# lhaippp/DMHomo

Measured on AMD Instinct MI355X. Metric: sampled images/sec (128x128, s_step=32), higher is better.
Workload: dtype f32; 1 GPU; DGM CFG-Unet dim=64 128x128 bs=25/GPU s_step=32 cond_scale=3 (BASELINE configs[1]); global_batch=25, cfg_mode=streams, hip_graph=True, weights=seeded random init

## Files before the change

dmhomo_amd/_lib.py:

```python
import ctypes as C
import os

import torch

_HERE = os.path.dirname(os.path.abspath(__file__))
LIB_PATH = os.environ.get('DMH_LIB_PATH') or os.path.join(_HERE, 'libdmhomo_hip.so')

c_f32p = C.c_void_p
c_i64 = C.c_int64
c_int = C.c_int
c_float = C.c_float


ABI_VERSION = 500


class DmhConv(C.Structure):
    _fields_ = [('struct_size', C.c_uint64)] + \
               [(n, C.c_void_p) for n in ('src0', 'src1', 'wpack', 'bias', 'in_coef', 'res', 'res_coef', 'out',
                                          'stats')] + \
               [(n, C.c_int32) for n in ('B', 'Hin', 'Win', 'C0', 'C1', 'Cout', 'KH', 'KW', 'stride', 'upsample2')] + \
               [('in_bound', C.c_void_p), ('in_bound_n', C.c_int32), ('fin_n', C.c_int32), ('fin_w', C.c_void_p),
                ('fin_b', C.c_void_p), ('fin_out', C.c_void_p), ('pix_stats', C.c_void_p), ('pix_eps', C.c_float),
                ('rows', C.c_void_p)]


class DmhPackJob(C.Structure):
    _fields_ = [('src', C.c_void_p), ('ws', C.c_void_p), ('wpack', C.c_void_p), ('Cout', C.c_int32), ('C0', C.c_int32),
                ('C1', C.c_int32), ('KH', C.c_int32), ('transposed', C.c_int32)]


class DmhStep(C.Structure):
    _fields_ = [('objective', C.c_int32), ('clip', C.c_int32), ('mode', C.c_int32), ('cond_scale', C.c_float),
                ('sqrt_recip_ac', C.c_float), ('sqrt_recipm1_ac', C.c_float), ('sqrt_ac', C.c_float),
                ('sqrt_1m_ac', C.c_float), ('c0', C.c_float), ('c1', C.c_float), ('c2', C.c_float)]


SIGNATURES = {
    'dmh_last_error': (C.c_char_p, []),
    'dmh_version': (c_int, []),
    'dmh_ws_standardize': (c_int, [c_f32p, c_f32p, c_int, c_int, c_float, C.c_void_p]),
    'dmh_conv_pack_floats': (c_i64, [c_int, c_int, c_int, c_int, c_int]),
    'dmh_pack_conv_weight': (c_int, [c_f32p, c_f32p, c_int, c_int, c_int, c_int, c_int, C.c_void_p]),
    'dmh_pack_conv_weights_multi': (c_int, [C.c_void_p, c_int, c_float, C.c_void_p]),
    'dmh_conv_up2_pack_floats': (c_i64, [c_int, c_int]),
    'dmh_pack_conv_weight_up2': (c_int, [c_f32p, c_f32p, c_int, c_int, C.c_void_p]),
    'dmh_conv_tiles': (c_int, [c_int, c_int, c_int, c_int]),
    'dmh_conv2d': (c_int, [C.POINTER(DmhConv), C.c_void_p]),
    'dmh_rows_from_keep': (c_int, [C.c_void_p, c_int, c_int, C.c_void_p, C.c_void_p]),
    'dmh_gn_finalize': (c_int, [c_f32p, c_int, c_f32p, c_f32p, c_f32p, c_i64, c_f32p, c_int, c_int, c_int, c_int,
                                c_float, C.c_void_p, C.c_void_p]),
    'dmh_gn_finalize_bound': (c_int, [c_f32p, c_int, c_f32p, c_f32p, c_f32p, c_i64, c_f32p, c_f32p, c_int, c_int, c_int,
                                      c_int, c_float, C.c_void_p, C.c_void_p]),
    'dmh_gn_silu_residual': (c_int, [c_f32p, c_f32p, c_f32p, c_f32p, c_int, c_int, c_int, C.c_void_p, C.c_void_p]),
    'dmh_gn_silu_residual_stats': (c_int, [c_f32p, c_f32p, c_f32p, c_f32p, c_f32p, c_int, c_int, c_int, c_float, C.c_void_p,
                                           C.c_void_p]),
    'dmh_chan_layernorm': (c_int, [c_f32p, c_f32p, c_f32p, c_f32p, c_i64, c_int, c_float, C.c_void_p, c_i64, C.c_void_p]),
    'dmh_linattn_splits': (c_int, [c_int]),
    'dmh_linattn_partial_floats': (c_i64, [c_int, c_int]),
    'dmh_linattn_context': (c_int, [c_f32p, c_f32p, c_int, c_int, C.c_void_p, C.c_void_p]),
    'dmh_linattn_merge': (c_int, [c_f32p, c_f32p, c_int, c_int, C.c_void_p, C.c_void_p]),
    'dmh_linattn_apply': (c_int, [c_f32p, c_f32p, c_f32p, c_int, c_int, c_float, C.c_void_p, C.c_void_p]),
    'dmh_conv_wgrad_workspace_floats': (c_i64, [c_int, c_int, c_int, c_int, c_int, c_int, c_int]),
    'dmh_conv_wgrad': (c_int, [c_f32p, c_f32p, c_f32p, c_f32p, c_f32p, c_f32p, c_f32p, c_int, c_int, c_int, c_int, c_int,
                               c_int, c_int, c_int, C.c_void_p]),
    'dmh_conv_unshuffle_wgrad_workspace_floats': (c_i64, [c_int, c_int, c_int, c_int, c_int]),
    'dmh_conv_unshuffle_wgrad': (c_int, [c_f32p, c_f32p, c_f32p, c_f32p, c_f32p, c_int, c_int, c_int, c_int, c_int, C.c_void_p]),
    'dmh_s2d_shift': (c_int, [c_f32p, c_f32p, c_int, c_int, c_int, c_int, C.c_void_p]),
    'dmh_d2s': (c_int, [c_f32p, c_f32p, c_int, c_int, c_int, c_int, C.c_void_p]),
    'dmh_sumpool2': (c_int, [c_f32p, c_f32p, c_int, c_int, c_int, c_int, C.c_void_p]),
    'dmh_gn_finalize_train': (c_int, [c_f32p, c_int, c_f32p, c_f32p, c_f32p, c_i64, c_f32p, c_f32p, c_int, c_int, c_int,
                                      c_int, c_float, C.c_void_p]),
    'dmh_gn_bwd_chunks': (c_int, [c_int]),
    'dmh_gn_silu_backward': (c_int, [c_f32p, c_f32p, c_f32p, c_f32p, c_f32p, c_f32p, c_f32p, c_i64, c_f32p, c_f32p, c_f32p,
                                     c_f32p, c_int, c_int, c_int, c_int, C.c_void_p]),
    'dmh_sum_over_batch': (c_int, [c_f32p, c_f32p, c_int, c_i64, C.c_void_p]),
    'dmh_ws_backward': (c_int, [c_f32p, c_f32p, c_f32p, c_int, c_int, c_float, C.c_void_p]),
    'dmh_lnb_blocks': (c_int, []),
    'dmh_chan_layernorm_backward': (c_int, [c_f32p, c_f32p, c_f32p, c_f32p, c_f32p, c_i64, c_int, c_float, C.c_void_p]),
    'dmh_linattn_merge_ms': (c_int, [c_f32p, c_f32p, c_f32p, c_int, c_int, C.c_void_p]),
    'dmh_linattn_bwd_workspace_floats': (c_i64, [c_int, c_int]),
    'dmh_linattn_backward': (c_int, [c_f32p, c_f32p, c_f32p, c_f32p, c_f32p, c_f32p, c_int, c_int, c_float, C.c_void_p]),
    'dmh_bgemm': (c_int, [c_f32p, C.POINTER(c_i64), c_f32p, C.POINTER(c_i64), c_f32p, C.POINTER(c_i64), c_int, c_int, c_int,
                          c_int, c_int, c_float, C.c_void_p]),
    'dmh_softmax_rows': (c_int, [c_f32p, c_f32p, c_i64, c_int, C.c_void_p]),
    'dmh_softmax_rows_backward': (c_int, [c_f32p, c_f32p, c_i64, c_int, C.c_void_p]),
    'dmh_act': (c_int, [c_f32p, c_f32p, c_f32p, c_i64, c_int, C.c_void_p]),
    'dmh_class_embed_backward': (c_int, [c_f32p, c_f32p, c_f32p, c_f32p, c_f32p, c_int, c_int, c_int, C.c_void_p]),
    'dmh_loss_backward_ddp': (c_int, [c_f32p, c_f32p, c_f32p, c_f32p, c_int, c_i64, c_int, c_float, C.c_void_p]),
    'dmh_loss_backward': (c_int, [c_f32p, c_f32p, c_f32p, c_f32p, c_f32p, c_f32p, c_f32p, c_f32p, c_int, c_int, c_int, c_int,
                                  C.c_void_p]),
    'dmh_sumsq_blocks': (c_int, []),
    'dmh_sumsq': (c_int, [c_f32p, c_i64, c_f32p, C.c_void_p]),
    'dmh_gradnorm_finalize': (c_int, [c_f32p, c_int, c_float, c_f32p, C.c_void_p]),
    'dmh_adam': (c_int, [c_f32p, c_f32p, c_f32p, c_f32p, c_f32p, c_i64, c_float, c_float, c_float, c_float, c_int,
                         C.c_void_p]),
    'dmh_ema': (c_int, [c_f32p, c_f32p, c_i64, c_float, C.c_void_p]),
    'dmh_multi_blocks': (c_i64, [C.c_void_p, c_int]),
    'dmh_sumsq_multi': (c_int, [C.c_void_p, C.c_void_p, c_int, c_f32p, C.c_void_p]),
    'dmh_adam_multi': (c_int, [C.c_void_p, C.c_void_p, C.c_void_p, C.c_void_p, C.c_void_p, c_int, c_f32p, c_float, c_float,
                               c_float, c_float, c_int, C.c_void_p]),
    'dmh_resize_bilinear_u8': (c_int, [C.c_void_p, c_f32p, c_int, c_int, c_int, c_int, c_int, c_int, c_i64, c_float,
                                       C.c_void_p]),
    'dmh_mask_open_nearest': (c_int, [c_f32p, c_f32p, c_int, c_int, c_int, c_int, c_int, c_i64, C.c_void_p]),
    'dmh_pixel_stats': (c_int, [c_f32p, c_f32p, c_i64, c_int, c_float, C.c_void_p, c_i64, C.c_void_p]),
    'dmh_linattn_fused_pack_floats': (c_i64, [c_int]),
    'dmh_linattn_fused_pack': (c_int, [c_f32p, c_f32p, c_int, C.c_void_p]),
    'dmh_linattn_fused_splits': (c_int, [c_int, c_int]),
    'dmh_linattn_fused_context': (c_int, [c_f32p, c_f32p, c_f32p, c_f32p, c_f32p, c_int, c_int, c_int, C.c_void_p, C.c_void_p]),
    'dmh_linattn_out_pack_floats': (c_i64, []),
    'dmh_linattn_out_pack': (c_int, [c_f32p, c_f32p, C.c_void_p]),
    'dmh_linattn_fused_apply_out': (c_int, [c_f32p, c_f32p, c_f32p, c_f32p, c_f32p, c_f32p, c_f32p, c_f32p, c_f32p, c_int,
                                            c_int, c_int, c_float, c_float, C.c_void_p, C.c_void_p]),
    'dmh_linattn_merge_n': (c_int, [c_f32p, c_f32p, c_int, c_int, c_int, C.c_void_p, C.c_void_p]),
    'dmh_linattn_fused_apply': (c_int, [c_f32p, c_f32p, c_f32p, c_f32p, c_f32p, c_f32p, c_int, c_int, c_int, c_float,
                                        C.c_void_p, C.c_void_p]),
    'dmh_attention': (c_int, [c_f32p, c_f32p, c_int, c_int, c_float, C.c_void_p, C.c_void_p]),
    'dmh_sinusoidal_embed': (c_int, [C.c_void_p, c_f32p, c_f32p, c_int, c_int, C.c_void_p]),
    'dmh_fourier_embed': (c_int, [C.c_void_p, c_f32p, c_f32p, c_int, c_int, C.c_void_p]),
    'dmh_class_embed': (c_int, [C.c_void_p, C.c_void_p, c_f32p, c_f32p, c_f32p, c_int, c_int, c_int, C.c_void_p]),
    'dmh_linear': (c_int, [c_f32p, c_i64, c_f32p, c_f32p, c_f32p, c_i64, c_int, c_int, c_int, c_int, c_int,
                           C.c_void_p]),
    'dmh_ss_gather': (c_int, [c_f32p, c_f32p, c_f32p, C.c_void_p, C.c_void_p, C.c_void_p, c_int, c_f32p, c_int, c_int, c_int,
                              C.c_void_p]),
    'dmh_assemble_input': (c_int, [c_f32p, c_int, c_f32p, c_int, c_f32p, c_f32p, c_int, c_int, c_int, c_int,
                                   C.c_void_p]),
    'dmh_final_conv_nchw': (c_int, [c_f32p, c_f32p, c_f32p, c_f32p, c_int, c_int, c_int, c_int, C.c_void_p]),
    'dmh_sampler_step': (c_int, [C.POINTER(DmhStep), c_f32p, c_f32p, c_f32p, c_f32p, c_f32p, c_f32p, c_f32p, c_i64,
                                 C.c_void_p, c_i64, C.c_void_p]),
    'dmh_sampler_step_dev': (c_int, [C.c_void_p, c_f32p, c_f32p, c_f32p, c_f32p, c_f32p, c_f32p, c_f32p, c_i64, C.c_void_p,
                                     c_i64, C.c_void_p]),
    'dmh_sampler_seek': (c_int, [C.c_void_p, c_int, C.c_void_p, C.c_void_p, c_int, C.c_void_p, C.c_void_p, c_int,
                                 C.c_void_p]),
    'dmh_sampler_step_ddp_dev': (c_int, [C.c_void_p, C.c_void_p, C.c_void_p, c_f32p, c_f32p, c_f32p, C.c_void_p, C.c_void_p,
                                         c_f32p, c_f32p, c_int, c_int, c_int, c_int, c_int, C.c_void_p]),
    'dmh_rng_indexed': (c_int, [c_f32p, c_int, c_i64, C.c_void_p, C.c_void_p, c_int, C.c_void_p]),
    'dmh_rng_keep_mask': (c_int, [C.c_void_p, c_int, C.c_void_p, C.c_void_p, c_float, C.c_void_p]),
    'dmh_rows_lincomb': (c_int, [c_f32p, c_f32p, c_f32p, c_f32p, c_f32p, c_f32p, c_int, c_i64, c_int, C.c_void_p]),
    'dmh_pixel_grid': (c_int, [c_f32p, c_int, c_int, c_int, c_float, C.c_void_p]),
    'dmh_norm_grid': (c_int, [c_f32p, c_f32p, c_int, c_int, c_int, C.c_void_p]),
    'dmh_homography_flow_points': (c_int, [C.c_void_p, C.c_void_p, C.c_void_p, c_int, c_int, c_int, c_int, c_int, C.c_void_p]),
    'dmh_dlt_points': (c_int, [C.c_void_p, C.c_void_p, C.c_void_p, C.c_void_p, c_int, c_int, C.c_void_p]),
    'dmh_affine': (c_int, [c_f32p, c_f32p, c_float, c_float, c_i64, C.c_void_p]),
    'dmh_affine_tail': (c_int, [c_f32p, c_int, c_int, c_int, c_int, c_float, c_float, C.c_void_p]),
    'dmh_q_sample': (c_int, [c_f32p, c_f32p, c_f32p, c_f32p, c_f32p, c_int, c_i64, C.c_void_p]),
    'dmh_diff_mean': (c_int, [c_f32p, c_f32p, c_f32p, c_int, C.c_void_p, c_f32p, c_int, c_int, c_int, C.c_void_p]),
    'dmh_loss_combine': (c_int, [c_f32p, c_f32p, c_f32p, c_f32p, c_int, C.c_void_p]),
    'dmh_to_uint8': (c_int, [c_f32p, C.c_void_p, c_i64, C.c_void_p]),
    'dmh_homography_flow': (c_int, [C.c_void_p, c_f32p, c_f32p, c_int, c_int, c_int, c_float, C.c_void_p]),
    'dmh_flow_to_image': (c_int, [c_f32p, c_f32p, c_int, c_int, c_float, C.c_void_p]),
    'dmh_flow_warp': (c_int, [c_f32p, c_f32p, c_f32p, C.c_void_p, C.c_void_p, c_int, c_int, c_int, c_int, c_int, c_int,
                              C.c_void_p]),
    'dmh_dlt_homography': (c_int, [c_f32p, C.c_void_p, C.c_void_p, c_int, c_int, c_int, C.c_void_p]),
    'dmh_post_process': (c_int, [c_f32p, c_f32p, c_f32p, c_f32p, c_f32p, c_int, c_int, c_int, C.c_void_p]),
    'dmh_preview_sheet': (c_int, [c_f32p, c_f32p, c_f32p, C.c_void_p, C.c_void_p, c_int, c_int, c_int, c_int, c_int, c_int,
                                  C.c_void_p]),
    'dmh_homography_warp': (c_int, [c_f32p, C.c_void_p, c_f32p, c_int, c_int, c_int, c_int, c_int, C.c_void_p]),
}

DLT_BLOCKS = 64

_lib = None


class DmhError(RuntimeError):
    pass


def lib():
    global _lib
    if _lib is None:
        if not os.path.exists(LIB_PATH):
            raise DmhError(f'{LIB_PATH} not found: build it with `python -c "import __graft_entry__ as g; g.build()"` '
                           f'or `make -C dmhomo_amd/csrc` — dmhomo_amd has no CPU / eager fallback')
        h = C.CDLL(LIB_PATH)
        for name, (res, args) in SIGNATURES.items():
            fn = getattr(h, name)
            fn.restype = res
            fn.argtypes = args
        got = int(h.dmh_version())
        if got != ABI_VERSION:
            raise DmhError(f'{LIB_PATH} reports ABI version {got}, this binding was written against {ABI_VERSION} '
                           f'(include/dmhomo_hip.h): rebuild the library with `make -C dmhomo_amd/csrc`')
        _lib = h
    return _lib


def stream():
    return C.c_void_p(torch.cuda.current_stream().cuda_stream)


def call(name, *args):
    h = lib()
    rc = getattr(h, name)(*args, stream())
    if rc != 0:
        raise DmhError(f'{name} failed ({rc}): {h.dmh_last_error().decode()}')


def ptr(t, dtype=torch.float32):
    if t is None:
        return None
    if not t.is_cuda:
        raise DmhError('dmhomo_amd kernels need tensors on the GPU (got a CPU tensor); there is no CPU path')
    if dtype is not None and t.dtype != dtype:
        raise DmhError(f'expected dtype {dtype}, got {t.dtype}')
    if not t.is_contiguous():
        raise DmhError('expected a contiguous tensor')
    return C.c_void_p(t.data_ptr())
```

dmhomo_amd/csrc/conv.hip:

```cpp
#include <stdlib.h>

#include "common.h"

#include "conv_args.h"

template <int KH, int KW, int S, int UPS, int KC, int TH, int TW>
struct ConvCfg {
  static constexpr int BM = TH * TW;
  static constexpr int MB = BM / 128;
  static constexpr int IN_H = (TH - 1) * S + KH;
  static constexpr int IN_W = (TW - 1) * S + KW;
  static constexpr int IN_PIX = IN_H * IN_W;
  static constexpr int KCP = KC + 4;
  static constexpr int C4 = KC / 4;
  static constexpr int NLOAD = (IN_PIX * C4 + 255) / 256;
  static constexpr int WL = 64 * C4 / 256;
  static constexpr int PAD = (S == 1) ? (KH / 2) : (KH == 4 ? 1 : 0);
  static constexpr int IN_FLOATS = IN_PIX * KCP;
  static constexpr int W_FLOATS = 64 * KCP;
  static constexpr int EPI_BYTES = 4 * 32 * 68 * 4;
  static constexpr int MAIN_BYTES = (IN_FLOATS + 2 * W_FLOATS) * 4;
  static constexpr int LDS_BYTES = MAIN_BYTES > EPI_BYTES ? MAIN_BYTES : EPI_BYTES;
};

template <int MB, int TH, int TW>
__device__ __forceinline__ void conv_epilogue(floatx16 (&acc)[MB][2], const ConvArgs& p, float* lds, int b, int n0,
                                              int oy0, int ox0, int tile_in_sample) {
  constexpr int EP = EpilogueRows::EP;
  const int lane = threadIdx.x & 63, wave = threadIdx.x >> 6, half = lane >> 5, l31 = lane & 31;
  float* wl = lds + wave * (32 * EP);
  EpilogueRows er(p, b, n0);
#pragma unroll
  for (int mb = 0; mb < MB; ++mb) {
    __syncthreads();
#pragma unroll
    for (int nb = 0; nb < 2; ++nb)
#pragma unroll
      for (int r = 0; r < 16; ++r) wl[((r & 3) + 8 * (r >> 2) + 4 * half) * EP + nb * 32 + l31] = acc[mb][nb][r];
    __syncthreads();
    er.template store_rows<TW>(p, wl, wave * (MB * 32) + mb * 32, oy0, ox0);
  }
  er.write_stats(p, lds, tile_in_sample);
}

template <int KH, int KW, int S, int UPS, int KC, int TH, int TW, int WPE>
__global__ __launch_bounds__(256, WPE) void conv_igemm_kernel(ConvArgs p) {
  using Cfg = ConvCfg<KH, KW, S, UPS, KC, TH, TW>;
  constexpr int MB = Cfg::MB, IN_W = Cfg::IN_W, IN_PIX = Cfg::IN_PIX, KCP = Cfg::KCP, C4 = Cfg::C4;
  constexpr int NLOAD = Cfg::NLOAD, WL = Cfg::WL, NTAPS = KH * KW;

  extern __shared__ __attribute__((aligned(16))) float lds[];
  float* in_tile = lds;
  float* w_tile = lds + Cfg::IN_FLOATS;

  const int tid = threadIdx.x;
  const int lane = tid & 63;
  const int wave = tid >> 6;
  const int half = lane >> 5;
  const int l31 = lane & 31;

  int t = blockIdx.x;
  const int tx = t % p.tilesX;
  t /= p.tilesX;
  const int ty = t % p.tilesY;
  if (t / p.tilesY >= dmh_rows_n(p.rows, p.B)) return;
  const int b = dmh_rows_phys(p.rows, t / p.tilesY);
  const int nt = blockIdx.y;
  const int n0 = nt * 64;
  const int tile_in_sample = ty * p.tilesX + tx;

  const int oy0 = ty * TH, ox0 = tx * TW;
  const int iy0 = oy0 * S - Cfg::PAD, ix0 = ox0 * S - Cfg::PAD;
  const int Hlim = UPS ? p.Hin * 2 : p.Hin;
  const int Wlim = UPS ? p.Win * 2 : p.Win;

  int arow[MB];
#pragma unroll
  for (int mb = 0; mb < MB; ++mb) {
    const int r = wave * (MB * 32) + mb * 32 + l31;
    const int py = r / TW, px = r % TW;
    arow[mb] = ((py * S) * IN_W + px * S) * KCP + half * 4;
  }
  const int brow = l31 * KCP + half * 4;

  floatx16 acc[MB][2];
#pragma unroll
  for (int mb = 0; mb < MB; ++mb)
#pragma unroll
    for (int nb = 0; nb < 2; ++nb)
#pragma unroll
      for (int r = 0; r < 16; ++r) acc[mb][nb][r] = 0.f;

  const int nchunks = p.nch0 + p.nch1;
  const float* wbase = p.wpack + (size_t)nt * nchunks * NTAPS * 64 * KC;

  float4 wreg[WL];
#pragma unroll
  for (int i = 0; i < WL; ++i) wreg[i] = ld4(wbase + (size_t)(tid + i * 256) * 4);

  const int c4 = tid % C4;
  int wbuf = 0;

  float4 v[NLOAD];
  float4 ca, cb;
  int poff[NLOAD];
  unsigned inside = 0;
#pragma unroll
  for (int i = 0; i < NLOAD; ++i) {
    const int pix = (tid + i * 256) / C4;
    const int pixc = pix < IN_PIX ? pix : IN_PIX - 1;
    const int yy = iy0 + pixc / IN_W, xx = ix0 + pixc % IN_W;
    const bool ok = pix < IN_PIX && yy >= 0 && yy < Hlim && xx >= 0 && xx < Wlim;
    const int yc = min(max(yy, 0), Hlim - 1), xc = min(max(xx, 0), Wlim - 1);
    const int sy = UPS ? (yc >> 1) : yc, sx = UPS ? (xc >> 1) : xc;
    poff[i] = (b * p.Hin + sy) * p.Win + sx;
    inside |= (ok ? 1u : 0u) << i;
  }
  auto issue_chunk_loads = [&](int ch) {
    const bool s1 = ch >= p.nch0;
    const float* src = s1 ? p.src1 : p.src0;
    const int Csrc = s1 ? p.C1 : p.C0;
    const int c = (s1 ? ch - p.nch0 : ch) * KC + c4 * 4;
    const int cc = c < Csrc ? c : 0;
#pragma unroll
    for (int i = 0; i < NLOAD; ++i) v[i] = ld4(src + (size_t)poff[i] * Csrc + cc);
    ca = make_float4(1.f, 1.f, 1.f, 1.f);
    cb = make_float4(0.f, 0.f, 0.f, 0.f);
    if (p.in_coef != nullptr && !s1) {
      ca = ld4(p.in_coef + (size_t)(b * 2 + 0) * p.C0 + cc);
      cb = ld4(p.in_coef + (size_t)(b * 2 + 1) * p.C0 + cc);
    }
  };
  issue_chunk_loads(0);
  const int wr_in0 = (tid / C4) * KCP + c4 * 4;
  const int wr_w0 = (tid / C4) * KCP + (tid % C4) * 4;

  for (int ch = 0; ch < nchunks; ++ch) {
    const bool s1c = ch >= p.nch0;
    const bool pro = (p.in_coef != nullptr) && !s1c;
    const bool cvalid = (s1c ? ch - p.nch0 : ch) * KC + c4 * 4 < (s1c ? p.C1 : p.C0);
    const unsigned msk = cvalid ? inside : 0u;
    __syncthreads();
#pragma unroll
    for (int i = 0; i < NLOAD; ++i) {
      if ((i + 1) * 256 <= IN_PIX * C4 || (tid + i * 256) / C4 < IN_PIX) {
        float4 x = v[i];
        if (!((msk >> i) & 1u)) {
          x = make_float4(0.f, 0.f, 0.f, 0.f);
        } else if (pro) {
          x.x = silu_fast(fmaf(ca.x, x.x, cb.x));
          x.y = silu_fast(fmaf(ca.y, x.y, cb.y));
          x.z = silu_fast(fmaf(ca.z, x.z, cb.z));
          x.w = silu_fast(fmaf(ca.w, x.w, cb.w));
        }
        st4(in_tile + wr_in0 + i * (256 / C4) * KCP, x);
      }
    }

    for (int tap = 0; tap < NTAPS; ++tap) {
      float* wt = w_tile + wbuf * Cfg::W_FLOATS;
#pragma unroll
      for (int i = 0; i < WL; ++i) st4(wt + wr_w0 + i * (256 / C4) * KCP, wreg[i]);
      __syncthreads();
      {
        int nch = ch, ntap = tap + 1;
        if (ntap == NTAPS) {
          ntap = 0;
          nch = ch + 1;
        }
        if (nch < nchunks) {
          const float* wsrc = wbase + ((size_t)nch * NTAPS + ntap) * 64 * KC;
#pragma unroll
          for (int i = 0; i < WL; ++i) wreg[i] = ld4(wsrc + (size_t)(tid + i * 256) * 4);
        }
        if (tap == NTAPS - 1) issue_chunk_loads(ch + 1 < nchunks ? ch + 1 : ch);
      }
      __builtin_amdgcn_sched_barrier(0);
      const int kh = tap / KW, kw = tap % KW;
      const float* at = in_tile + (kh * IN_W + kw) * KCP;
      const float* bt = wt + brow;
#pragma unroll
      for (int k8 = 0; k8 < KC / 8; ++k8) {
        float4 a[MB], bq[2];
#pragma unroll
        for (int mb = 0; mb < MB; ++mb) a[mb] = ld4(at + arow[mb] + k8 * 8);
#pragma unroll
        for (int nb = 0; nb < 2; ++nb) bq[nb] = ld4(bt + nb * 32 * KCP + k8 * 8);
#pragma unroll
        for (int mb = 0; mb < MB; ++mb)
#pragma unroll
          for (int nb = 0; nb < 2; ++nb) {
            acc[mb][nb] = __builtin_amdgcn_mfma_f32_32x32x2f32(a[mb].x, bq[nb].x, acc[mb][nb], 0, 0, 0);
            acc[mb][nb] = __builtin_amdgcn_mfma_f32_32x32x2f32(a[mb].y, bq[nb].y, acc[mb][nb], 0, 0, 0);
            acc[mb][nb] = __builtin_amdgcn_mfma_f32_32x32x2f32(a[mb].z, bq[nb].z, acc[mb][nb], 0, 0, 0);
            acc[mb][nb] = __builtin_amdgcn_mfma_f32_32x32x2f32(a[mb].w, bq[nb].w, acc[mb][nb], 0, 0, 0);
          }
      }
      __builtin_amdgcn_sched_barrier(0);
      wbuf ^= 1;
    }
  }

  conv_epilogue<MB, TH, TW>(acc, p, lds, b, n0, oy0, ox0, tile_in_sample);
}

__global__ void pack_conv_weight_kernel(const float* __restrict__ w, float* __restrict__ wp, int Cout, int C0,
                                        int C1, int KH, int KW, int KC, int nch0, int nch1, int64_t total) {
  const int64_t idx = (int64_t)blockIdx.x * blockDim.x + threadIdx.x;
  if (idx >= total) return;
  int64_t r = idx;
  const int k = r % KC;
  r /= KC;
  const int j = r % 64;
  r /= 64;
  const int tap = r % (KH * KW);
  r /= (KH * KW);
  const int ch = r % (nch0 + nch1);
  const int nt = r / (nch0 + nch1);
  const int o = nt * 64 + j;
  int c;
  bool ok;
  if (ch < nch0) {
    c = ch * KC + k;
    ok = c < C0;
  } else {
    c = (ch - nch0) * KC + k;
    ok = c < C1;
    c += C0;
  }
  float val = 0.f;
  if (ok && o < Cout) val = w[((size_t)o * (C0 + C1) + c) * (KH * KW) + tap];
  wp[idx] = val;
}

__global__ __launch_bounds__(256) void ws_standardize_kernel(const float* __restrict__ w, float* __restrict__ out,
                                                             int K, float eps) {
  __shared__ float red[8];
  const int o = blockIdx.x;
  const float* wr = w + (size_t)o * K;
  float s = 0.f;
  for (int i = threadIdx.x; i < K; i += 256) s += wr[i];
  for (int off = 32; off; off >>= 1) s += __shfl_xor(s, off);
  if ((threadIdx.x & 63) == 0) red[threadIdx.x >> 6] = s;
  __syncthreads();
  const float mean = (red[0] + red[1] + red[2] + red[3]) / (float)K;
  float q = 0.f;
  for (int i = threadIdx.x; i < K; i += 256) {
    const float d = wr[i] - mean;
    q = fmaf(d, d, q);
  }
  for (int off = 32; off; off >>= 1) q += __shfl_xor(q, off);
  if ((threadIdx.x & 63) == 0) red[4 + (threadIdx.x >> 6)] = q;
  __syncthreads();
  const float var = (red[4] + red[5] + red[6] + red[7]) / (float)K;
  const float rstd = 1.0f / sqrtf(var + eps);
  for (int i = threadIdx.x; i < K; i += 256) out[(size_t)o * K + i] = (wr[i] - mean) * rstd;
}

template <int KH, int KW, int S, int UPS, int KC, int TH, int TW, int WPE = 2>
static int launch_conv(const DmhConv* d, int Hout, int Wout, hipStream_t st) {
  using Cfg = ConvCfg<KH, KW, S, UPS, KC, TH, TW>;
  ConvArgs a = fill_conv_args(d, Hout, Wout, KC, TH, TW);
  dim3 grid(a.tilesX * a.tilesY * a.B, cdiv(a.Cout, 64));
  hipLaunchKernelGGL((conv_igemm_kernel<KH, KW, S, UPS, KC, TH, TW, WPE>), grid, dim3(256), Cfg::LDS_BYTES, st, a);
  DMH_CHECK_LAUNCH("dmh_conv2d");
  return DMH_OK;
}

#define DMH_CONV3_DEFAULT 9
static int conv3_variant() {
  static int v = -1;
  if (v < 0) {
    const char* e = getenv("DMH_CONV3_VARIANT");
    v = e ? atoi(e) : DMH_CONV3_DEFAULT;
    if (v != 0 && v != 6) v = DMH_CONV3_DEFAULT;
  }
  return v;
}

static bool use_f16x3(int KH, int stride) {
  return conv3_variant() == 9 && stride == 1 && (KH == 3 || KH == 1 || KH == 7);
}
static bool use_f16x3_s2d(int KH, int stride, int C0, int C1) {
  return conv3_variant() == 9 && KH == 4 && stride == 2 && C1 == 0 && C0 % 32 == 0;
}

static int conv_out_dim(int in, int KH, int stride, int ups) {
  if (ups) return in * 2;
  if (stride == 1) return in;
  return KH == 4 ? (in + 2 - 4) / 2 + 1 : in / 2;
}

static int conv_th(int KH, int stride) {
  if (stride == 2) return 8;
  if (use_f16x3(KH, stride)) return 8;
  if (KH == 3 && conv3_variant() == 6) return 8;
  return 16;
}

extern "C" int dmh_conv_tiles(int Hout, int Wout, int KH, int stride) {
  if (!dmh_dims_ok({Hout, Wout})) return -1;
  return cdiv(Hout, conv_th(KH, stride)) * cdiv(Wout, 16);
}

extern "C" int64_t dmh_conv_pack_floats(int Cout, int C0, int C1, int KH, int KW) {
  if (!dmh_dims_ok({Cout, C0}) || !dmh_dims_ok({C1}, 0) || !dmh_dims_ok({KH, KW}, 1, 16)) return -1;
  if (KH == 3 && conv3_variant() == 6) return dmh_wino_pack_floats(Cout, C0, C1);
  if (use_f16x3(KH, (KH == 4 || KH == 2) ? 2 : 1) || use_f16x3_s2d(KH, 2, C0, C1))
    return dmh_f16x3_pack_floats(Cout, C0, C1, KH, KW);
  const int stride = (KH == 4 || KH == 2) ? 2 : 1;
  const int KC = conv_kc(KH, stride);
  return (int64_t)cdiv(Cout, 64) * (cdiv(C0, KC) + cdiv(C1, KC)) * KH * KW * 64 * KC;
}

extern "C" int dmh_pack_conv_weight(const float* w, float* wpack, int Cout, int C0, int C1, int KH, int KW,
                                    void* stream) {
  DMH_REQUIRE(w && wpack && Cout > 0 && C0 > 0 && C1 >= 0, "dmh_pack_conv_weight: bad arguments");
  DMH_REQUIRE(KH == KW && (KH == 1 || KH == 2 || KH == 3 || KH == 4 || KH == 7),
              "dmh_pack_conv_weight: unsupported kernel %dx%d", KH, KW);
  if (KH == 3 && conv3_variant() == 6) return dmh_wino_pack(w, wpack, Cout, C0, C1, (hipStream_t)stream);
  if (use_f16x3(KH, (KH == 4 || KH == 2) ? 2 : 1) || use_f16x3_s2d(KH, 2, C0, C1))
    return dmh_f16x3_pack(w, wpack, Cout, C0, C1, KH, KW, (hipStream_t)stream);
  const int stride = (KH == 4 || KH == 2) ? 2 : 1;
  const int KC = conv_kc(KH, stride);
  const int nch0 = cdiv(C0, KC), nch1 = cdiv(C1, KC);
  const int64_t total = dmh_conv_pack_floats(Cout, C0, C1, KH, KW);
  hipLaunchKernelGGL(pack_conv_weight_kernel, dim3((unsigned)cdiv64(total, 256)), dim3(256), 0, (hipStream_t)stream,
                     w, wpack, Cout, C0, C1, KH, KW, KC, nch0, nch1, total);
  DMH_CHECK_LAUNCH("dmh_pack_conv_weight");
  return DMH_OK;
}

extern "C" int64_t dmh_conv_up2_pack_floats(int Cout, int C0) {
  if (!dmh_dims_ok({Cout, C0})) return -1;
  if (!use_f16x3(3, 1) || Cout % 64 != 0 || C0 % 4 != 0) return -1;
  return dmh_f16x3_up2_pack_floats(Cout, C0);
}
extern "C" int dmh_pack_conv_weight_up2(const float* w, float* wpack, int Cout, int C0, void* stream) {
  DMH_REQUIRE(w && wpack && dmh_conv_up2_pack_floats(Cout, C0) > 0, "dmh_pack_conv_weight_up2: bad arguments");
  return dmh_f16x3_up2_pack(w, wpack, Cout, C0, (hipStream_t)stream);
}

extern "C" int dmh_pack_conv_weights_multi(const DmhPackJob* jobs, int njobs, float ws_eps, void* stream) {
  DMH_REQUIRE(jobs && njobs > 0, "dmh_pack_conv_weights_multi: bad arguments");
  DMH_REQUIRE(conv3_variant() == 9, "dmh_pack_conv_weights_multi: only the fp16-piece images (DMH_CONV3_VARIANT=9)");
  for (int i = 0; i < njobs; ++i) {
    const DmhPackJob& j = jobs[i];
    DMH_REQUIRE(j.src && j.wpack && j.Cout > 0 && j.C0 > 0 && j.C1 >= 0 && (j.KH == 1 || j.KH == 3) &&
                    (j.transposed == 0 || (j.transposed == 1 && j.C1 == 0)),
                "dmh_pack_conv_weights_multi: job %d: stride-1 1x1 / 3x3 weights only (Cout %d, C0 %d, C1 %d, KH %d, transposed %d)",
                i, j.Cout, j.C0, j.C1, j.KH, j.transposed);
  }
  return dmh_f16x3_pack_multi(jobs, njobs, ws_eps, (hipStream_t)stream);
}

extern "C" int dmh_ws_standardize(const float* w, float* w_out, int Cout, int K, float eps, void* stream) {
  DMH_REQUIRE(w && w_out && Cout > 0 && K > 0, "dmh_ws_standardize: bad arguments");
  hipLaunchKernelGGL(ws_standardize_kernel, dim3(Cout), dim3(256), 0, (hipStream_t)stream, w, w_out, K, eps);
  DMH_CHECK_LAUNCH("dmh_ws_standardize");
  return DMH_OK;
}

extern "C" int dmh_conv2d(const DmhConv* d, void* stream) {
  DMH_REQUIRE(d && d->struct_size == sizeof(DmhConv),
              "dmh_conv2d: DmhConv.struct_size is %llu, this library's DmhConv has %llu bytes (header / library mismatch)",
              d ? (unsigned long long)d->struct_size : 0ull, (unsigned long long)sizeof(DmhConv));
  DMH_REQUIRE(d->src0 && d->wpack, "dmh_conv2d: null pointer");
  DMH_REQUIRE(d->B > 0 && d->Hin > 0 && d->Win > 0 && d->C0 > 0 && d->Cout > 0, "dmh_conv2d: bad shape");
  DMH_REQUIRE(d->C0 % 4 == 0 && (!d->src1 || d->C1 % 4 == 0),
              "dmh_conv2d: input channels must be a multiple of 4 (got %d, %d)", d->C0, d->C1);
  DMH_REQUIRE(!(d->in_coef && d->src1), "dmh_conv2d: the GroupNorm prologue applies to a single source");
  DMH_REQUIRE(!(d->res_coef && !d->res), "dmh_conv2d: res_coef without res");
  DMH_REQUIRE(d->Cout % 4 == 0, "dmh_conv2d: Cout must be a multiple of 4 (got %d)", d->Cout);
  DMH_REQUIRE(!d->in_bound || (d->in_coef && d->in_bound_n > 0 && d->in_bound_n <= 64),
              "dmh_conv2d: in_bound needs in_coef and 1..64 bounds per sample (got %d)", d->in_bound_n);
  hipStream_t st = (hipStream_t)stream;
  const int Hout = conv_out_dim(d->Hin, d->KH, d->stride, d->upsample2);
  const int Wout = conv_out_dim(d->Win, d->KW, d->stride, d->upsample2);
  const int key = d->KH * 100 + d->stride * 10 + d->upsample2;
  DMH_REQUIRE(d->KH == d->KW, "dmh_conv2d: non-square kernel");
  if (d->fin_w) {
    DMH_REQUIRE(d->fin_out && d->fin_n > 0 && d->fin_n <= 8, "dmh_conv2d: fin_w needs fin_out and 1 <= fin_n <= 8 (got %d)",
                d->fin_n);
    DMH_REQUIRE(d->KH == 1 && d->stride == 1 && d->Cout <= 64 && use_f16x3(1, 1),
                "dmh_conv2d: the fused final projection rides on the 1x1 fp16-piece kernel with Cout <= 64 (got %dx%d, Cout %d)",
                d->KH, d->KW, d->Cout);
  } else {
    DMH_REQUIRE(d->out, "dmh_conv2d: null pointer");
  }
  DMH_REQUIRE(!d->pix_stats || (d->KH == 1 && d->stride == 1 && d->Cout == 64 && use_f16x3(1, 1)),
              "dmh_conv2d: pix_stats rides on the 1x1 fp16-piece kernel with Cout == 64 (got %dx%d, Cout %d)", d->KH, d->KW,
              d->Cout);
  switch (key) {
    case 110:
      if (use_f16x3(1, 1)) return dmh_f16x3_launch(d, Hout, Wout, st);
      return launch_conv<1, 1, 1, 0, 32, 16, 16>(d, Hout, Wout, st);
    case 310:
      switch (conv3_variant()) {
        case 6: return dmh_wino_launch(d, Hout, Wout, st);
        case 9: return dmh_f16x3_launch(d, Hout, Wout, st);
        default: return launch_conv<3, 3, 1, 0, 32, 16, 16, 2>(d, Hout, Wout, st);
      }
    case 311:
      switch (conv3_variant()) {
        case 6: return dmh_wino_launch(d, Hout, Wout, st);
        case 9: return dmh_f16x3_launch(d, Hout, Wout, st);
        default: return launch_conv<3, 3, 1, 1, 32, 16, 16, 2>(d, Hout, Wout, st);
      }
    case 312:
      DMH_REQUIRE(use_f16x3(3, 1) && !d->src1 && d->Cout % 64 == 0 && !d->stats,
                  "dmh_conv2d: the sub-pixel upsampling conv needs the fp16-piece kernels, one source, Cout %% 64 == 0, no stats");
      return dmh_f16x3_launch_up2(d, Hout, Wout, st);
    case 710:
      if (use_f16x3(7, 1)) return dmh_f16x3_launch(d, Hout, Wout, st);
      return launch_conv<7, 7, 1, 0, 16, 16, 16>(d, Hout, Wout, st);
    case 420:
      if (use_f16x3_s2d(4, 2, d->C0, d->src1 ? d->C1 : 0)) {
        DMH_REQUIRE(!d->in_coef, "dmh_conv2d: the 4x4 / stride-2 conv takes no GroupNorm prologue");
        return dmh_f16x3_launch(d, Hout, Wout, st);
      }
      return launch_conv<4, 4, 2, 0, 16, 8, 16>(d, Hout, Wout, st);
    case 220:
      DMH_REQUIRE(d->Hin % 2 == 0 && d->Win % 2 == 0, "dmh_conv2d: 2x2/s2 needs even input size");
      return launch_conv<2, 2, 2, 0, 16, 8, 16>(d, Hout, Wout, st);
    default:
      dmh_set_error("dmh_conv2d: unsupported variant k=%d stride=%d upsample=%d", d->KH, d->stride, d->upsample2);
      return DMH_EINVAL;
  }
}
```

dmhomo_amd/csrc/conv_args.h:

```cpp
#pragma once
#include "common.h"

typedef float floatx16 __attribute__((ext_vector_type(16)));

struct ConvArgs {
  const float* src0;
  const float* src1;
  const float* wpack;
  const float* bias;
  const float* in_coef;
  const float* res;
  const float* res_coef;
  float* out;
  float* stats;
  const float* oscale;
  const float* in_bound;
  int in_bound_n;
  int fin_n;
  const float* fin_w;
  const float* fin_b;
  float* fin_out;
  float* pix_stats;
  float pix_eps;
  int B, Hin, Win, C0, C1, Cout, Hout, Wout;
  int nch0, nch1, tilesX, tilesY;
  int ablate;
  int xcd;
  const int32_t* rows;
};


static inline ConvArgs fill_conv_args(const DmhConv* d, int Hout, int Wout, int KC, int TH, int TW) {
  ConvArgs a;
  a.src0 = d->src0;
  a.src1 = d->src1;
  a.wpack = d->wpack;
  a.bias = d->bias;
  a.in_coef = d->in_coef;
  a.res = d->res;
  a.res_coef = d->res_coef;
  a.out = d->out;
  a.stats = d->stats;
  a.oscale = nullptr;
  a.in_bound = d->in_coef ? d->in_bound : nullptr;
  a.in_bound_n = d->in_bound_n;
  a.fin_n = d->fin_w ? d->fin_n : 0;
  a.fin_w = d->fin_w;
  a.fin_b = d->fin_b;
  a.fin_out = d->fin_out;
  a.pix_stats = d->pix_stats;
  a.pix_eps = d->pix_eps;
  a.B = d->B;
  a.Hin = d->Hin;
  a.Win = d->Win;
  a.C0 = d->C0;
  a.C1 = d->src1 ? d->C1 : 0;
  a.Cout = d->Cout;
  a.Hout = Hout;
  a.Wout = Wout;
  a.nch0 = cdiv(a.C0, KC);
  a.nch1 = cdiv(a.C1, KC);
  a.tilesX = cdiv(Wout, TW);
  a.tilesY = cdiv(Hout, TH);
  a.ablate = 0;
  a.xcd = 1;
  a.rows = d->rows;
  return a;
}


int64_t dmh_wino_pack_floats(int Cout, int C0, int C1);
int dmh_wino_pack(const float* w, float* wpack, int Cout, int C0, int C1, hipStream_t st);
int dmh_wino_launch(const DmhConv* d, int Hout, int Wout, hipStream_t st);


int64_t dmh_f16x3_pack_floats(int Cout, int C0, int C1, int KH, int KW);
int dmh_f16x3_pack(const float* w, float* wpack, int Cout, int C0, int C1, int KH, int KW, hipStream_t st);
int dmh_f16x3_launch(const DmhConv* d, int Hout, int Wout, hipStream_t st);
int dmh_f16x3_pack_multi(const DmhPackJob* jobs, int njobs, float eps, hipStream_t st);
int64_t dmh_f16x3_up2_pack_floats(int Cout, int C0);
int dmh_f16x3_up2_pack(const float* w, float* wpack, int Cout, int C0, hipStream_t st);
int dmh_f16x3_launch_up2(const DmhConv* d, int Hout, int Wout, hipStream_t st);


struct EpilogueRows {
  static constexpr int EP = 68;
  int b, n0, chn, c4, rsub;
  bool cok;
  float4 bias, ra, rb, s1, s2, osc;

  __device__ __forceinline__ EpilogueRows(const ConvArgs& p, int b_, int n0_) : b(b_), n0(n0_) {
    const int lane = threadIdx.x & 63;
    c4 = lane & 15;
    rsub = lane >> 4;
    chn = n0 + c4 * 4;
    cok = chn < p.Cout;
    bias = make_float4(0.f, 0.f, 0.f, 0.f);
    ra = bias;
    rb = bias;
    s1 = bias;
    s2 = bias;
    osc = make_float4(1.f, 1.f, 1.f, 1.f);
    if (cok && p.oscale) osc = ld4(p.oscale + chn);
    if (cok && p.bias) bias = ld4(p.bias + chn);
    if (cok && p.res_coef) {
      ra = ld4(p.res_coef + (size_t)(b * 2 + 0) * p.Cout + chn);
      rb = ld4(p.res_coef + (size_t)(b * 2 + 1) * p.Cout + chn);
    }
  }

  template <int TW, bool FIN = false>
  __device__ __forceinline__ void store_rows(const ConvArgs& p, const float* wl, int row_base, int oy0, int ox0,
                                             int mul = 1, int dy = 0, int dx = 0) {
    const int c4_ = c4;
    store_rows_fn<TW, 8, FIN>(p, [wl, c4_](int rr) { return ld4(wl + rr * EP + c4_ * 4); }, row_base, oy0, ox0, mul, dy, dx);
  }

  size_t oo[8];
  bool okr[8];
  float4 rv[8];
  bool pre = false;
  template <int TW, int NR = 8>
  __device__ __forceinline__ void prefetch_rows(const ConvArgs& p, int row_base, int oy0, int ox0, int mul = 1, int dy = 0,
                                                int dx = 0) {
#pragma unroll
    for (int i = 0; i < NR; ++i) {
      const int row = row_base + i * 4 + rsub;
      const int oy = (oy0 + row / TW) * mul + dy, ox = (ox0 + row % TW) * mul + dx;
      okr[i] = cok && oy < p.Hout && ox < p.Wout;
      const int oyc = min(oy, p.Hout - 1), oxc = min(ox, p.Wout - 1);
      oo[i] = ((size_t)(b * p.Hout + oyc) * p.Wout + oxc) * p.Cout + (cok ? chn : 0);
    }
    if (p.res) {
#pragma unroll
      for (int i = 0; i < NR; ++i) rv[i] = ld4(p.res + oo[i]);
    }
    pre = true;
  }

  template <int TW, int NR = 8, bool FIN = false, typename Fetch>
  __device__ __forceinline__ void store_rows_fn(const ConvArgs& p, Fetch fetch, int row_base, int oy0, int ox0,
                                                int mul = 1, int dy = 0, int dx = 0) {
    if (!pre) prefetch_rows<TW, NR>(p, row_base, oy0, ox0, mul, dy, dx);
    pre = false;
    float4 val[8];
#pragma unroll
    for (int i = 0; i < NR; ++i) val[i] = fetch(i * 4 + rsub);
#pragma unroll
    for (int i = 0; i < NR; ++i) {
      val[i].x = fmaf(val[i].x, osc.x, bias.x);
      val[i].y = fmaf(val[i].y, osc.y, bias.y);
      val[i].z = fmaf(val[i].z, osc.z, bias.z);
      val[i].w = fmaf(val[i].w, osc.w, bias.w);
    }
    if (p.res) {
      if (p.res_coef) {
#pragma unroll
        for (int i = 0; i < NR; ++i) {
          val[i].x += silu_fast(fmaf(ra.x, rv[i].x, rb.x));
          val[i].y += silu_fast(fmaf(ra.y, rv[i].y, rb.y));
          val[i].z += silu_fast(fmaf(ra.z, rv[i].z, rb.z));
          val[i].w += silu_fast(fmaf(ra.w, rv[i].w, rb.w));
        }
      } else {
#pragma unroll
        for (int i = 0; i < NR; ++i) {
          val[i].x += rv[i].x;
          val[i].y += rv[i].y;
          val[i].z += rv[i].z;
          val[i].w += rv[i].w;
        }
      }
    }
    if constexpr (FIN) {
      if (p.fin_n > 0) {
        const int hw = p.Hout * p.Wout;
#pragma unroll
        for (int o = 0; o < 8; ++o) {
          if (o < p.fin_n) {
            const float4 wq = cok ? ld4(p.fin_w + (size_t)o * p.Cout + chn) : make_float4(0.f, 0.f, 0.f, 0.f);
            const float bo = p.fin_b ? p.fin_b[o] : 0.f;
#pragma unroll
            for (int i = 0; i < NR; ++i) {
              float acc = fmaf(val[i].x, wq.x, 0.f);
              acc = fmaf(val[i].y, wq.y, acc);
              acc = fmaf(val[i].z, wq.z, acc);
              acc = fmaf(val[i].w, wq.w, acc);
              const float t = row16_sum(acc);
              const int row = row_base + i * 4 + rsub;
              const int oy = (oy0 + row / TW) * mul + dy, ox = (ox0 + row % TW) * mul + dx;
              if (c4 == o && oy < p.Hout && ox < p.Wout) p.fin_out[((size_t)b * p.fin_n + o) * hw + oy * p.Wout + ox] = t + bo;
            }
          }
        }
      }
      if (p.pix_stats) {
#pragma unroll
        for (int i = 0; i < NR; ++i) {
          float s = (val[i].x + val[i].y) + (val[i].z + val[i].w);
          s = lanes_sum<16>(s);
          const float mean = s / 64.0f;
          const float dx_ = val[i].x - mean, dy_ = val[i].y - mean, dz_ = val[i].z - mean, dw_ = val[i].w - mean;
          float qsum = (dx_ * dx_ + dy_ * dy_) + (dz_ * dz_ + dw_ * dw_);
          qsum = lanes_sum<16>(qsum);
          if (c4 == 0 && okr[i]) {
            float* ps = p.pix_stats + (oo[i] / (size_t)p.Cout) * 2;
            ps[0] = mean;
            ps[1] = 1.0f / sqrtf(qsum / 64.0f + p.pix_eps);
          }
        }
      }
    }
#pragma unroll
    for (int i = 0; i < NR; ++i) {
      if (okr[i] && (!FIN || p.out)) st4(p.out + oo[i], val[i]);
      const float k = okr[i] ? 1.f : 0.f;
      const float vx = val[i].x * k, vy = val[i].y * k, vz = val[i].z * k, vw = val[i].w * k;
      s1.x += vx;
      s1.y += vy;
      s1.z += vz;
      s1.w += vw;
      s2.x = fmaf(vx, vx, s2.x);
      s2.y = fmaf(vy, vy, s2.y);
      s2.z = fmaf(vz, vz, s2.z);
      s2.w = fmaf(vw, vw, s2.w);
    }
  }

  template <int WM, int WN, int TH>
  __device__ __forceinline__ void write_stats_grid(const ConvArgs& p, float* lds, int ty, int tx, int by = -1) {
    if (by < 0) by = blockIdx.y;
    if (!p.stats) return;
    const int lane = threadIdx.x & 63, wave = threadIdx.x >> 6, tid = threadIdx.x;
    s1.x = rows_sum(s1.x);
    s1.y = rows_sum(s1.y);
    s1.z = rows_sum(s1.z);
    s1.w = rows_sum(s1.w);
    s2.x = rows_sum(s2.x);
    s2.y = rows_sum(s2.y);
    s2.z = rows_sum(s2.z);
    s2.w = rows_sum(s2.w);
    __syncthreads();
    float* red = lds;
    if (lane < 16) {
      float* q = red + (wave * 64 + c4 * 4) * 2;
      q[0] = s1.x;
      q[1] = s2.x;
      q[2] = s1.y;
      q[3] = s2.y;
      q[4] = s1.z;
      q[5] = s2.z;
      q[6] = s1.w;
      q[7] = s2.w;
    }
    __syncthreads();
    if (tid < 128) {
      const int q = tid >> 6, c = tid & 63;
      const int g = WN == 1 ? q : 0, wnq = WN == 1 ? 0 : q;
      const int chan = (by * WN + wnq) * 64 + c;
      const int srow = ty * (TH / 8) + g;
      if (chan < p.Cout && srow * 8 < p.Hout) {
        const int w0 = (g * 2 + 0) * WN + wnq, w1 = (g * 2 + 1) * WN + wnq;
        const float a0 = red[(w0 * 64 + c) * 2 + 0] + red[(w1 * 64 + c) * 2 + 0];
        const float a1 = red[(w0 * 64 + c) * 2 + 1] + red[(w1 * 64 + c) * 2 + 1];
        const int stiles = ((p.Hout + 7) / 8) * p.tilesX;
        float* st = p.stats + ((size_t)(b * stiles + srow * p.tilesX + tx) * p.Cout + chan) * 2;
        st[0] = a0;
        st[1] = a1;
      }
    }
  }

  __device__ __forceinline__ void write_stats(const ConvArgs& p, float* lds, int tile_in_sample) {
    if (!p.stats) return;
    const int lane = threadIdx.x & 63, wave = (threadIdx.x >> 6) & 3, tid = threadIdx.x & 255;
    lds += (threadIdx.x >> 8) * 512;
    s1.x = rows_sum(s1.x);
    s1.y = rows_sum(s1.y);
    s1.z = rows_sum(s1.z);
    s1.w = rows_sum(s1.w);
    s2.x = rows_sum(s2.x);
    s2.y = rows_sum(s2.y);
    s2.z = rows_sum(s2.z);
    s2.w = rows_sum(s2.w);
    __syncthreads();
    float* red = lds;
    if (lane < 16) {
      float* q = red + (wave * 64 + c4 * 4) * 2;
      q[0] = s1.x;
      q[1] = s2.x;
      q[2] = s1.y;
      q[3] = s2.y;
      q[4] = s1.z;
      q[5] = s2.z;
      q[6] = s1.w;
      q[7] = s2.w;
    }
    __syncthreads();
    if (tid < 64 && n0 + tid < p.Cout) {
      float a0 = 0.f, a1 = 0.f;
#pragma unroll
      for (int w = 0; w < 4; ++w) {
        a0 += red[(w * 64 + tid) * 2 + 0];
        a1 += red[(w * 64 + tid) * 2 + 1];
      }
      float* st = p.stats + ((size_t)(b * p.tilesX * p.tilesY + tile_in_sample) * p.Cout + n0 + tid) * 2;
      st[0] = a0;
      st[1] = a1;
    }
  }
};
```

dmhomo_amd/csrc/conv_f16x3.hip:

```cpp
#include <stdlib.h>

#include "common.h"

#include "conv_args.h"

typedef _Float16 half8 __attribute__((ext_vector_type(8)));
typedef _Float16 half4 __attribute__((ext_vector_type(4)));
typedef float float4v __attribute__((ext_vector_type(4)));

namespace {

constexpr int KC = 32;
constexpr int PITCH = 160;
constexpr int STEP_U4 = 4 * 64;

template <int KH, int KW, int S, int UPS, int TH, int TW, int WM, int WN>
struct F16Cfg {
  static_assert(WM * WN == 4, "four waves per workgroup");
  static constexpr bool SUB = UPS == 3;
  static_assert(SUB || TH * TW == WM * 64, "64 pixels per wave");
  static_assert(!SUB || (KH == 2 && KW == 2 && S == 1 && TH == 4 && TW == 16 && WM == 4 && WN == 1), "sub-pixel geometry");
  static constexpr int IN_H = SUB ? TH + 2 : (TH - 1) * S + KH;
  static constexpr int IN_W = SUB ? TW + 2 : (TW - 1) * S + KW;
  static constexpr int IN_PIX = IN_H * IN_W;
  static constexpr int QS = UPS == 4 ? 2 : 3, NQ = 1 << QS;
  static constexpr int NLOAD = (IN_PIX * NQ + 255) / 256;
  static constexpr int PAD = UPS == 2 ? 0 : ((S == 1) ? (KH / 2) : (KH == 4 ? 1 : 0));
  static constexpr int ROWP = IN_W * PITCH;
  static constexpr int IN_BYTES = IN_H * ROWP;
  static constexpr int EPI_BYTES = 4 * 32 * EpilogueRows::EP * 4;
  static constexpr int TILE_BYTES = IN_BYTES > EPI_BYTES ? IN_BYTES : EPI_BYTES;
  static constexpr int LDS_BYTES = TILE_BYTES + 16;
};

__device__ __forceinline__ unsigned absbits(float x) { return __float_as_uint(x) & 0x7fffffffu; }

__device__ __forceinline__ int64_t f16x3_frag_floats_dev(int Cout, int C0, int C1, int T) {
  return (int64_t)((Cout + 63) / 64) * ((C0 + KC - 1) / KC + (C1 + KC - 1) / KC) * T * 2 * STEP_U4 * 4;
}

}

template <int KH, int KW, int S, int UPS, int TH, int TW, int WM, int WN>
__global__ __launch_bounds__(256, 2) void conv_f16x3_kernel(ConvArgs p) {
  using Cfg = F16Cfg<KH, KW, S, UPS, TH, TW, WM, WN>;
  constexpr bool PK = UPS == 4;
  constexpr int IN_W = Cfg::IN_W, IN_PIX = Cfg::IN_PIX, NLOAD = Cfg::NLOAD, NTAPS = PK ? (KH * KW + 1) / 2 : KH * KW,
                ROWP = Cfg::ROWP;

  extern __shared__ __attribute__((aligned(16))) float lds[];
  unsigned char* in_tile = reinterpret_cast<unsigned char*>(lds);
  unsigned* mxslot = reinterpret_cast<unsigned*>(in_tile + Cfg::TILE_BYTES);

  const int tid = threadIdx.x;
  const int lane = tid & 63;
  const int wave = tid >> 6;
  const int wave_u = __builtin_amdgcn_readfirstlane(wave);
  const int kg = lane >> 4;
  const int l15 = lane & 15;
  const int wm = wave / WN, wn = wave % WN;

  int t = blockIdx.x, by = blockIdx.y, nb = gridDim.x;
  if (p.rows) {
    nb = p.tilesX * p.tilesY * p.rows[0];
    const int lin = t + by * (int)gridDim.x;
    if (lin >= nb * (int)gridDim.y) return;
    t = lin % nb;
    by = lin / nb;
  }
  if (p.xcd) {
    const int total = nb * gridDim.y, lin = t + by * nb;
    const int q = total >> 3, r = total & 7, xcd = lin & 7, local = lin >> 3;
    const int nl = xcd * q + min(xcd, r) + local;
    if (p.xcd == 2) {
      by = nl % (int)gridDim.y;
      t = nl / (int)gridDim.y;
    } else {
      t = nl % nb;
      by = nl / nb;
    }
  }
  const int tx = t % p.tilesX;
  t /= p.tilesX;
  const int ty = t % p.tilesY;
  const int b = dmh_rows_phys(p.rows, t / p.tilesY);
  const int nt = UPS == 3 ? wm * (int)gridDim.y + by : by * WN + wn;
  const int n0 = UPS == 3 ? by * 64 : nt * 64;

  const int oy0 = ty * TH, ox0 = tx * TW;
  const int iy0 = oy0 * S - Cfg::PAD, ix0 = ox0 * S - Cfg::PAD;
  const int Hlim = UPS == 1 ? p.Hin * 2 : (UPS == 2 ? p.Hin / 2 + 1 : p.Hin);
  const int Wlim = UPS == 1 ? p.Win * 2 : (UPS == 2 ? p.Win / 2 + 1 : p.Win);

  if (tid < 2) mxslot[tid] = 0u;
#ifdef DMH_STAMPS
  unsigned long long tk[8] = {0, 0, 0, 0, 0, 0, 0, 0};
  unsigned long long t_prev, t_now;
#define STAMP(i)                                                                 \
  __builtin_amdgcn_sched_barrier(0);                                             \
  asm volatile("s_memtime %0\n\ts_waitcnt lgkmcnt(0)" : "=s"(t_now)::"memory"); \
  __builtin_amdgcn_sched_barrier(0);                                             \
  tk[i] += t_now - t_prev;                                                       \
  t_prev = t_now;
  asm volatile("s_memtime %0\n\ts_waitcnt lgkmcnt(0)" : "=s"(t_prev)::"memory");
  const unsigned long long t_begin = t_prev;
  const unsigned long long rt_begin = __builtin_amdgcn_s_memrealtime();
#else
#define STAMP(i)
#endif

  static_assert(TW == 16, "a 16-row MFMA block is one tile row");
  int arow[4];
#pragma unroll
  for (int mb = 0; mb < 4; ++mb)
    arow[mb] = UPS == 3 ? (mb + (wm >> 1)) * ROWP + (l15 + (wm & 1)) * PITCH + kg * 16
                        : ((wm * 4 + mb) * S) * ROWP + (l15 * S) * PITCH + (PK ? (kg & 1) : kg) * 16;

  float4v acc[4][4];
#pragma unroll
  for (int mb = 0; mb < 4; ++mb)
#pragma unroll
    for (int nb = 0; nb < 4; ++nb) acc[mb][nb] = float4v{0.f, 0.f, 0.f, 0.f};

  const int nchunks = p.nch0 + p.nch1;
  const int nsteps = nchunks * NTAPS * 2;
  const uint4* wbase = reinterpret_cast<const uint4*>(p.wpack) + (size_t)__builtin_amdgcn_readfirstlane(nt) * nsteps * STEP_U4;

  constexpr bool ROWREUSE = KH == 3 && KW == 3 && S == 1 && UPS != 3 && UPS != 2;
  constexpr int NSTEP = NTAPS * 2;
  constexpr int NB = (NSTEP % 3 == 0 && WN != 1) ? 3 : 2;
  uint4 bq[NB][4];
  auto tap_of = [](int pos) constexpr { return ROWREUSE ? (pos % 3) * 3 + pos / 3 : pos; };
  auto load_b = [&](int buf, int ch_, int st_) {
    if (st_ >= NSTEP) {
      st_ -= NSTEP;
      ch_ += 1;
    }
    if (ch_ >= nchunks) ch_ = nchunks - 1;
    const uint4* src = wbase + ((size_t)(ch_ * NTAPS + tap_of(st_ >> 1)) * 2 + (st_ & 1)) * STEP_U4;
#pragma unroll
    for (int i = 0; i < 4; ++i) bq[buf][i] = src[i * 64 + lane];
  };
#pragma unroll
  for (int i = 0; i < NB - 1; ++i) load_b(i, 0, i);

  constexpr int QS = Cfg::QS, NQ = Cfg::NQ;
  const int c4 = tid & (NQ - 1);
  float4 v[NLOAD];
  constexpr bool PACKPW = KH == 3 && KW == 3 && S == 1 && UPS == 0 && WN == 1;
  int poff[NLOAD], wroff[PACKPW ? 1 : NLOAD];
  const int y0c = min(max(iy0, 0), Hlim - 1), x0c = min(max(ix0, 0), Wlim - 1);
  const int pbase = PACKPW ? (b * p.Hin + y0c) * p.Win + x0c : 0;
  unsigned inside = 0;
#pragma unroll
  for (int i = 0; i < NLOAD; ++i) {
    const int pix = (tid + i * 256) >> QS;
    const int pixc = pix < IN_PIX ? pix : IN_PIX - 1;
    const int wro = (pixc / IN_W) * ROWP + (pixc % IN_W) * PITCH + c4 * 8;
    if (!PACKPW) wroff[i] = wro;
    const int yy = iy0 + pixc / IN_W, xx = ix0 + pixc % IN_W;
    const bool ok = pix < IN_PIX && yy >= 0 && yy < Hlim && xx >= 0 && xx < Wlim;
    const int yc = min(max(yy, 0), Hlim - 1), xc = min(max(xx, 0), Wlim - 1);
    const int sy = UPS == 1 ? (yc >> 1) : yc, sx = UPS == 1 ? (xc >> 1) : xc;
    poff[i] = UPS == 2 ? ((yc << 16) | xc) : (b * p.Hin + sy) * p.Win + sx;
    if (PACKPW) poff[i] = (int)((unsigned)wro | ((unsigned)((yc - y0c) * p.Win + (xc - x0c)) << 16));
    inside |= (ok ? 1u : 0u) << i;
  }
  unsigned inside_ch = inside;
  const float* ld_src = p.src0;
  int ld_C = p.C0, ld_c = 0, ld_py = 0, ld_px = 0;
  auto issue_prep = [&](int ch) {
    const bool s1 = ch >= p.nch0;
    ld_src = s1 ? p.src1 : p.src0;
    ld_C = s1 ? p.C1 : p.C0;
    if (UPS == 2) {
      const int nchc = p.C0 / KC, par = ch / nchc;
      ld_py = par >> 1;
      ld_px = par & 1;
      ld_c = (ch - par * nchc) * KC + c4 * 4;
      inside_ch = 0u;
    } else {
      const int c = (s1 ? ch - p.nch0 : ch) * KC + c4 * 4;
      ld_c = c < ld_C ? c : 0;
    }
  };
  auto issue_one = [&](int i) {
    const float* a;
    if (UPS == 2) {
      const int ry = 2 * (poff[i] >> 16) - 1 + ld_py, rx = 2 * (poff[i] & 0xffff) - 1 + ld_px;
      const bool ok = ((inside >> i) & 1u) && ry >= 0 && ry < p.Hin && rx >= 0 && rx < p.Win;
      const int yc = min(max(ry, 0), p.Hin - 1), xc = min(max(rx, 0), p.Win - 1);
      a = ld_src + ((size_t)(b * p.Hin + yc) * p.Win + xc) * ld_C + ld_c;
      inside_ch |= (ok ? 1u : 0u) << i;
    } else {
      if (PACKPW) a = ld_src + (size_t)pbase * ld_C + (int)(((unsigned)poff[i] >> 16) * (unsigned)ld_C + (unsigned)ld_c);
      else a = ld_src + (size_t)poff[i] * ld_C + ld_c;
    }
#ifdef DMH_STAMPS
    a = (p.ablate & 32) ? ld_src + ld_c : a;
#endif
    v[i] = ld4(a);
  };
  issue_prep(0);
#pragma unroll
  for (int i = 0; i < NLOAD; ++i) issue_one(i);
  __syncthreads();
#ifdef DMH_STAMPS
  if (p.ablate & 128) {
    const float* gs = p.src0 + (size_t)b * p.Hin * p.Win * p.C0;
    double q1 = 0.0, q2 = 0.0;
#pragma unroll
    for (int j = 0; j < 4; ++j) {
      const float2 t2 = *reinterpret_cast<const float2*>(gs + (size_t)(((tid & 31) + 32 * j) * 8 + (tid >> 5)) * 2);
      q1 += (double)t2.x;
      q2 += (double)t2.y;
    }
    for (int off = 16; off; off >>= 1) {
      q1 += __shfl_xor(q1, off);
      q2 += __shfl_xor(q2, off);
    }
    const double nn = (double)p.Hin * p.Win * (p.C0 / 8);
    const double mean = q1 / nn;
    double var = q2 / nn - mean * mean;
    var = var < 0.0 ? 0.0 : var;
    const float rstd = (float)(1.0 / sqrt(var + 1e-5)), meanf = (float)mean;
    float* tab = reinterpret_cast<float*>(in_tile);
    float* gtab = tab + 2 * 768;
    if ((tid & 31) == 0) {
      gtab[(tid >> 5) * 2 + 0] = meanf;
      gtab[(tid >> 5) * 2 + 1] = rstd;
    }
    __syncthreads();
    const float* cf = p.in_coef ? p.in_coef + (size_t)b * 2 * p.C0 : p.bias;
    for (int c = tid; c < p.C0 && c < 768; c += 256) {
      const int g8 = c / max(p.C0 / 8, 1);
      const float ga = cf ? cf[c % 64] : 1.f, be = cf ? cf[(c + 32) % 64] : 0.f;
      const float aa = gtab[g8 * 2 + 1] * ga;
      tab[c * 2 + 0] = aa;
      tab[c * 2 + 1] = be - gtab[g8 * 2 + 0] * aa;
    }
    __syncthreads();
    const float probe = tab[(tid & 63) * 2] + tab[(tid & 63) * 2 + 1];
    asm volatile("" ::"v"(probe));
    __syncthreads();
  }
#endif

  int e_run = 16;
  bool stat = p.in_bound != nullptr;
  int e_fix = 16;
  if (stat) {
    float m = 0.f;
    for (int i = 0; i < p.in_bound_n; ++i) {
      const float v = p.in_bound[b * p.in_bound_n + i];
      m = (v < INFINITY) ? fmaxf(m, v) : INFINITY;
    }
    const unsigned mb = __builtin_amdgcn_readfirstlane(__float_as_uint(m));
    stat = mb < 0x7f000000u;
    e_fix = min(max((int)(mb >> 23) + 1, 16), 254);
  }
  for (int ch = 0; ch < nchunks; ++ch) {
    const bool s1c = ch >= p.nch0;
    const bool pro = (p.in_coef != nullptr) && !s1c;
    float4 ca = make_float4(1.f, 1.f, 1.f, 1.f), cb = make_float4(0.f, 0.f, 0.f, 0.f);
    if (pro) {
      const int cq = ch * KC + c4 * 4;
      const int ccq = cq < p.C0 ? cq : 0;
      ca = ld4(p.in_coef + (size_t)(b * 2 + 0) * p.C0 + ccq);
      cb = ld4(p.in_coef + (size_t)(b * 2 + 1) * p.C0 + ccq);
    }
    const bool cvalid = UPS == 2 || (s1c ? ch - p.nch0 : ch) * KC + c4 * 4 < (s1c ? p.C1 : p.C0);
    const unsigned msk = cvalid ? inside_ch : 0u;
    if (pro) {
#pragma unroll
      for (int i = 0; i < NLOAD; ++i) {
        if ((i + 1) * 256 > IN_PIX * NQ && ((wave_u * 64 + i * 256) >> QS) >= IN_PIX) continue;
        v[i].x = silu_fast(fmaf(ca.x, v[i].x, cb.x));
        v[i].y = silu_fast(fmaf(ca.y, v[i].y, cb.y));
        v[i].z = silu_fast(fmaf(ca.z, v[i].z, cb.z));
        v[i].w = silu_fast(fmaf(ca.w, v[i].w, cb.w));
      }
    }
    if (!stat) {
      float mxf = 0.f;
#pragma unroll
      for (int i = 0; i < NLOAD; ++i) {
        if (pro && (i + 1) * 256 > IN_PIX * NQ && ((wave_u * 64 + i * 256) >> QS) >= IN_PIX) continue;
        mxf = fmaxf(fmaxf(mxf, fmaxf(fabsf(v[i].x), fabsf(v[i].y))), fmaxf(fabsf(v[i].z), fabsf(v[i].w)));
      }
      unsigned mx = __float_as_uint(mxf);
      mx = wave_max_u32(mx);
      if (lane == 0) atomicMax(&mxslot[ch & 1], mx);
    }
    STAMP(0)
    __syncthreads();
    STAMP(1)
    const int e_old = e_run;
    int e_ch = e_fix;
    if (!stat) {
      const unsigned bmx = mxslot[ch & 1];
      if (tid == 0) mxslot[(ch + 1) & 1] = 0u;
      e_ch = min(max((int)(__builtin_amdgcn_readfirstlane(bmx) >> 23), 16), 254);
    }
    e_run = max(e_run, e_ch);
    const float sc = __uint_as_float((unsigned)(268 - e_run) << 23);
    if (e_run != e_old && ch > 0) {
      const int fe = 127 + e_old - e_run;
      const float f = fe > 0 ? __uint_as_float((unsigned)fe << 23) : 0.f;
#pragma unroll
      for (int mb = 0; mb < 4; ++mb)
#pragma unroll
        for (int nb = 0; nb < 4; ++nb) acc[mb][nb] *= f;
    }
    const bool more = ch + 1 < nchunks;
    if (more) issue_prep(ch + 1);
#ifdef DMH_STAMPS
    if (p.ablate & 1) {
#pragma unroll
      for (int i = 0; i < NLOAD; ++i)
        if (more) issue_one(i);
    } else
#endif
#pragma unroll
    for (int i = 0; i < NLOAD; ++i) {
      if ((i + 1) * 256 <= IN_PIX * NQ || ((tid + i * 256) >> QS) < IN_PIX) {
        const float si = ((msk >> i) & 1u) ? sc : 0.f;
        uint2 h1, h2;
        dmh_split2(v[i].x, v[i].y, si, h1.x, h2.x);
        dmh_split2(v[i].z, v[i].w, si, h1.y, h2.y);
        int slot = PACKPW ? poff[i] : wroff[i];
        if (PACKPW) asm volatile("v_and_b32 %0, 0xffff, %0" : "+v"(slot));
        unsigned char* dst = in_tile + slot;
        *reinterpret_cast<uint2*>(dst) = h1;
        *reinterpret_cast<uint2*>(dst + 64) = h2;
      }
      if (more) issue_one(i);
    }
    STAMP(2)
    __syncthreads();
    STAMP(3)
    __builtin_amdgcn_sched_barrier(0);

    half8 a[4][2];
    half8 ar[ROWREUSE ? 5 : 1][2];
    auto read_a = [&](int tap) {
      const unsigned char* at = in_tile + (tap / KW) * ROWP + (tap % KW) * PITCH;
      if constexpr (PK) {
        const int t0 = 2 * tap, t1 = 2 * tap + 1 < KH * KW ? 2 * tap + 1 : 2 * tap;
        const int o0 = (t0 / KW) * ROWP + (t0 % KW) * PITCH, o1 = (t1 / KW) * ROWP + (t1 % KW) * PITCH;
        at = in_tile + ((kg >> 1) ? o1 : o0);
      }
#pragma unroll
      for (int mb = 0; mb < 4; ++mb)
#pragma unroll
        for (int pl = 0; pl < 2; ++pl) a[mb][pl] = *reinterpret_cast<const half8*>(at + arow[mb] + pl * 64);
    };
    auto read_rows = [&](int kx, int r0, int r1) {
      const unsigned char* at = in_tile + kx * PITCH;
#pragma unroll
      for (int r = r0; r < r1; ++r)
#pragma unroll
        for (int pl = 0; pl < 2; ++pl)
          ar[ROWREUSE ? r % 5 : 0][pl] = *reinterpret_cast<const half8*>(at + arow[0] + r * ROWP + pl * 64);
    };
#ifdef DMH_STAMPS
    if (!(p.ablate & 2))
#endif
    {
#pragma unroll
      for (int st = 0; st < NSTEP; ++st) {
#ifdef DMH_STAMPS
        if (!(p.ablate & 8))
#endif
        load_b((st + NB - 1) % NB, ch, st + NB - 1);
        __builtin_amdgcn_sched_barrier(0);
        const int pos = st >> 1;
#ifdef DMH_STAMPS
        if (!(p.ablate & 16) || st == 0)
#endif
        {
          if (ROWREUSE) {
            if ((st & 1) == 0) read_rows(pos / 3, pos % 3 == 0 ? 0 : 3 + pos % 3, 4 + pos % 3);
          } else if ((st & 1) == 0) {
            read_a(pos);
          }
        }
        auto afrag = [&](int mb, int pl) -> half8 {
          if constexpr (ROWREUSE) return ar[(mb + pos % 3) % 5][pl];
          else return a[mb][pl];
        };
#define DMH_A(mb, pl) afrag(mb, pl)
#pragma unroll
        for (int mb = 0; mb < 4; ++mb)
#pragma unroll
          for (int nb = 0; nb < 2; ++nb) {
            float4v& c = acc[mb][(st & 1) * 2 + nb];
            const half8 g1 = __builtin_bit_cast(half8, bq[st % NB][nb * 2]), g2 = __builtin_bit_cast(half8, bq[st % NB][nb * 2 + 1]);
            const half8 h1 = DMH_A(mb, 0), h2 = DMH_A(mb, 1);
            asm("v_mfma_f32_16x16x32_f16 %0, %1, %4, %0\n\t"
                "v_mfma_f32_16x16x32_f16 %0, %2, %3, %0\n\t"
                "v_mfma_f32_16x16x32_f16 %0, %1, %3, %0"
                : "+v"(c) : "v"(g1), "v"(g2), "v"(h1), "v"(h2));
          }
#undef DMH_A
      }
    }
#pragma unroll
    for (int mb = 0; mb < 4; mb += 2)
      asm volatile("s_nop 15" : "+v"(acc[mb][0]), "+v"(acc[mb][1]), "+v"(acc[mb][2]), "+v"(acc[mb][3]), "+v"(acc[mb + 1][0]),
                   "+v"(acc[mb + 1][1]), "+v"(acc[mb + 1][2]), "+v"(acc[mb + 1][3]));
    __builtin_amdgcn_sched_barrier(0);
    STAMP(4)
  }

#ifdef DMH_STAMPS
  if (!(p.ablate & 4))
#endif
  {
    constexpr int EP = EpilogueRows::EP;
    const float inv_s = __uint_as_float((unsigned)(e_run - 14) << 23);
    float* wl = lds + wave * (32 * EP);
    EpilogueRows er(p, b, n0);
    if (UPS == 3 && p.oscale) er.osc = ld4(p.oscale + nt * 64 + er.c4 * 4);
    er.osc.x *= inv_s;
    er.osc.y *= inv_s;
    er.osc.z *= inv_s;
    er.osc.w *= inv_s;
    __syncthreads();
#pragma unroll
    for (int hb = 0; hb < 2; ++hb) {
#pragma unroll
      for (int m2 = 0; m2 < 2; ++m2)
#pragma unroll
        for (int nb = 0; nb < 4; ++nb)
          *reinterpret_cast<float4v*>(wl + (m2 * 16 + l15) * EP + nb * 16 + kg * 4) = acc[hb * 2 + m2][nb];
      __builtin_amdgcn_fence(__ATOMIC_RELEASE, "wavefront");
      __builtin_amdgcn_wave_barrier();
      __builtin_amdgcn_fence(__ATOMIC_ACQUIRE, "wavefront");
      if (UPS == 3) er.template store_rows<TW>(p, wl, hb * 32, oy0, ox0, 2, wm >> 1, wm & 1);
      else er.template store_rows<TW, (KH == 1 && KW == 1 && WN == 1 && UPS == 0)>(p, wl, wm * 64 + hb * 32, oy0, ox0);
    }
#ifdef DMH_STAMPS
    STAMP(5)
    if (p.stats && lane == 0 && by == 0) {
      const int stiles = ((p.Hout + 7) / 8) * p.tilesX;
      unsigned long long* d = reinterpret_cast<unsigned long long*>(
                                  p.stats + ((size_t)(b * stiles + (ty * (TH / 8)) * p.tilesX + tx) * p.Cout) * 2) + wave * 8;
      for (int i = 0; i < 6; ++i) d[i] = tk[i];
      d[6] = t_now - t_begin;
      d[7] = __builtin_amdgcn_s_memrealtime() - rt_begin;
    }
#else
    er.template write_stats_grid<WM, WN, TH>(p, lds, ty, tx, by);
#endif
  }
}
#undef STAMP

__global__ __launch_bounds__(64) void f16x3_wscale_kernel(const float* __restrict__ w, float* __restrict__ oscale,
                                                           int Cout, int K) {
  const int o = blockIdx.x;
  float m = 0.f;
  if (o < Cout)
    for (int i = threadIdx.x; i < K; i += 64) m = fmaxf(m, fabsf(w[(size_t)o * K + i]));
  for (int off = 32; off; off >>= 1) m = fmaxf(m, __shfl_xor(m, off));
  if (threadIdx.x == 0) {
    float s = 1.f;
    if (m > 0.f && m < 3.0e38f) {
      int e;
      frexpf(m, &e);
      s = ldexpf(1.f, min(max(e - 15, -100), 100));
    }
    oscale[o] = s;
  }
}

__global__ void pack_f16x3_weight_kernel(const float* __restrict__ w, const float* __restrict__ oscale,
                                         _Float16* __restrict__ wp, int Cout, int C0, int C1, int NTAPS, int nch0,
                                         int nch1, int64_t total, int s2d, int pk) {
  const int64_t idx = (int64_t)blockIdx.x * blockDim.x + threadIdx.x;
  if (idx >= total) return;
  int64_t r = idx;
  const int j = r % 8;
  r /= 8;
  const int lane = r % 64;
  r /= 64;
  const int plane = r % 2;
  r /= 2;
  const int nb = r % 2;
  r /= 2;
  const int nh = r % 2;
  r /= 2;
  const int tap = r % NTAPS;
  r /= NTAPS;
  const int ch = r % (nch0 + nch1);
  const int nt = r / (nch0 + nch1);
  const int o = nt * 64 + nh * 32 + nb * 16 + (lane & 15);
  const int k = (lane >> 4) * 8 + j;
  int c;
  bool ok;
  if (ch < nch0) {
    c = ch * KC + k;
    ok = c < C0;
  } else {
    c = (ch - nch0) * KC + k;
    ok = c < C1;
    c += C0;
  }
  float ws = 0.f;
  if (s2d) {
    const int nchc = C0 / KC, par = ch / nchc;
    const int cr = (ch - par * nchc) * KC + k;
    const int ky = 2 * (tap >> 1) + (par >> 1), kx = 2 * (tap & 1) + (par & 1);
    if (o < Cout) ws = w[((size_t)o * C0 + cr) * 16 + ky * 4 + kx] / oscale[o];
  } else if (pk) {
    const int tt = 2 * tap + (k >> 4), cc = k & 15;
    if (o < Cout && cc < C0 && tt < 49) ws = w[((size_t)o * C0 + cc) * 49 + tt] / oscale[o];
  } else if (ok && o < Cout) {
    ws = w[((size_t)o * (C0 + C1) + c) * NTAPS + tap] / oscale[o];
  }
  const _Float16 g1 = (_Float16)ws;
  const _Float16 g2 = (_Float16)(ws - (float)g1);
  wp[idx] = plane == 0 ? g1 : g2;
}

static int64_t f16x3_frag_floats(int Cout, int C0, int C1, int KH, int KW);
#define PM_MAX 32
struct PmTable {
  const float* src[PM_MAX];
  float* ws[PM_MAX];
  float* wpack[PM_MAX];
  int Cout[PM_MAX], C0[PM_MAX], C1[PM_MAX], T[PM_MAX], tr[PM_MAX];
  int blk0[PM_MAX + 1];
  int count;
};
__device__ __forceinline__ int pm_find(const PmTable& t, int blk) {
  int lo = 0, hi = t.count;
  while (hi - lo > 1) {
    const int mid = (lo + hi) >> 1;
    if (t.blk0[mid] <= blk) lo = mid; else hi = mid;
  }
  return lo;
}
__device__ __forceinline__ float pm_elem(const float* w, int o, int c, int tap, int Cout, int Cin, int T, int tr) {
  return tr ? w[((size_t)c * Cout + o) * T + (T - 1 - tap)] : w[((size_t)o * Cin + c) * T + tap];
}
__global__ __launch_bounds__(256) void pm_ws_kernel(PmTable t, float eps) {
  __shared__ float red[8];
  const int ti = pm_find(t, blockIdx.x), o = blockIdx.x - t.blk0[ti];
  const int K = (t.tr[ti] ? t.Cout[ti] : t.C0[ti] + t.C1[ti]) * t.T[ti];
  const float* wr = t.src[ti] + (size_t)o * K;
  float* out = t.ws[ti] + (size_t)o * K;
  float s = 0.f;
  for (int i = threadIdx.x; i < K; i += 256) s += wr[i];
  for (int off = 32; off; off >>= 1) s += __shfl_xor(s, off);
  if ((threadIdx.x & 63) == 0) red[threadIdx.x >> 6] = s;
  __syncthreads();
  const float mean = (red[0] + red[1] + red[2] + red[3]) / (float)K;
  float q = 0.f;
  for (int i = threadIdx.x; i < K; i += 256) {
    const float d = wr[i] - mean;
    q = fmaf(d, d, q);
  }
  for (int off = 32; off; off >>= 1) q += __shfl_xor(q, off);
  if ((threadIdx.x & 63) == 0) red[4 + (threadIdx.x >> 6)] = q;
  __syncthreads();
  const float var = (red[4] + red[5] + red[6] + red[7]) / (float)K;
  const float rstd = 1.0f / sqrtf(var + eps);
  for (int i = threadIdx.x; i < K; i += 256) out[i] = (wr[i] - mean) * rstd;
}
__global__ __launch_bounds__(64) void pm_wscale_kernel(PmTable t) {
  const int ti = pm_find(t, blockIdx.x), o = blockIdx.x - t.blk0[ti];
  const int Cout = t.Cout[ti], Cin = t.C0[ti] + t.C1[ti], T = t.T[ti], tr = t.tr[ti], K = Cin * T;
  const float* w = t.ws[ti] ? t.ws[ti] : t.src[ti];
  float* oscale = t.wpack[ti] + f16x3_frag_floats_dev(Cout, t.C0[ti], t.C1[ti], T);
  float m = 0.f;
  if (o < Cout)
    for (int i = threadIdx.x; i < K; i += 64) m = fmaxf(m, fabsf(pm_elem(w, o, i / T, i % T, Cout, Cin, T, tr)));
  for (int off = 32; off; off >>= 1) m = fmaxf(m, __shfl_xor(m, off));
  if (threadIdx.x == 0) {
    float sc = 1.f;
    if (m > 0.f && m < 3.0e38f) {
      int e;
      frexpf(m, &e);
      sc = ldexpf(1.f, min(max(e - 15, -100), 100));
    }
    oscale[o] = sc;
  }
}
__global__ __launch_bounds__(256) void pm_pack_kernel(PmTable t) {
  const int ti = pm_find(t, blockIdx.x);
  const int Cout = t.Cout[ti], C0 = t.C0[ti], C1 = t.C1[ti], T = t.T[ti], tr = t.tr[ti];
  const int nch0 = (C0 + KC - 1) / KC, nch1 = (C1 + KC - 1) / KC;
  const int64_t frag = f16x3_frag_floats_dev(Cout, C0, C1, T);
  const int64_t total = frag * 2;
  const float* w = t.ws[ti] ? t.ws[ti] : t.src[ti];
  const float* oscale = t.wpack[ti] + frag;
  _Float16* wp = reinterpret_cast<_Float16*>(t.wpack[ti]);
  const int64_t base = (int64_t)(blockIdx.x - t.blk0[ti]) * 2048;
  for (int64_t idx = base + threadIdx.x; idx < min(base + 2048, total); idx += 256) {
    int64_t r = idx;
    const int j = r % 8;
    r /= 8;
    const int lane = r % 64;
    r /= 64;
    const int plane = r % 2;
    r /= 2;
    const int nb = r % 2;
    r /= 2;
    const int nh = r % 2;
    r /= 2;
    const int tap = r % T;
    r /= T;
    const int ch = r % (nch0 + nch1);
    const int nt = r / (nch0 + nch1);
    const int o = nt * 64 + nh * 32 + nb * 16 + (lane & 15);
    const int k = (lane >> 4) * 8 + j;
    int c;
    bool ok;
    if (ch < nch0) {
      c = ch * KC + k;
      ok = c < C0;
    } else {
      c = (ch - nch0) * KC + k;
      ok = c < C1;
      c += C0;
    }
    float ws = 0.f;
    if (ok && o < Cout) ws = pm_elem(w, o, c, tap, Cout, C0 + C1, T, tr) / oscale[o];
    const _Float16 g1 = (_Float16)ws;
    const _Float16 g2 = (_Float16)(ws - (float)g1);
    wp[idx] = plane == 0 ? g1 : g2;
  }
}

int dmh_f16x3_pack_multi(const DmhPackJob* jobs, int njobs, float eps, hipStream_t st) {
  for (int phase = 0; phase < 3; ++phase) {
    for (int i0 = 0; i0 < njobs;) {
      PmTable t;
      int k = 0, blocks = 0;
      for (; k < PM_MAX && i0 < njobs; ++i0) {
        const DmhPackJob& j = jobs[i0];
        if (phase == 0 && !j.ws) continue;
        const int T = j.KH * j.KH;
        t.src[k] = j.src;
        t.ws[k] = j.ws;
        t.wpack[k] = j.wpack;
        t.Cout[k] = j.Cout;
        t.C0[k] = j.C0;
        t.C1[k] = j.C1;
        t.T[k] = T;
        t.tr[k] = j.transposed;
        t.blk0[k] = blocks;
        if (phase == 0) blocks += j.transposed ? j.C0 + j.C1 : j.Cout;
        else if (phase == 1) blocks += cdiv(j.Cout, 64) * 64;
        else blocks += (int)cdiv64(f16x3_frag_floats(j.Cout, j.C0, j.C1, j.KH, j.KH) * 2, 2048);
        ++k;
      }
      if (k == 0) continue;
      t.blk0[k] = blocks;
      t.count = k;
      if (phase == 0) hipLaunchKernelGGL(pm_ws_kernel, dim3(blocks), dim3(256), 0, st, t, eps);
      else if (phase == 1) hipLaunchKernelGGL(pm_wscale_kernel, dim3(blocks), dim3(64), 0, st, t);
      else hipLaunchKernelGGL(pm_pack_kernel, dim3(blocks), dim3(256), 0, st, t);
      DMH_CHECK_LAUNCH("dmh_pack_conv_weights_multi");
    }
  }
  return DMH_OK;
}

static bool f16x3_pk(int C0, int C1, int KH) { return KH == 7 && C1 == 0 && C0 <= 16; }

static int64_t f16x3_frag_floats(int Cout, int C0, int C1, int KH, int KW) {
  if (KH == 4) return (int64_t)cdiv(Cout, 64) * (4 * C0 / KC) * 4 * 2 * STEP_U4 * 4;
  if (f16x3_pk(C0, C1, KH)) return (int64_t)cdiv(Cout, 64) * 25 * 2 * STEP_U4 * 4;
  return (int64_t)cdiv(Cout, 64) * (cdiv(C0, KC) + cdiv(C1, KC)) * KH * KW * 2 * STEP_U4 * 4;
}

int64_t dmh_f16x3_pack_floats(int Cout, int C0, int C1, int KH, int KW) {
  return f16x3_frag_floats(Cout, C0, C1, KH, KW) + (int64_t)cdiv(Cout, 64) * 64;
}

int dmh_f16x3_pack(const float* w, float* wpack, int Cout, int C0, int C1, int KH, int KW, hipStream_t st) {
  const bool s2d = KH == 4;
  const int nch0 = s2d ? 4 * C0 / KC : cdiv(C0, KC), nch1 = s2d ? 0 : cdiv(C1, KC);
  const int64_t frag = f16x3_frag_floats(Cout, C0, C1, KH, KW);
  float* oscale = wpack + frag;
  hipLaunchKernelGGL(f16x3_wscale_kernel, dim3(cdiv(Cout, 64) * 64), dim3(64), 0, st, w, oscale, Cout,
                     (C0 + C1) * KH * KW);
  const int64_t total = frag * 2;
  const bool pk = f16x3_pk(C0, C1, KH);
  hipLaunchKernelGGL(pack_f16x3_weight_kernel, dim3((unsigned)cdiv64(total, 256)), dim3(256), 0, st, w, oscale,
                     reinterpret_cast<_Float16*>(wpack), Cout, C0, C1, s2d ? 4 : (pk ? 25 : KH * KW), nch0, nch1, total,
                     s2d ? 1 : 0, pk ? 1 : 0);
  DMH_CHECK_LAUNCH("dmh_pack_conv_weight(f16x3)");
  return DMH_OK;
}

template <int KH, int KW, int S, int UPS, int TH, int TW, int WM, int WN>
static int launch_f16x3(const DmhConv* d, int Hout, int Wout, hipStream_t st) {
  using Cfg = F16Cfg<KH, KW, S, UPS, TH, TW, WM, WN>;
  ConvArgs a = fill_conv_args(d, Hout, Wout, KC, TH, TW);
  if (UPS == 2) a.nch0 = 4 * a.C0 / KC;
  a.oscale = d->wpack + f16x3_frag_floats(d->Cout, a.C0, a.C1, UPS == 2 ? 4 : KH, UPS == 2 ? 4 : KW);
#ifdef DMH_STAMPS
  if (const char* e = getenv("DMH_WINO_ABLATE")) a.ablate = atoi(e);
#endif
  auto kern = conv_f16x3_kernel<KH, KW, S, UPS, TH, TW, WM, WN>;
  DMH_RAISE_LDS_ONCE(kern, Cfg::LDS_BYTES, "dmh_conv2d(f16x3)");
  static const int xcd_deep = [] {
    const char* e = getenv("DMH_CONV_XCD_DEEP");
    return e ? atoi(e) : 32;
  }();
  if (xcd_deep > 0 && Hout <= xcd_deep && cdiv(a.Cout, 64 * WN) > 1) a.xcd = 2;
  dim3 grid(a.tilesX * a.tilesY * a.B, cdiv(a.Cout, 64 * WN));
  hipLaunchKernelGGL(kern, grid, dim3(256), Cfg::LDS_BYTES, st, a);
  DMH_CHECK_LAUNCH("dmh_conv2d(f16x3)");
  return DMH_OK;
}

__global__ void subpixel_weight_kernel(const float* __restrict__ w, float* __restrict__ wv, int Cout, int Cin) {
  const int64_t idx = (int64_t)blockIdx.x * blockDim.x + threadIdx.x;
  const int64_t total = (int64_t)4 * Cout * Cin * 4;
  if (idx >= total) return;
  const int tb = idx & 1, ta = (idx >> 1) & 1;
  int64_t r = idx >> 2;
  const int c = r % Cin;
  r /= Cin;
  const int o = r % Cout, par = r / Cout;
  const int dy = par >> 1, dx = par & 1;
  const int ky0 = dy == 0 ? (ta == 0 ? 0 : 1) : (ta == 0 ? 0 : 2), ky1 = dy == 0 ? (ta == 0 ? 0 : 2) : (ta == 0 ? 1 : 2);
  const int kx0 = dx == 0 ? (tb == 0 ? 0 : 1) : (tb == 0 ? 0 : 2), kx1 = dx == 0 ? (tb == 0 ? 0 : 2) : (tb == 0 ? 1 : 2);
  const float* wk = w + ((size_t)o * Cin + c) * 9;
  float s = 0.f;
  for (int ky = ky0; ky <= ky1; ++ky)
    for (int kx = kx0; kx <= kx1; ++kx) s += wk[ky * 3 + kx];
  wv[idx] = s;
}

int64_t dmh_f16x3_up2_pack_floats(int Cout, int C0) {
  return dmh_f16x3_pack_floats(4 * Cout, C0, 0, 2, 2) + (int64_t)16 * Cout * C0;
}

int dmh_f16x3_up2_pack(const float* w, float* wpack, int Cout, int C0, hipStream_t st) {
  float* wv = wpack + dmh_f16x3_pack_floats(4 * Cout, C0, 0, 2, 2);
  const int64_t total = (int64_t)16 * Cout * C0;
  hipLaunchKernelGGL(subpixel_weight_kernel, dim3((unsigned)cdiv64(total, 256)), dim3(256), 0, st, w, wv, Cout, C0);
  return dmh_f16x3_pack(wv, wpack, 4 * Cout, C0, 0, 2, 2, st);
}

int dmh_f16x3_launch_up2(const DmhConv* d, int Hout, int Wout, hipStream_t st) {
  using Cfg = F16Cfg<2, 2, 1, 3, 4, 16, 4, 1>;
  ConvArgs a = fill_conv_args(d, Hout, Wout, KC, 4, 16);
  a.tilesX = cdiv(d->Win, 16);
  a.tilesY = cdiv(d->Hin, 4);
  a.oscale = d->wpack + f16x3_frag_floats(4 * d->Cout, a.C0, 0, 2, 2);
  auto kern = conv_f16x3_kernel<2, 2, 1, 3, 4, 16, 4, 1>;
  DMH_RAISE_LDS_ONCE(kern, Cfg::LDS_BYTES, "dmh_conv2d(f16x3 sub-pixel)");
  dim3 grid(a.tilesX * a.tilesY * a.B, cdiv(a.Cout, 64));
  hipLaunchKernelGGL(kern, grid, dim3(256), Cfg::LDS_BYTES, st, a);
  DMH_CHECK_LAUNCH("dmh_conv2d(f16x3 sub-pixel)");
  return DMH_OK;
}

int dmh_f16x3_launch(const DmhConv* d, int Hout, int Wout, hipStream_t st) {
  const bool wide = d->Cout % 128 == 0;
  if (d->KH == 4) {
    return wide ? launch_f16x3<2, 2, 1, 2, 8, 16, 2, 2>(d, Hout, Wout, st)
                : launch_f16x3<2, 2, 1, 2, 16, 16, 4, 1>(d, Hout, Wout, st);
  }
  if (d->KH == 7) {
    if (f16x3_pk(d->C0, d->src1 ? d->C1 : 0, 7)) return launch_f16x3<7, 7, 1, 4, 16, 16, 4, 1>(d, Hout, Wout, st);
    return launch_f16x3<7, 7, 1, 0, 16, 16, 4, 1>(d, Hout, Wout, st);
  }
  if (d->KH == 1) {
    return wide ? launch_f16x3<1, 1, 1, 0, 8, 16, 2, 2>(d, Hout, Wout, st)
                : launch_f16x3<1, 1, 1, 0, 16, 16, 4, 1>(d, Hout, Wout, st);
  }
  if (d->upsample2) {
    return wide ? launch_f16x3<3, 3, 1, 1, 8, 16, 2, 2>(d, Hout, Wout, st)
                : launch_f16x3<3, 3, 1, 1, 16, 16, 4, 1>(d, Hout, Wout, st);
  }
  if (wide) return launch_f16x3<3, 3, 1, 0, 8, 16, 2, 2>(d, Hout, Wout, st);
  DMH_REQUIRE(17 * (int64_t)d->Win + 17 < 65536, "dmh_conv2d: 3x3 with Cout %% 128 != 0 supports Win <= 3853 (got %d)", d->Win);
  return launch_f16x3<3, 3, 1, 0, 16, 16, 4, 1>(d, Hout, Wout, st);
}
```

dmhomo_amd/csrc/norm.hip:

```cpp
#include "common.h"

__global__ __launch_bounds__(256) void gn_finalize_kernel(const float* __restrict__ stats, int tiles,
                                                          const float* __restrict__ gamma,
                                                          const float* __restrict__ beta, const float* __restrict__ ss,
                                                          int64_t ss_stride, float* __restrict__ coef, int C, int groups,
                                                          int hw, float eps, float* __restrict__ mr,
                                                          float* __restrict__ bound, const int32_t* __restrict__ rows) {
  __shared__ double red[2][4];
  __shared__ float bred[4];
  const int jb = blockIdx.x / groups, g = blockIdx.x % groups;
  if (jb >= dmh_rows_n(rows, gridDim.x / groups)) return;
  const int b = dmh_rows_phys(rows, jb);
  const int bg = b * groups + g;
  const int cg = C / groups;
  const int lane = threadIdx.x;
  double s1 = 0.0, s2 = 0.0;
  const int total = tiles * cg;
  for (int i = lane; i < total; i += 256) {
    const int tile = i / cg, cc = i % cg;
    const float2 st = *reinterpret_cast<const float2*>(stats + ((size_t)(b * tiles + tile) * C + g * cg + cc) * 2);
    s1 += (double)st.x;
    s2 += (double)st.y;
  }
  for (int off = 32; off; off >>= 1) {
    s1 += __shfl_xor(s1, off);
    s2 += __shfl_xor(s2, off);
  }
  if ((lane & 63) == 0) {
    red[0][lane >> 6] = s1;
    red[1][lane >> 6] = s2;
  }
  __syncthreads();
  s1 = (red[0][0] + red[0][1]) + (red[0][2] + red[0][3]);
  s2 = (red[1][0] + red[1][1]) + (red[1][2] + red[1][3]);
  const double n = (double)hw * (double)cg;
  const double mean = s1 / n;
  double var = s2 / n - mean * mean;
  if (var < 0.0) var = 0.0;
  const float rstd = (float)(1.0 / sqrt(var + (double)eps));
  const float meanf = (float)mean;
  if (mr && lane == 0) {
    mr[(size_t)bg * 2 + 0] = meanf;
    mr[(size_t)bg * 2 + 1] = rstd;
  }
  const float spread = (s2 > 4096.0 * n * (var + (double)eps)) ? INFINITY : (float)sqrt(s2 > 0.0 ? s2 : 0.0);
  float bmax = 0.f;
  for (int cc = lane; cc < cg; cc += 256) {
    const int c = g * cg + cc;
    float a = rstd * gamma[c];
    float bb = beta[c] - meanf * a;
    if (ss) {
      const float sc = ss[b * ss_stride + c] + 1.0f;
      const float sh = ss[b * ss_stride + C + c];
      a = a * sc;
      bb = fmaf(bb, sc, sh);
    }
    coef[(size_t)(b * 2 + 0) * C + c] = a;
    coef[(size_t)(b * 2 + 1) * C + c] = bb;
    bmax = fmaxf(bmax, spread < INFINITY ? fmaf(fabsf(a), spread, fabsf(fmaf(meanf, a, bb))) : INFINITY);
  }
  if (bound) {
    for (int off = 32; off; off >>= 1) bmax = fmaxf(bmax, __shfl_xor(bmax, off));
    if ((lane & 63) == 0) bred[lane >> 6] = bmax;
    __syncthreads();
    if (lane == 0) bound[bg] = fmaxf(fmaxf(bred[0], bred[1]), fmaxf(bred[2], bred[3]));
  }
}

template <int LPP>
__global__ __launch_bounds__(256) void gn_silu_residual_kernel(const float* __restrict__ y,
                                                               const float* __restrict__ coef,
                                                               const float* __restrict__ res, float* __restrict__ out,
                                                               int64_t per_sample4, int C, int64_t total4_all,
                                                               float* __restrict__ pstats, float eps,
                                                               const int32_t* __restrict__ rows) {
  const int C4 = C >> 2;
  const int lane = threadIdx.x & 63;
  const int64_t total4 = rows ? per_sample4 * rows[0] : total4_all;
  for (int64_t i0 = (int64_t)blockIdx.x * 256 + threadIdx.x; i0 - lane < total4; i0 += (int64_t)gridDim.x * 256) {
    const bool ok = i0 < total4;
    if (LPP == 0 && !ok) break;
    const int64_t il = ok ? i0 : total4 - 1;
    const int jb = (int)(il / per_sample4);
    const int b = dmh_rows_phys(rows, jb);
    const int64_t i = il + (int64_t)(b - jb) * per_sample4;
    const int c = (int)(i % C4) * 4;
    const float4 a = ld4(coef + (size_t)(b * 2 + 0) * C + c);
    const float4 bb = ld4(coef + (size_t)(b * 2 + 1) * C + c);
    const float4 v = ld4(y + i * 4);
    float4 r = make_float4(0.f, 0.f, 0.f, 0.f);
    if (res) r = ld4(res + i * 4);
    float4 o;
    o.x = silu_fast(fmaf(a.x, v.x, bb.x)) + r.x;
    o.y = silu_fast(fmaf(a.y, v.y, bb.y)) + r.y;
    o.z = silu_fast(fmaf(a.z, v.z, bb.z)) + r.z;
    o.w = silu_fast(fmaf(a.w, v.w, bb.w)) + r.w;
    if (ok) st4(out + i * 4, o);
    if (LPP > 0) {
      float s = 0.f;
      s += (o.x + o.y) + (o.z + o.w);
      s = lanes_sum<(LPP > 0 ? LPP : 1)>(s);
      const float mean = s / (float)C;
      float qsum = 0.f;
      const float dx = o.x - mean, dy = o.y - mean, dz = o.z - mean, dw = o.w - mean;
      qsum += (dx * dx + dy * dy) + (dz * dz + dw * dw);
      qsum = lanes_sum<(LPP > 0 ? LPP : 1)>(qsum);
      if (ok && (threadIdx.x % (LPP > 0 ? LPP : 1)) == 0) {
        const int64_t pix = i / C4;
        pstats[pix * 2 + 0] = mean;
        pstats[pix * 2 + 1] = 1.0f / sqrtf(qsum / (float)C + eps);
      }
    }
  }
}

template <int LPP, int NV>
__global__ __launch_bounds__(256) void chan_layernorm_kernel(const float* __restrict__ x, const float* __restrict__ g,
                                                             const float* __restrict__ res, float* __restrict__ out,
                                                             int64_t npix_all, int C, float eps,
                                                             const int32_t* __restrict__ rows, int64_t pix_per_row) {
  const int C4 = C >> 2;
  const int sub = threadIdx.x % LPP;
  const int64_t pix_per_block = 256 / LPP;
  const int64_t npix = rows ? pix_per_row * rows[0] : npix_all;
  for (int64_t pl = (int64_t)blockIdx.x * pix_per_block + threadIdx.x / LPP; pl < npix;
       pl += (int64_t)gridDim.x * pix_per_block) {
    const int64_t pix = rows ? (int64_t)rows[1 + pl / pix_per_row] * pix_per_row + pl % pix_per_row : pl;
    float4 v[NV];
    float s = 0.f;
#pragma unroll
    for (int j = 0; j < NV; ++j) {
      const int q = sub + j * LPP;
      v[j] = make_float4(0.f, 0.f, 0.f, 0.f);
      if (q < C4) v[j] = ld4(x + pix * C + q * 4);
      s += (v[j].x + v[j].y) + (v[j].z + v[j].w);
    }
    s = lanes_sum<LPP>(s);
    const float mean = s / (float)C;
    float qsum = 0.f;
#pragma unroll
    for (int j = 0; j < NV; ++j) {
      const int q = sub + j * LPP;
      if (q < C4) {
        const float dx = v[j].x - mean, dy = v[j].y - mean, dz = v[j].z - mean, dw = v[j].w - mean;
        qsum += (dx * dx + dy * dy) + (dz * dz + dw * dw);
      }
    }
    qsum = lanes_sum<LPP>(qsum);
    const float rstd = 1.0f / sqrtf(qsum / (float)C + eps);
#pragma unroll
    for (int j = 0; j < NV; ++j) {
      const int q = sub + j * LPP;
      if (q < C4) {
        const float4 gg = ld4(g + q * 4);
        float4 o;
        o.x = (v[j].x - mean) * rstd * gg.x;
        o.y = (v[j].y - mean) * rstd * gg.y;
        o.z = (v[j].z - mean) * rstd * gg.z;
        o.w = (v[j].w - mean) * rstd * gg.w;
        if (res) {
          const float4 r = ld4(res + pix * C + q * 4);
          o.x += r.x;
          o.y += r.y;
          o.z += r.z;
          o.w += r.w;
        }
        st4(out + pix * C + q * 4, o);
      }
    }
  }
}

extern "C" int dmh_gn_finalize(const float* stats, int tiles, const float* gamma, const float* beta, const float* ss,
                               int64_t ss_stride, float* coef, int B, int C, int groups, int hw, float eps,
                               const int32_t* rows, void* stream) {
  DMH_REQUIRE(stats && gamma && beta && coef, "dmh_gn_finalize: null pointer");
  DMH_REQUIRE(B > 0 && C > 0 && groups > 0 && C % groups == 0 && tiles > 0 && hw > 0, "dmh_gn_finalize: bad shape");
  hipLaunchKernelGGL(gn_finalize_kernel, dim3(B * groups), dim3(256), 0, (hipStream_t)stream, stats, tiles, gamma, beta,
                     ss, ss_stride, coef, C, groups, hw, eps, (float*)nullptr, (float*)nullptr, rows);
  DMH_CHECK_LAUNCH("dmh_gn_finalize");
  return DMH_OK;
}

extern "C" int dmh_gn_finalize_bound(const float* stats, int tiles, const float* gamma, const float* beta, const float* ss,
                                     int64_t ss_stride, float* coef, float* bound, int B, int C, int groups, int hw,
                                     float eps, const int32_t* rows, void* stream) {
  DMH_REQUIRE(stats && gamma && beta && coef && bound, "dmh_gn_finalize_bound: null pointer");
  DMH_REQUIRE(B > 0 && C > 0 && groups > 0 && C % groups == 0 && tiles > 0 && hw > 0, "dmh_gn_finalize_bound: bad shape");
  hipLaunchKernelGGL(gn_finalize_kernel, dim3(B * groups), dim3(256), 0, (hipStream_t)stream, stats, tiles, gamma, beta,
                     ss, ss_stride, coef, C, groups, hw, eps, (float*)nullptr, bound, rows);
  DMH_CHECK_LAUNCH("dmh_gn_finalize_bound");
  return DMH_OK;
}

extern "C" int dmh_gn_finalize_train(const float* stats, int tiles, const float* gamma, const float* beta,
                                     const float* ss, int64_t ss_stride, float* coef, float* mr, int B, int C,
                                     int groups, int hw, float eps, void* stream) {
  DMH_REQUIRE(stats && gamma && beta && coef && mr, "dmh_gn_finalize_train: null pointer");
  DMH_REQUIRE(B > 0 && C > 0 && groups > 0 && C % groups == 0 && tiles > 0 && hw > 0, "dmh_gn_finalize_train: bad shape");
  hipLaunchKernelGGL(gn_finalize_kernel, dim3(B * groups), dim3(256), 0, (hipStream_t)stream, stats, tiles, gamma, beta,
                     ss, ss_stride, coef, C, groups, hw, eps, mr, (float*)nullptr, (const int32_t*)nullptr);
  DMH_CHECK_LAUNCH("dmh_gn_finalize_train");
  return DMH_OK;
}

extern "C" int dmh_gn_silu_residual(const float* y, const float* coef, const float* res, float* out, int B, int HW,
                                    int C, const int32_t* rows, void* stream) {
  DMH_REQUIRE(y && coef && out, "dmh_gn_silu_residual: null pointer");
  DMH_REQUIRE(B > 0 && HW > 0 && C > 0 && C % 4 == 0, "dmh_gn_silu_residual: bad shape (C %% 4 != 0?)");
  const int64_t per_sample4 = (int64_t)HW * C / 4;
  const int64_t total4 = per_sample4 * B;
  const unsigned grid = (unsigned)(cdiv64(total4, 256) < 8192 ? cdiv64(total4, 256) : 8192);
  hipLaunchKernelGGL(gn_silu_residual_kernel<0>, dim3(grid), dim3(256), 0, (hipStream_t)stream, y, coef, res, out,
                     per_sample4, C, total4, (float*)nullptr, 0.f, rows);
  DMH_CHECK_LAUNCH("dmh_gn_silu_residual");
  return DMH_OK;
}

extern "C" int dmh_gn_silu_residual_stats(const float* y, const float* coef, const float* res, float* out, float* pstats,
                                          int B, int HW, int C, float eps, const int32_t* rows, void* stream) {
  DMH_REQUIRE(y && coef && out && pstats, "dmh_gn_silu_residual_stats: null pointer");
  DMH_REQUIRE(B > 0 && HW > 0 && (C == 64 || C == 128 || C == 256),
              "dmh_gn_silu_residual_stats: C must be 64, 128 or 256 (got %d)", C);
  const int64_t per_sample4 = (int64_t)HW * C / 4;
  const int64_t total4 = per_sample4 * B;
  const unsigned grid = (unsigned)(cdiv64(total4, 256) < 8192 ? cdiv64(total4, 256) : 8192);
  hipStream_t st = (hipStream_t)stream;
  if (C == 64)
    hipLaunchKernelGGL(gn_silu_residual_kernel<16>, dim3(grid), dim3(256), 0, st, y, coef, res, out, per_sample4, C, total4,
                       pstats, eps, rows);
  else if (C == 128)
    hipLaunchKernelGGL(gn_silu_residual_kernel<32>, dim3(grid), dim3(256), 0, st, y, coef, res, out, per_sample4, C, total4,
                       pstats, eps, rows);
  else
    hipLaunchKernelGGL(gn_silu_residual_kernel<64>, dim3(grid), dim3(256), 0, st, y, coef, res, out, per_sample4, C, total4,
                       pstats, eps, rows);
  DMH_CHECK_LAUNCH("dmh_gn_silu_residual_stats");
  return DMH_OK;
}

template <int LPP, int NV>
static int launch_ln(const float* x, const float* g, const float* res, float* out, int64_t npix, int C, float eps,
                     const int32_t* rows, int64_t ppr, hipStream_t st) {
  const int64_t ppb = 256 / LPP;
  const int64_t need = cdiv64(npix, ppb);
  const unsigned grid = (unsigned)(need < 16384 ? need : 16384);
  hipLaunchKernelGGL((chan_layernorm_kernel<LPP, NV>), dim3(grid), dim3(256), 0, st, x, g, res, out, npix, C, eps, rows, ppr);
  DMH_CHECK_LAUNCH("dmh_chan_layernorm");
  return DMH_OK;
}

template <int LPP, int NV>
__global__ __launch_bounds__(256) void pixel_stats_kernel(const float* __restrict__ x, float* __restrict__ stats,
                                                          int64_t npix_all, int C, float eps,
                                                          const int32_t* __restrict__ rows, int64_t pix_per_row) {
  const int C4 = C >> 2;
  const int sub = threadIdx.x % LPP;
  const int64_t pix_per_block = 256 / LPP;
  const int64_t npix = rows ? pix_per_row * rows[0] : npix_all;
  for (int64_t pl = (int64_t)blockIdx.x * pix_per_block + threadIdx.x / LPP; pl < npix;
       pl += (int64_t)gridDim.x * pix_per_block) {
    const int64_t pix = rows ? (int64_t)rows[1 + pl / pix_per_row] * pix_per_row + pl % pix_per_row : pl;
    float4 v[NV];
    float s = 0.f;
#pragma unroll
    for (int j = 0; j < NV; ++j) {
      const int q = sub + j * LPP;
      v[j] = make_float4(0.f, 0.f, 0.f, 0.f);
      if (q < C4) v[j] = ld4(x + pix * C + q * 4);
      s += (v[j].x + v[j].y) + (v[j].z + v[j].w);
    }
    s = lanes_sum<LPP>(s);
    const float mean = s / (float)C;
    float qsum = 0.f;
#pragma unroll
    for (int j = 0; j < NV; ++j) {
      const int q = sub + j * LPP;
      if (q < C4) {
        const float dx = v[j].x - mean, dy = v[j].y - mean, dz = v[j].z - mean, dw = v[j].w - mean;
        qsum += (dx * dx + dy * dy) + (dz * dz + dw * dw);
      }
    }
    qsum = lanes_sum<LPP>(qsum);
    if (sub == 0) {
      stats[pix * 2 + 0] = mean;
      stats[pix * 2 + 1] = 1.0f / sqrtf(qsum / (float)C + eps);
    }
  }
}

template <int LPP, int NV>
static int launch_ps(const float* x, float* stats, int64_t npix, int C, float eps, const int32_t* rows, int64_t ppr,
                     hipStream_t st) {
  const int64_t ppb = 256 / LPP;
  const int64_t need = cdiv64(npix, ppb);
  const unsigned grid = (unsigned)(need < 16384 ? need : 16384);
  hipLaunchKernelGGL((pixel_stats_kernel<LPP, NV>), dim3(grid), dim3(256), 0, st, x, stats, npix, C, eps, rows, ppr);
  DMH_CHECK_LAUNCH("dmh_pixel_stats");
  return DMH_OK;
}

extern "C" int dmh_pixel_stats(const float* x, float* stats, int64_t npix, int C, float eps, const int32_t* rows,
                               int64_t pix_per_row, void* stream) {
  DMH_REQUIRE(x && stats, "dmh_pixel_stats: null pointer");
  DMH_REQUIRE(!rows || (pix_per_row > 0 && npix % pix_per_row == 0), "dmh_pixel_stats: rows needs pix_per_row dividing npix");
  DMH_REQUIRE(npix > 0 && C > 0 && C % 4 == 0 && C <= 2048, "dmh_pixel_stats: unsupported C=%d", C);
  hipStream_t st = (hipStream_t)stream;
  const int C4 = C / 4;
  if (C4 <= 8) return launch_ps<8, 1>(x, stats, npix, C, eps, rows, pix_per_row, st);
  if (C4 <= 16) return launch_ps<16, 1>(x, stats, npix, C, eps, rows, pix_per_row, st);
  if (C4 <= 32) return launch_ps<32, 1>(x, stats, npix, C, eps, rows, pix_per_row, st);
  if (C4 <= 64) return launch_ps<64, 1>(x, stats, npix, C, eps, rows, pix_per_row, st);
  if (C4 <= 128) return launch_ps<64, 2>(x, stats, npix, C, eps, rows, pix_per_row, st);
  if (C4 <= 256) return launch_ps<64, 4>(x, stats, npix, C, eps, rows, pix_per_row, st);
  return launch_ps<64, 8>(x, stats, npix, C, eps, rows, pix_per_row, st);
}

extern "C" int dmh_chan_layernorm(const float* x, const float* g, const float* res, float* out, int64_t npix, int C,
                                  float eps, const int32_t* rows, int64_t pix_per_row, void* stream) {
  DMH_REQUIRE(x && g && out, "dmh_chan_layernorm: null pointer");
  DMH_REQUIRE(!rows || (pix_per_row > 0 && npix % pix_per_row == 0), "dmh_chan_layernorm: rows needs pix_per_row dividing npix");
  DMH_REQUIRE(npix > 0 && C > 0 && C % 4 == 0 && C <= 2048, "dmh_chan_layernorm: unsupported C=%d", C);
  hipStream_t st = (hipStream_t)stream;
  const int C4 = C / 4;
  if (C4 <= 2) return launch_ln<2, 1>(x, g, res, out, npix, C, eps, rows, pix_per_row, st);
  if (C4 <= 4) return launch_ln<4, 1>(x, g, res, out, npix, C, eps, rows, pix_per_row, st);
  if (C4 <= 8) return launch_ln<8, 1>(x, g, res, out, npix, C, eps, rows, pix_per_row, st);
  if (C4 <= 16) return launch_ln<16, 1>(x, g, res, out, npix, C, eps, rows, pix_per_row, st);
  if (C4 <= 32) return launch_ln<32, 1>(x, g, res, out, npix, C, eps, rows, pix_per_row, st);
  if (C4 <= 64) return launch_ln<64, 1>(x, g, res, out, npix, C, eps, rows, pix_per_row, st);
  if (C4 <= 128) return launch_ln<64, 2>(x, g, res, out, npix, C, eps, rows, pix_per_row, st);
  if (C4 <= 256) return launch_ln<64, 4>(x, g, res, out, npix, C, eps, rows, pix_per_row, st);
  return launch_ln<64, 8>(x, g, res, out, npix, C, eps, rows, pix_per_row, st);
}
```

dmhomo_amd/engine.py:

```python
import torch

from . import ops
from .layout import ATTN_SCALE, HIDDEN, sinusoidal_freq, unet_layout

FUSED_FINAL = True


class _Res:
    __slots__ = ('conv1', 'g1', 'b1', 'conv2', 'g2', 'b2', 'res', 'ss_off', 'cout')


class _Attn:
    __slots__ = ('linear', 'ln_g', 'qkv', 'pla', 'plo', 'out', 'out_g')


class UnetEngine:
    def __init__(self, module, groups=8):
        self.module = module
        self.groups = groups
        self._sig = None
        self._rows = None

    def _signature(self):
        return (getattr(self.module, '_dmh_epoch', 0),) + tuple((p.data_ptr(), p._version) for p in self.module.parameters())

    def ensure_prepared(self):
        sig = self._signature()
        if sig != self._sig:
            self.prepare()
            self._sig = sig

    def prepare(self):
        sd = {k: v.detach() for k, v in self.module.named_parameters()}
        dev = next(iter(sd.values())).device
        if dev.type != 'cuda':
            raise RuntimeError('dmhomo_amd: the UNet must live on the GPU (call .cuda()); there is no CPU path')
        f32 = lambda k: sd[k].to(torch.float32).contiguous()

        def conv(w, b, c0, c1=0, ws=False, stride=1, ups=0):
            w = f32(w)
            if ws:
                w = ops.ws_standardize(w)
            return ops.PackedConv(w, None if b is None else f32(b), c0, c1, stride, ups)

        L = unet_layout(sd)
        self.dim, self.has_classes = L.dim, L.has_classes
        emb_dim = sd['time_mlp.3.weight'].shape[0] * (2 if self.has_classes else 1)
        self.emb_dim = emb_dim

        self.fourier_w = f32('time_mlp.0.weights') if L.fourier else None
        if self.fourier_w is None:
            self.freq = sinusoidal_freq(self.dim, dev)
        self.t_w1, self.t_b1 = f32('time_mlp.1.weight').t().contiguous(), f32('time_mlp.1.bias')
        self.t_w2, self.t_b2 = f32('time_mlp.3.weight').t().contiguous(), f32('time_mlp.3.bias')
        if self.has_classes:
            self.c_table, self.c_null = f32('classes_emb.weight'), f32('null_classes_emb')
            self.c_w1, self.c_b1 = f32('classes_mlp.0.weight').t().contiguous(), f32('classes_mlp.0.bias')
            self.c_w2, self.c_b2 = f32('classes_mlp.2.weight').t().contiguous(), f32('classes_mlp.2.bias')

        w0 = f32('init_conv.weight')
        self.cin, self.cin_pad = L.cin, L.cin_pad
        if self.cin_pad != self.cin:
            wp = torch.zeros((w0.shape[0], self.cin_pad, 7, 7), device=dev, dtype=torch.float32)
            wp[:, :self.cin] = w0
            w0 = wp
        self.init_conv = ops.PackedConv(w0, f32('init_conv.bias'), self.cin_pad)

        def res(n):
            r, k = _Res(), n.keys
            r.cout, r.ss_off = n.cout, n.ss_off
            r.conv1 = conv(k['w1'], k['b1'], n.c0, n.c1, ws=True)
            r.g1, r.b1 = f32(k['g1']), f32(k['be1'])
            r.conv2 = conv(k['w2'], k['b2'], n.cout, ws=True)
            r.g2, r.b2 = f32(k['g2']), f32(k['be2'])
            r.res = conv(k['rw'], k['rb'], n.c0, n.c1) if 'rw' in k else None
            return r

        def attn(n):
            a, k, c = _Attn(), n.keys, n.c0
            a.linear = n.kind == 'linattn'
            a.ln_g = f32(k['g']).reshape(-1).contiguous()
            a.pla = None
            if a.linear and c % 32 == 0:
                a.qkv = None
                a.pla = ops.PackedLinAttn(f32(k['qkv']))
            else:
                a.qkv = conv(k['qkv'], None, c)
            a.out = conv(k['ow'], k['ob'], HIDDEN)
            a.out_g = f32(k['og']).reshape(-1).contiguous() if a.linear else None
            a.plo = None
            if a.pla is not None and c == 64:
                a.plo = ops.PackedLinAttnOut(f32(k['ow']), f32(k['ob']), a.out_g)
            return a

        self.blocks = []
        for n in L.nodes:
            k = n.keys
            if n.kind == 'res':
                b = res(n)
            elif n.kind in ('linattn', 'attn'):
                b = attn(n)
            elif n.kind == 'unshuffle':
                w22 = f32(k['w']).reshape(n.cout, n.c0, 2, 2).contiguous()
                b = ops.PackedConv(w22, f32(k['b']), n.c0, 0, stride=2)
            else:
                b = conv(k['w'], k['b'], n.c0, stride=2 if n.kind == 'down4' else 1, ups=1 if n.kind == 'up3' else 0)
            self.blocks.append((n, b))
        nxt = [b for _, b in self.blocks[1:]] + [None]
        self._pixel_stats = [isinstance(a, _Attn) and a.pla is not None for a in nxt]
        self.final_w = f32('final_conv.weight').reshape(L.out_dim, -1).contiguous()
        self.final_b = f32('final_conv.bias')
        res_nodes = [n for n in L.nodes if n.kind == 'res']
        self.mlp_wt = torch.cat([f32(n.keys['mlp_w']).t() for n in res_nodes], dim=1).contiguous()
        self.mlp_b = torch.cat([f32(n.keys['mlp_b']) for n in res_nodes]).contiguous()

    def _res(self, r, x0, x1, ss_all, pixel_stats=False, pre=None, final=None, keep_out=True, fin_out=None):
        B, H, W, _ = x0.shape
        hw = H * W
        rows = self._rows
        y1, st1 = pre if pre is not None else ops.conv2d(r.conv1, x0, x1, want_stats=True, rows=rows)
        ss = ss_all[:, r.ss_off:r.ss_off + 2 * r.cout]
        coef1, bound1 = ops.gn_finalize(st1, r.g1, r.b1, hw, self.groups, ss, want_bound=True, rows=rows)
        y2, st2 = ops.conv2d(r.conv2, y1, in_coef=coef1, want_stats=True, in_bound=bound1, rows=rows)
        coef2 = ops.gn_finalize(st2, r.g2, r.b2, hw, self.groups, rows=rows)
        if final is not None:
            return ops.conv2d(r.res, x0, x1, res=y2, res_coef=coef2, final=final, keep_out=keep_out, fin_out=fin_out, rows=rows)
        if r.res is not None:
            if pixel_stats and r.cout == 64 and r.res.k == 1 and ops.f16x3_default():
                return ops.conv2d(r.res, x0, x1, res=y2, res_coef=coef2, pixel_stats=True, rows=rows)
            x = ops.conv2d(r.res, x0, x1, res=y2, res_coef=coef2, rows=rows)
            return (x, None) if pixel_stats else x
        assert x1 is None
        if pixel_stats:
            if r.cout in ops.PIXEL_STATS_FUSABLE:
                return ops.gn_silu_residual(y2, coef2, x0, pixel_stats=True, rows=rows)
            return ops.gn_silu_residual(y2, coef2, x0, rows=rows), None
        return ops.gn_silu_residual(y2, coef2, x0, rows=rows)

    def _attn(self, a, x, stats=None):
        rows = self._rows
        if a.plo is not None:
            return ops.linear_attention_fused(x, a.ln_g, a.pla, ATTN_SCALE, out=a.plo, stats=stats, rows=rows)
        if a.pla is not None:
            o = ops.linear_attention_fused(x, a.ln_g, a.pla, ATTN_SCALE, stats=stats, rows=rows)
            y = ops.conv2d(a.out, o, rows=rows)
            return ops.chan_layernorm(y, a.out_g, res=x, rows=rows)
        xn = ops.chan_layernorm(x, a.ln_g, rows=rows)
        qkv = ops.conv2d(a.qkv, xn, rows=rows)
        if a.linear:
            o = ops.linear_attention_core(qkv, ATTN_SCALE, rows=rows)
            y = ops.conv2d(a.out, o, rows=rows)
            return ops.chan_layernorm(y, a.out_g, res=x, rows=rows)
        o = ops.attention_core(qkv, ATTN_SCALE, rows=rows)
        return ops.conv2d(a.out, o, res=x, rows=rows)

    def embed(self, time, class_rows, reps):
        B = time.shape[0]
        td = self.t_w2.shape[1]
        cond = torch.empty((reps * B, self.emb_dim), device=time.device, dtype=torch.float32)
        se = ops.fourier_embed(time, self.fourier_w) if self.fourier_w is not None else ops.sinusoidal_embed(time, self.freq)
        hmid = ops.linear(se, self.t_w1, self.t_b1, act_out='gelu')
        for r in range(reps):
            ops.linear(hmid, self.t_w2, self.t_b2, out=cond[r * B:(r + 1) * B, :td])
        if self.has_classes:
            for r, (classes, keep) in enumerate(class_rows):
                ce = ops.class_embed(classes, keep, self.c_table, self.c_null)
                cm = ops.linear(ce, self.c_w1, self.c_b1, act_out='gelu')
                ops.linear(cm, self.c_w2, self.c_b2, out=cond[r * B:(r + 1) * B, td:])
        return cond

    def ss_tables(self, times):
        self.ensure_prepared()
        assert self.has_classes and self.emb_dim == 2 * self.t_w2.shape[1] and self.emb_dim % 4 == 0
        dev, td = self.mlp_wt.device, self.t_w2.shape[1]
        t = torch.as_tensor(list(times), dtype=torch.int64).to(dev)
        ncls = self.c_table.shape[0]
        cls = torch.arange(ncls + 1, dtype=torch.int64, device=dev).clamp(max=ncls - 1)
        keep = torch.ones((ncls + 1,), dtype=torch.uint8, device=dev)
        keep[ncls] = 0
        cond_t = self.embed(t, [(torch.zeros_like(t), None)], 1)
        cond_t[:, td:].zero_()
        cond_c = self.embed(torch.zeros((ncls + 1,), dtype=torch.int64, device=dev), [(cls, keep)], 1)
        cond_c[:, :td].zero_()
        T = ops.linear(cond_t, self.mlp_wt, None, act_in='silu')
        Ct = ops.linear(cond_c, self.mlp_wt, None, act_in='silu')
        return T, Ct

    def stem(self, xin):
        self.ensure_prepared()
        return ops.conv2d(self.init_conv, xin)

    def first_conv(self, x0):
        self.ensure_prepared()
        return ops.conv2d(self.blocks[0][1].conv1, x0, None, want_stats=True)

    def trunk(self, x0, cond, taps=None, first=None, out=None, ss_all=None, rows=None):
        self.ensure_prepared()
        self._rows = rows
        try:
            return self._trunk(x0, cond, taps, first, out, ss_all)
        finally:
            self._rows = None

    def _trunk(self, x0, cond, taps, first, out, ss_all):
        rows = self._rows

        def tap(name, v):
            if taps is not None:
                taps[name] = v
            return v
        if ss_all is None:
            ss_all = ops.linear(cond, self.mlp_wt, self.mlp_b, act_in='silu')
        x = tap('init_conv', x0)
        hs, pst, last = [x], None, len(self.blocks) - 1
        for i, (n, b) in enumerate(self.blocks):
            x1 = hs.pop() if n.c1 else None
            if n.kind == 'res':
                if i == last and FUSED_FINAL and b.res is not None and b.res.k == 1 and b.cout <= 64 \
                        and self.final_w.shape[0] <= 8 and ops.f16x3_default():
                    x, y = self._res(b, x, x1, ss_all, final=(self.final_w, self.final_b), keep_out=taps is not None,
                                     fin_out=out)
                    tap(n.name, x)
                    return y
                if self._pixel_stats[i]:
                    x, pst = self._res(b, x, x1, ss_all, pixel_stats=True)
                else:
                    x = self._res(b, x, x1, ss_all, pre=first if i == 0 else None)
            elif n.kind in ('linattn', 'attn'):
                x, pst = self._attn(b, x, pst), None
            else:
                x = ops.conv2d(b, x, rows=rows)
            tap(n.name, x)
            if n.push:
                hs.append(x)
        y = ops.final_conv_nchw(x, self.final_w, self.final_b)
        if out is not None:
            out.copy_(y)
            return out
        return y
```

dmhomo_amd/ops.py:

```python
import ctypes as C

import os

import torch

from . import _lib
from ._lib import call, ptr, lib

F32 = torch.float32


def _empty(shape, like, dtype=F32):
    return torch.empty(shape, device=like.device, dtype=dtype)


def ws_standardize(w, eps=1e-5):
    w = w.detach().contiguous()
    out = torch.empty_like(w)
    cout = w.shape[0]
    call('dmh_ws_standardize', ptr(w), ptr(out), cout, w.numel() // cout, float(eps))
    return out


class PackBatch:

    def __init__(self):
        self.jobs, self.pre, self.specials, self._keep, self._arr = [], [], [], [], None

    def add(self, src, ws, wpack, cout, c0, c1, kh, transposed):
        self.jobs.append(_lib.DmhPackJob(ptr(src), ptr(ws), ptr(wpack), cout, c0, c1, kh, int(transposed)))
        self._keep.append((src, ws, wpack))
        self._arr = None

    def run(self, eps=1e-5):
        for f in self.pre:
            f()
        if self.jobs:
            if self._arr is None:
                self._arr = (_lib.DmhPackJob * len(self.jobs))(*self.jobs)
            call('dmh_pack_conv_weights_multi', C.cast(self._arr, C.c_void_p), len(self.jobs), float(eps))
        for f in self.specials:
            f()


def f16x3_default():
    return os.environ.get('DMH_CONV3_VARIANT', '9') == '9'


def _batchable(kh, stride, upsample2):
    return kh in (1, 3) and stride == 1 and not upsample2 and os.environ.get('DMH_CONV3_VARIANT', '9') == '9'


class PackedConv:
    __slots__ = ('wpack', 'bias', 'cout', 'c0', 'c1', 'k', 'stride', 'upsample2', '_w', '_up2')

    def __init__(self, w_oihw, bias, c0, c1=0, stride=1, upsample2=0, subpixel=True, batch=None, ws_from=None):
        w = w_oihw.detach()
        assert w.is_contiguous()
        cout, cin, kh, kw = w.shape
        assert cin == c0 + c1 and kh == kw, (w.shape, c0, c1)
        self._w = w
        n_up2 = lib().dmh_conv_up2_pack_floats(cout, c0) if (upsample2 and kh == 3 and c1 == 0 and subpixel) else -1
        self._up2 = n_up2 > 0
        if self._up2:
            self.wpack = _empty((n_up2,), w)
            upsample2 = 2
        else:
            self.wpack = _empty((lib().dmh_conv_pack_floats(cout, c0, c1, kh, kw),), w)
        self.bias = None if bias is None else bias.detach().contiguous()
        self.cout, self.c0, self.c1, self.k, self.stride, self.upsample2 = cout, c0, c1, kh, stride, upsample2
        if batch is not None and _batchable(kh, stride, upsample2):
            if ws_from is not None:
                batch.add(ws_from.detach(), w, self.wpack, cout, c0, c1, kh, 0)
            else:
                batch.add(w, None, self.wpack, cout, c0, c1, kh, 0)
        else:
            assert ws_from is None
            if batch is not None:
                batch.specials.append(self.repack)
            self.repack()

    def repack(self):
        if self._up2:
            call('dmh_pack_conv_weight_up2', ptr(self._w), ptr(self.wpack), self.cout, self.c0)
        else:
            call('dmh_pack_conv_weight', ptr(self._w), ptr(self.wpack), self.cout, self.c0, self.c1, self.k, self.k)


def conv_out_hw(pc, h, w):
    if pc.upsample2:
        return h * 2, w * 2
    if pc.stride == 2:
        return h // 2, w // 2
    return h, w


CONV_LOG = None


def rows_from_keep(keep, extra=0):
    B = keep.shape[0]
    rows = torch.empty((1 + B + extra,), device=keep.device, dtype=torch.int32)
    call('dmh_rows_from_keep', ptr(keep, torch.uint8), B, int(extra), ptr(rows, torch.int32))
    return rows


def _rows(rows):
    return ptr(rows, torch.int32)


def conv2d(pc, src0, src1=None, in_coef=None, res=None, res_coef=None, want_stats=False, in_bound=None, final=None,
           keep_out=True, pixel_stats=False, eps=1e-5, fin_out=None, rows=None):
    B, H, W, c0 = src0.shape
    assert c0 == pc.c0 and (pc.c1 == 0) == (src1 is None), (src0.shape, pc.c0, pc.c1)
    if src1 is not None:
        assert src1.shape == (B, H, W, pc.c1), (src1.shape, pc.c1)
    ho, wo = conv_out_hw(pc, H, W)
    assert keep_out or final is not None
    out = _empty((B, ho, wo, pc.cout), src0) if keep_out else None
    fin_w = fin_b = None
    if final is not None:
        fin_w, fin_b = final
        assert fin_w.shape[1] == pc.cout and fin_w.is_contiguous() and not want_stats, (fin_w.shape, pc.cout)
        if fin_out is None:
            fin_out = _empty((B, fin_w.shape[0], ho, wo), src0)
        assert fin_out.shape == (B, fin_w.shape[0], ho, wo) and fin_out.is_contiguous() and fin_out.dtype == F32
    else:
        assert fin_out is None
    pst = None
    if pixel_stats:
        assert final is None and not want_stats and pc.cout == 64 and pc.k == 1, (pc.cout, pc.k)
        pst = _empty((B, ho * wo, 2), src0)
    stats = None
    if want_stats:
        tiles = lib().dmh_conv_tiles(ho, wo, pc.k, pc.stride)
        stats = _empty((B, tiles, pc.cout, 2), src0)
    if res is not None:
        assert res.shape == (B, ho, wo, pc.cout), (res.shape, (B, ho, wo, pc.cout))
    d = _lib.DmhConv(C.sizeof(_lib.DmhConv), ptr(src0), ptr(src1), ptr(pc.wpack), ptr(pc.bias), ptr(in_coef), ptr(res), ptr(res_coef),
                     ptr(out), ptr(stats), B, H, W, pc.c0, pc.c1, pc.cout, pc.k, pc.k, pc.stride, pc.upsample2,
                     ptr(in_bound), 0 if in_bound is None else in_bound.shape[1],
                     0 if fin_w is None else fin_w.shape[0], ptr(fin_w), ptr(fin_b), ptr(fin_out), ptr(pst), float(eps), _rows(rows))
    if CONV_LOG is not None:
        e0, e1 = torch.cuda.Event(enable_timing=True), torch.cuda.Event(enable_timing=True)
        e0.record()
        call('dmh_conv2d', C.byref(d))
        e1.record()
        CONV_LOG.append((e0, e1, pc.k, pc.stride, B, ho, wo, pc.c0 + pc.c1, pc.cout, pc.upsample2, in_coef is not None))
    else:
        call('dmh_conv2d', C.byref(d))
    if final is not None:
        return out, fin_out
    if pixel_stats:
        return out, pst
    return (out, stats) if want_stats else out


def gn_finalize(stats, gamma, beta, hw, groups, ss=None, eps=1e-5, want_bound=False, rows=None):
    B, tiles, Cc, _ = stats.shape
    coef = _empty((B, 2, Cc), stats)
    ss_ptr, ss_stride = None, 0
    if ss is not None:
        assert ss.stride(1) == 1 and ss.shape[0] == B and ss.shape[1] == 2 * Cc
        ss_ptr, ss_stride = C.c_void_p(ss.data_ptr()), ss.stride(0)
    if want_bound:
        bound = _empty((B, groups), stats)
        call('dmh_gn_finalize_bound', ptr(stats), tiles, ptr(gamma), ptr(beta), ss_ptr, ss_stride, ptr(coef), ptr(bound),
             B, Cc, groups, hw, float(eps), _rows(rows))
        return coef, bound
    call('dmh_gn_finalize', ptr(stats), tiles, ptr(gamma), ptr(beta), ss_ptr, ss_stride, ptr(coef), B, Cc, groups,
         hw, float(eps), _rows(rows))
    return coef


PIXEL_STATS_FUSABLE = (64, 128, 256)


def gn_silu_residual(y, coef, res, pixel_stats=False, eps=1e-5, rows=None):
    B, H, W, Cc = y.shape
    out = torch.empty_like(y)
    if pixel_stats:
        stats = _empty((B, H * W, 2), y)
        call('dmh_gn_silu_residual_stats', ptr(y), ptr(coef), ptr(res), ptr(out), ptr(stats), B, H * W, Cc, float(eps),
             _rows(rows))
        return out, stats
    call('dmh_gn_silu_residual', ptr(y), ptr(coef), ptr(res), ptr(out), B, H * W, Cc, _rows(rows))
    return out


def chan_layernorm(x, g, res=None, eps=1e-5, rows=None):
    Cc = x.shape[-1]
    out = torch.empty_like(x)
    npix = x.numel() // Cc
    call('dmh_chan_layernorm', ptr(x), ptr(g), ptr(res), ptr(out), npix, Cc, float(eps), _rows(rows), npix // x.shape[0])
    return out


def linear_attention_core(qkv, scale, rows=None):
    B, H, W, c = qkv.shape
    assert c == 384
    n = H * W
    partial = _empty((lib().dmh_linattn_partial_floats(B, n),), qkv)
    ctx = _empty((B, 4, 32, 32), qkv)
    out = _empty((B, H, W, 128), qkv)
    call('dmh_linattn_context', ptr(qkv), ptr(partial), B, n, _rows(rows))
    call('dmh_linattn_merge', ptr(partial), ptr(ctx), B, n, _rows(rows))
    call('dmh_linattn_apply', ptr(qkv), ptr(ctx), ptr(out), B, n, float(scale), _rows(rows))
    return out


class PackedLinAttn:

    def __init__(self, w_qkv):
        c = w_qkv.shape[1]
        assert w_qkv.shape[0] == 384 and c % 32 == 0, w_qkv.shape
        w = w_qkv.detach().reshape(384, c).contiguous().float()
        self.c = c
        self.wpack = _empty((lib().dmh_linattn_fused_pack_floats(c),), w)
        call('dmh_linattn_fused_pack', ptr(w), ptr(self.wpack), c)


class PackedLinAttnOut:

    def __init__(self, w_out, bias, ln_g):
        assert tuple(w_out.shape[:2]) == (64, 128), w_out.shape
        w = w_out.detach().reshape(64, 128).contiguous().float()
        self.wpack = _empty((lib().dmh_linattn_out_pack_floats(),), w)
        call('dmh_linattn_out_pack', ptr(w), ptr(self.wpack))
        self.bias = bias.detach().contiguous().float()
        self.ln_g = ln_g.detach().reshape(-1).contiguous().float()


def linear_attention_fused(x, ln_g, pla, scale, eps=1e-5, out=None, stats=None, rows=None):
    B, H, W, c = x.shape
    assert c == pla.c
    n = H * W
    if stats is None:
        stats = _empty((B, n, 2), x)
        call('dmh_pixel_stats', ptr(x), ptr(stats), B * n, c, float(eps), _rows(rows), n)
    assert stats.shape == (B, n, 2)
    ns = lib().dmh_linattn_fused_splits(B, n)
    partial = _empty((B, ns, 4, 1088), x)
    ctx = _empty((B, 4, 32, 32), x)
    call('dmh_linattn_fused_context', ptr(x), ptr(stats), ptr(ln_g), ptr(pla.wpack), ptr(partial), B, n, c, _rows(rows))
    call('dmh_linattn_merge_n', ptr(partial), ptr(ctx), B, n, ns, _rows(rows))
    if out is not None:
        y = _empty((B, H, W, 64), x)
        call('dmh_linattn_fused_apply_out', ptr(x), ptr(stats), ptr(ln_g), ptr(pla.wpack), ptr(ctx), ptr(out.wpack),
             ptr(out.bias), ptr(out.ln_g), ptr(y), B, n, c, float(scale), float(eps), _rows(rows))
        return y
    o = _empty((B, H, W, 128), x)
    call('dmh_linattn_fused_apply', ptr(x), ptr(stats), ptr(ln_g), ptr(pla.wpack), ptr(ctx), ptr(o), B, n, c,
         float(scale), _rows(rows))
    return o


def attention_core(qkv, scale, rows=None):
    B, H, W, c = qkv.shape
    assert c == 384
    out = _empty((B, H, W, 128), qkv)
    call('dmh_attention', ptr(qkv), ptr(out), B, H * W, float(scale), _rows(rows))
    return out


ACT = {None: 0, 'silu': 1, 'gelu': 2}


def sinusoidal_embed(t, freq):
    R, dim = t.shape[0], freq.shape[0] * 2
    out = _empty((R, dim), freq)
    call('dmh_sinusoidal_embed', ptr(t, torch.int64), ptr(freq), ptr(out), R, dim)
    return out


def fourier_embed(t, weights):
    R, half = t.shape[0], weights.shape[0]
    out = _empty((R, 2 * half + 1), weights)
    call('dmh_fourier_embed', ptr(t, torch.int64), ptr(weights), ptr(out), R, half)
    return out


def class_embed(classes, keep, table, null_emb):
    R, dim = classes.shape[0], table.shape[1]
    out = _empty((R, dim), table)
    call('dmh_class_embed', ptr(classes, torch.int64), ptr(keep, torch.uint8), ptr(table), ptr(null_emb), ptr(out), R,
         dim, table.shape[0])
    return out


def linear(x, wt, bias, act_in=None, act_out=None, out=None):
    R, in_dim = x.shape
    out_dim = wt.shape[1]
    assert wt.shape[0] == in_dim and x.stride(1) == 1
    if out is None:
        out = _empty((R, out_dim), wt)
    assert out.shape == (R, out_dim) and out.stride(1) == 1
    call('dmh_linear', C.c_void_p(x.data_ptr()), x.stride(0), ptr(wt), ptr(bias), C.c_void_p(out.data_ptr()),
         out.stride(0), R, in_dim, out_dim, ACT[act_in], ACT[act_out])
    return out


def ss_gather(T, Ct, bias, cursor, classes, keep, out=None):
    B, N = classes.shape[0], T.shape[1]
    if out is None:
        out = _empty((B, N), T)
    assert out.shape == (B, N) and out.is_contiguous() and Ct.shape[1] == N and bias.shape == (N,)
    call('dmh_ss_gather', ptr(T), ptr(Ct), ptr(bias), ptr(cursor, torch.int32), ptr(classes, torch.int64),
         ptr(keep, torch.uint8), Ct.shape[0] - 1, ptr(out), B, N, T.shape[0])
    return out


def assemble_input(a, b=None, m=None, reps=1, cpad=None, out=None):
    B, ca, H, W = a.shape
    cb = 0 if b is None else b.shape[1]
    if cpad is None:
        cpad = (ca + cb + 3) // 4 * 4
    if out is None:
        out = _empty((reps * B, H, W, cpad), a)
    elif tuple(out.shape) != (reps * B, H, W, cpad):
        raise ValueError(f'assemble_input: out has shape {tuple(out.shape)}, expected {(reps * B, H, W, cpad)}')
    call('dmh_assemble_input', ptr(a), ca, ptr(b), cb, ptr(m), ptr(out), B, reps, H * W, cpad)
    return out


def final_conv_nchw(x, w, bias):
    R, H, W, Cc = x.shape
    cout = w.shape[0]
    out = _empty((R, cout, H, W), x)
    call('dmh_final_conv_nchw', ptr(x), ptr(w), ptr(bias), ptr(out), R, H * W, Cc, cout)
    return out


OBJECTIVE = {'pred_noise': 0, 'pred_x0': 1, 'pred_v': 2}
MODE_DDIM, MODE_LAST, MODE_DDPM = 0, 1, 2


def sampler_step(step, model_cond, model_null, x, noise, want_x_start=True, want_pred_noise=False, keep=None):
    img = torch.empty_like(x)
    xs = torch.empty_like(x) if want_x_start else None
    pn = torch.empty_like(x) if want_pred_noise else None
    call('dmh_sampler_step', C.byref(step), ptr(model_cond), ptr(model_null), ptr(x), ptr(noise), ptr(img), ptr(xs),
         ptr(pn), x.numel(), ptr(keep, torch.uint8), x.numel() // x.shape[0])
    return img, xs, pn


def step_table(steps, times, device):
    n = len(steps)
    if n < 1 or len(times) != n:
        raise ValueError(f'step_table: {n} steps, {len(times)} times')
    for i, st in enumerate(steps):
        if st.objective not in (0, 1, 2) or st.mode not in (MODE_DDIM, MODE_LAST, MODE_DDPM):
            raise ValueError(f'step_table: entry {i} has objective {st.objective} / mode {st.mode}')
        if (st.mode == MODE_LAST) != (i == n - 1) and st.mode != MODE_DDPM:
            raise ValueError(f'step_table: entry {i} of {n} has mode {st.mode}: MODE_LAST belongs to the last entry only')
    sz = C.sizeof(_lib.DmhStep)
    arr = (_lib.DmhStep * n)(*steps)
    raw = torch.frombuffer(bytearray(C.string_at(C.addressof(arr), n * sz)), dtype=torch.uint8).clone()
    table = raw.to(device)
    tt = torch.tensor(list(times), dtype=torch.int64).to(device)
    cursor = torch.zeros((1,), dtype=torch.int32, device=device)
    cur = torch.zeros((sz,), dtype=torch.uint8, device=device)
    return table, tt, cursor, cur


def sampler_seek(cursor, k, table, times, cur, tcond):
    call('dmh_sampler_seek', ptr(cursor, torch.int32), int(k), ptr(table, torch.uint8), ptr(times, torch.int64),
         times.shape[0], ptr(cur, torch.uint8), ptr(tcond, torch.int64), tcond.shape[0])


def sampler_step_dev(cur, model_cond, model_null, x, noise, out=None, keep=None):
    img = torch.empty_like(x) if out is None else out
    call('dmh_sampler_step_dev', ptr(cur, torch.uint8), ptr(model_cond), ptr(model_null), ptr(x), ptr(noise), ptr(img),
         None, None, x.numel(), ptr(keep, torch.uint8), x.numel() // x.shape[0])
    return img


def sampler_step_ddp_dev(cur, cursor, draws, model_out, img, noise=None, sample_ids=None, state=None, x_start=None, xin=None,
                         self_cond=False):
    B, Cc, H, W = img.shape
    for t in (model_out, noise, x_start):
        if t is not None and tuple(t.shape) != (B, Cc, H, W):
            raise ValueError(f'sampler_step_ddp_dev: {tuple(t.shape)} against img {(B, Cc, H, W)}')
    cin = Cc * (2 if self_cond else 1)
    if xin is not None:
        if xin.dim() != 4 or tuple(xin.shape[:3]) != (B, H, W):
            raise ValueError(f'sampler_step_ddp_dev: xin {tuple(xin.shape)} against img {(B, Cc, H, W)}')
        cpad = xin.shape[3]
    else:
        cpad = (cin + 3) // 4 * 4
    if sample_ids is not None and sample_ids.shape[0] < B:
        raise ValueError(f'sampler_step_ddp_dev: {sample_ids.shape[0]} sample ids for {B} rows')
    call('dmh_sampler_step_ddp_dev', ptr(cur, torch.uint8), ptr(cursor, torch.int32), ptr(draws, torch.int32), ptr(model_out),
         ptr(img), ptr(noise), ptr(sample_ids, torch.int64), ptr(state, torch.int64), ptr(x_start), ptr(xin), B, Cc, H * W, cpad,
         int(bool(self_cond)))
    return img


def rng_indexed(shape, sample_ids, state, kind=0):
    B = int(shape[0])
    assert sample_ids.shape == (B,) and state.shape == (4,) and state.dtype == torch.int64
    out = torch.empty(tuple(shape), device=sample_ids.device, dtype=F32)
    call('dmh_rng_indexed', ptr(out), B, out.numel() // B, ptr(sample_ids, torch.int64), ptr(state, torch.int64), int(kind))
    return out


def rng_keep_mask(sample_ids, state, prob):
    B = sample_ids.shape[0]
    out = torch.empty((B,), device=sample_ids.device, dtype=torch.uint8)
    call('dmh_rng_keep_mask', ptr(out, torch.uint8), B, ptr(sample_ids, torch.int64), ptr(state, torch.int64), float(prob))
    return out


def affine(x, scale, shift, out=None):
    x = x.contiguous()
    y = torch.empty_like(x) if out is None else out
    call('dmh_affine', ptr(x), ptr(y), float(scale), float(shift), x.numel())
    return y


def lerp(a, b, lam):
    B = a.shape[0]
    ca = torch.full((B,), 1.0 - lam, device=a.device, dtype=torch.float32)
    cb = torch.full((B,), lam, device=a.device, dtype=torch.float32)
    return q_sample(a.contiguous(), b.contiguous(), ca, cb)


def affine_tail_(x, c0, scale, shift):
    B, Cc, H, W = x.shape
    call('dmh_affine_tail', ptr(x), B, Cc, H * W, c0, float(scale), float(shift))
    return x


def q_sample(x_start, noise, ca, cb):
    out = torch.empty_like(x_start)
    B = x_start.shape[0]
    call('dmh_q_sample', ptr(x_start), ptr(noise), ptr(ca), ptr(cb), ptr(out), B, x_start.numel() // B)
    return out


def rows_lincomb(x, ca, y=None, cb=None, div=None, clamp=False):
    x = x.contiguous()
    B = x.shape[0]
    out = torch.empty_like(x)
    call('dmh_rows_lincomb', ptr(x), ptr(None if y is None else y.contiguous()), ptr(ca.contiguous()),
         ptr(None if cb is None else cb.contiguous()), ptr(None if div is None else div.contiguous()), ptr(out), B,
         x.numel() // B, int(bool(clamp)))
    return out


def diff_mean(a, b, mask=None, squared=False):
    B, Cc, H, W = a.shape
    ws = torch.empty((B, 64), device=a.device, dtype=torch.float64)
    out = torch.empty((B,), device=a.device, dtype=F32)
    call('dmh_diff_mean', ptr(a), ptr(b), ptr(mask), int(bool(squared)), ptr(ws, torch.float64), ptr(out), B, Cc,
         H * W)
    return out


def loss_combine(l, photo, w):
    out = torch.empty((1,), device=l.device, dtype=F32)
    call('dmh_loss_combine', ptr(l), ptr(photo), ptr(w), ptr(out), l.shape[0])
    return out[0]


def to_uint8(img):
    out = torch.empty(img.shape, device=img.device, dtype=torch.uint8)
    call('dmh_to_uint8', ptr(img), ptr(out, torch.uint8), img.numel())
    return out


def homography_flow(Hm, H, W, max_flow=256., want_flow=True, want_rgb=True):
    B = Hm.shape[0]
    flow = torch.empty((B, 2, H, W), device=Hm.device, dtype=F32) if want_flow else None
    rgb = torch.empty((B, 3, H, W), device=Hm.device, dtype=F32) if want_rgb else None
    call('dmh_homography_flow', ptr(Hm, torch.float64), ptr(flow), ptr(rgb), B, H, W, float(max_flow))
    return flow, rgb


def flow_to_image(flow, max_flow=256.):
    B, _, H, W = flow.shape
    rgb = torch.empty((B, 3, H, W), device=flow.device, dtype=F32)
    call('dmh_flow_to_image', ptr(flow), ptr(rgb), B, H * W, float(max_flow))
    return rgb


FLOW_WARP_PAD = {'border': 0, 'zeros': 1, 'reflection': 2}
FLOW_WARP_MODE = {'bilinear': 0, 'nearest': 1, 'bicubic': 2}


def flow_warp(x, flow, want_indices=False, pad='border', mode='bilinear'):
    B, Cc, H, W = x.shape
    assert flow.shape == (B, 2, H, W)
    out = torch.empty_like(x)
    x0 = y0 = None
    if want_indices:
        x0 = torch.empty((B, H, W), device=x.device, dtype=torch.int32)
        y0 = torch.empty((B, H, W), device=x.device, dtype=torch.int32)
    call('dmh_flow_warp', ptr(x), ptr(flow), ptr(out), ptr(x0, torch.int32), ptr(y0, torch.int32), B, Cc, H, W,
         FLOW_WARP_PAD[pad], FLOW_WARP_MODE[mode])
    return (out, x0, y0) if want_indices else out


def pixel_grid(B, H, W, start, device):
    out = torch.empty((B, 2, H, W), device=device, dtype=F32)
    call('dmh_pixel_grid', ptr(out), B, H, W, float(start))
    return out


def norm_grid(v):
    B, two, H, W = v.shape
    assert two == 2
    out = torch.empty((B, H, W, 2), device=v.device, dtype=F32)
    call('dmh_norm_grid', ptr(v.contiguous()), ptr(out), B, H, W)
    return out


def homography_flow_points(Hm, idx):
    B, divide = Hm.shape[:2]
    Bi, three, H, W = idx.shape
    assert three == 3 and Hm.shape[2:] == (3, 3)
    out = torch.empty((B, 2, H, W), device=Hm.device, dtype=torch.float64)
    call('dmh_homography_flow_points', ptr(Hm.contiguous(), torch.float64), ptr(idx.contiguous(), torch.float64),
         ptr(out, torch.float64), B, divide, Bi, H, W)
    return out


def dlt_points(src, off):
    N, P, two = src.shape
    assert two == 2 and off.shape == src.shape
    ws = torch.empty((N, _lib.DLT_BLOCKS, 44), device=src.device, dtype=torch.float64)
    out = torch.empty((N, 3, 3), device=src.device, dtype=torch.float64)
    call('dmh_dlt_points', ptr(src.contiguous(), torch.float64), ptr(off.contiguous(), torch.float64),
         ptr(ws, torch.float64), ptr(out, torch.float64), N, P)
    return out


def dlt_homography(flow):
    B, _, H, W = flow.shape
    ws = torch.empty((B, _lib.DLT_BLOCKS, 44), device=flow.device, dtype=torch.float64)
    out = torch.empty((B, 3, 3), device=flow.device, dtype=torch.float64)
    call('dmh_dlt_homography', ptr(flow), ptr(ws, torch.float64), ptr(out, torch.float64), B, H, W)
    return out


def _preview_inputs(img, mask, flow):
    B, C6, H, W = img.shape
    assert C6 == 6 and mask.shape == (B, 1, H, W) and flow.shape == (B, 2, H, W), (img.shape, mask.shape, flow.shape)
    return B, H, W


def post_process(img, mask, flow):
    B, H, W = _preview_inputs(img, mask, flow)
    buf1 = torch.empty((B, 3, H, 4 * W), device=img.device, dtype=F32)
    buf2 = torch.empty_like(buf1)
    call('dmh_post_process', ptr(img), ptr(mask), ptr(flow), ptr(buf1), ptr(buf2), B, H, W)
    return buf1, buf2


def grid_shape(B, H, W, nrow=8, padding=2):
    if B == 1:
        return H, W, 1
    xmaps = min(int(nrow), B)
    ymaps = -(-B // xmaps)
    return ymaps * (H + padding) + padding, xmaps * (W + padding) + padding, xmaps


def preview_sheet(img, mask, flow, nrow=8, padding=2, bgr=True):
    B, H, W = _preview_inputs(img, mask, flow)
    Hs, Ws, _ = grid_shape(B, H, 4 * W, nrow, padding)
    s1 = torch.empty((Hs, Ws, 3), device=img.device, dtype=torch.uint8)
    s2 = torch.empty_like(s1)
    call('dmh_preview_sheet', ptr(img), ptr(mask), ptr(flow), ptr(s1, torch.uint8), ptr(s2, torch.uint8), B, H, W, int(nrow),
         int(padding), int(bool(bgr)))
    return s1, s2


def homography_warp(src, homos, dsize):
    B, C3, H, W = src.shape
    assert C3 == 3 and homos.shape == (B, 3, 3), (src.shape, homos.shape)
    Wd, Hd = int(dsize[0]), int(dsize[1])
    dst = torch.empty((B, 3, Hd, Wd), device=src.device, dtype=F32)
    call('dmh_homography_warp', ptr(src), ptr(homos, torch.float64), ptr(dst), B, H, W, Hd, Wd)
    return dst


def conv_wgrad(dy, src0, src1=None, k=3, in_coef=None, want_bias=True, ups=0):
    B, H, W, cout = dy.shape
    c0 = src0.shape[3]
    c1 = 0 if src1 is None else src1.shape[3]
    dw = _empty((cout, c0 + c1, k, k), dy)
    db = _empty((cout,), dy) if want_bias else None
    work = _empty((lib().dmh_conv_wgrad_workspace_floats(B, H, W, c0, c1, cout, k),), dy)
    call('dmh_conv_wgrad', ptr(dy.contiguous()), ptr(src0), ptr(src1), ptr(in_coef), ptr(dw), ptr(db), ptr(work), B, H, W,
         c0, c1, cout, k, int(ups))
    return (dw, db) if want_bias else dw


class _DgradPacked(PackedConv):
    __slots__ = ()

    def __init__(self, w, c_in_total, batch):
        w = w.detach()
        cout_src, cin_src, kh, kw = w.shape
        assert cin_src == c_in_total and kh == kw and w.is_contiguous()
        self._w, self._up2 = w, False
        self.wpack = _empty((lib().dmh_conv_pack_floats(cin_src, cout_src, 0, kh, kw),), w)
        self.bias = None
        self.cout, self.c0, self.c1, self.k, self.stride, self.upsample2 = cin_src, cout_src, 0, kh, 1, 0
        batch.add(w, None, self.wpack, cin_src, cout_src, 0, kh, 1)


def conv_dgrad_pack(w, c_in_total, batch=None):
    if batch is not None and _batchable(w.shape[-1], 1, 0):
        return _DgradPacked(w, c_in_total, batch)
    wt = w.detach().flip(2, 3).transpose(0, 1).contiguous()
    assert wt.shape[0] == c_in_total
    if batch is not None:
        w_src = w.detach()
        batch.pre.append(lambda: wt.copy_(w_src.flip(2, 3).transpose(0, 1)))
    return PackedConv(wt, None, w.shape[0], batch=batch)


def gn_finalize_train(stats, gamma, beta, hw, groups, ss=None, eps=1e-5):
    B, tiles, Cc, _ = stats.shape
    coef = _empty((B, 2, Cc), stats)
    mr = _empty((B, groups, 2), stats)
    ss_ptr, ss_stride = None, 0
    if ss is not None:
        assert ss.stride(1) == 1 and ss.shape[0] == B and ss.shape[1] == 2 * Cc
        ss_ptr, ss_stride = C.c_void_p(ss.data_ptr()), ss.stride(0)
    call('dmh_gn_finalize_train', ptr(stats), tiles, ptr(gamma), ptr(beta), ss_ptr, ss_stride, ptr(coef), ptr(mr), B, Cc,
         groups, hw, float(eps))
    return coef, mr


def gn_silu_backward(dout, y, coef, mr, gamma, beta, groups, ss=None):
    B, H, W, Cc = y.shape
    hw = H * W
    dy = _empty(y.shape, y)
    pg = _empty((B, 4, Cc), y)
    part = _empty((B, lib().dmh_gn_bwd_chunks(hw), Cc, 2), y)
    bcoef = _empty((B, 3, Cc), y)
    ss_ptr, ss_stride = None, 0
    if ss is not None:
        assert ss.stride(1) == 1 and ss.shape[0] == B and ss.shape[1] == 2 * Cc
        ss_ptr, ss_stride = C.c_void_p(ss.data_ptr()), ss.stride(0)
    call('dmh_gn_silu_backward', ptr(dout), ptr(y), ptr(coef), ptr(mr), ptr(gamma), ptr(beta), ss_ptr, ss_stride, ptr(dy),
         ptr(pg), ptr(part), ptr(bcoef), B, hw, Cc, groups)
    gb = _empty((4, Cc), y)
    call('dmh_sum_over_batch', ptr(pg), ptr(gb), B, 4 * Cc)
    dss = pg.reshape(B, 4 * Cc)[:, 2 * Cc:] if ss is not None else None
    return dy, gb[0], gb[1], dss


def ws_backward(w, dwh, eps=1e-5):
    cout = w.shape[0]
    w, dwh = w.contiguous(), dwh.contiguous()
    dw = torch.empty_like(w)
    call('dmh_ws_backward', ptr(w), ptr(dwh), ptr(dw), cout, w.numel() // cout, float(eps))
    return dw


def chan_layernorm_backward(x, g, dout, eps=1e-5):
    Cc = x.shape[-1]
    x, dout = x.contiguous(), dout.contiguous()
    dx = torch.empty_like(x)
    nb = lib().dmh_lnb_blocks()
    part = _empty((nb, Cc), x)
    call('dmh_chan_layernorm_backward', ptr(x), ptr(g), ptr(dout), ptr(dx), ptr(part), x.numel() // Cc, Cc, float(eps))
    dg = _empty((Cc,), x)
    call('dmh_sum_over_batch', ptr(part), ptr(dg), nb, Cc)
    return dx, dg


def linear_attention_core_train(qkv, scale):
    B, H, W, c = qkv.shape
    assert c == 384
    n = H * W
    partial = _empty((lib().dmh_linattn_partial_floats(B, n),), qkv)
    ctx = _empty((B, 4, 32, 32), qkv)
    ms = _empty((B, 4, 32, 2), qkv)
    out = _empty((B, H, W, 128), qkv)
    call('dmh_linattn_context', ptr(qkv), ptr(partial), B, n, None)
    call('dmh_linattn_merge_ms', ptr(partial), ptr(ctx), ptr(ms), B, n)
    call('dmh_linattn_apply', ptr(qkv), ptr(ctx), ptr(out), B, n, float(scale), None)
    return out, dict(qkv=qkv, ctx=ctx, ms=ms, scale=float(scale))


def linear_attention_core_backward(sv, dout):
    qkv = sv['qkv']
    B, H, W, _ = qkv.shape
    n = H * W
    dqkv = torch.empty_like(qkv)
    work = _empty((lib().dmh_linattn_bwd_workspace_floats(B, n),), qkv)
    call('dmh_linattn_backward', ptr(qkv), ptr(sv['ctx']), ptr(sv['ms']), ptr(dout.contiguous()), ptr(dqkv), ptr(work), B, n,
         sv['scale'])
    return dqkv


def _strides4(*v):
    return (C.c_int64 * 4)(*v)


def bgemm(a, sa, b, sb, c, sc, M, N, K, nbo, nbi, alpha=1.0):
    def base(t):
        if isinstance(t, tuple):
            return C.c_void_p(t[0].data_ptr() + 4 * t[1])
        return ptr(t)
    call('dmh_bgemm', base(a), _strides4(*sa), base(b), _strides4(*sb), base(c), _strides4(*sc), M, N, K, nbo, nbi,
         float(alpha))


def attention_core_train(qkv, scale):
    B, H, W, c = qkv.shape
    assert c == 384
    n = H * W
    S = _empty((B, 4, n, n), qkv)
    bgemm(qkv, (n * 384, 32, 384, 1), (qkv, 128), (n * 384, 32, 1, 384), S, (4 * n * n, n * n, n, 1), n, n, 32, B, 4, scale)
    P = torch.empty_like(S)
    call('dmh_softmax_rows', ptr(S), ptr(P), B * 4 * n, n)
    out = _empty((B, H, W, 128), qkv)
    bgemm(P, (4 * n * n, n * n, n, 1), (qkv, 256), (n * 384, 32, 384, 1), out, (n * 128, 32, 128, 1), n, 32, n, B, 4)
    return out, dict(qkv=qkv, P=P, scale=float(scale))


def attention_core_backward(sv, dout):
    qkv, P, scale = sv['qkv'], sv['P'], sv['scale']
    B, H, W, _ = qkv.shape
    n = H * W
    dout = dout.contiguous()
    dqkv = torch.empty_like(qkv)
    sP, sQ, sO = (4 * n * n, n * n, n, 1), (n * 384, 32, 384, 1), (n * 128, 32, 128, 1)
    bgemm(P, (4 * n * n, n * n, 1, n), dout, sO, (dqkv, 256), sQ, n, 32, n, B, 4)
    dP = torch.empty_like(P)
    bgemm(dout, sO, (qkv, 256), (n * 384, 32, 1, 384), dP, sP, n, n, 32, B, 4)
    call('dmh_softmax_rows_backward', ptr(P), ptr(dP), B * 4 * n, n)
    bgemm(dP, sP, (qkv, 128), sQ, dqkv, sQ, n, 32, n, B, 4, scale)
    bgemm(dP, (4 * n * n, n * n, 1, n), qkv, sQ, (dqkv, 128), sQ, n, 32, n, B, 4, scale)
    return dqkv


def conv_up_backward(dy, x, w, dpack=None):
    B, H, W, c = x.shape
    dpack = dpack or conv_dgrad_pack(w, c)
    gup = conv2d(dpack, dy)
    dx = torch.empty_like(x)
    call('dmh_sumpool2', ptr(gup), ptr(dx), B, H, W, c)
    dw, db = conv_wgrad(dy, x, k=3, ups=1)
    return dx, dw, db


_DOWN_K = {0: {-1: 3, 0: 1}, 1: {0: 2, 1: 0}}


def conv_down_dgrad_pack(w, batch=None):
    cout, c = w.shape[0], w.shape[1]
    w3 = torch.zeros((4 * c, cout, 3, 3), device=w.device, dtype=torch.float32)

    def fill():
        for ry in (0, 1):
            for rx in (0, 1):
                par = ry * 2 + rx
                for a, ky in _DOWN_K[ry].items():
                    for b, kx in _DOWN_K[rx].items():
                        w3[par * c:(par + 1) * c, :, a + 1, b + 1] = w[:, :, ky, kx].t()
    fill()
    if batch is not None:
        batch.pre.append(fill)
    return PackedConv(w3, None, cout, batch=batch)


def conv_down_backward(dy, x, w, dpack=None):
    B, H, W, c = x.shape
    cout = dy.shape[3]
    dpack = dpack or conv_down_dgrad_pack(w)
    g4 = conv2d(dpack, dy)
    dx = torch.empty_like(x)
    call('dmh_d2s', ptr(g4), ptr(dx), B, H // 2, W // 2, c)
    X = _empty((B, H // 2 + 1, W // 2 + 1, 4 * c), x)
    call('dmh_s2d_shift', ptr(x.contiguous()), ptr(X), B, H, W, c)
    dw2, db = conv_wgrad(dy, X, k=2)
    dw = dw2.view(cout, 2, 2, c, 2, 2).permute(0, 3, 4, 1, 5, 2).reshape(cout, c, 4, 4).contiguous()
    return dx, dw, db


def conv_unshuffle_wgrad(dy, x, want_bias=True):
    B, H, W, c = x.shape
    cout = dy.shape[3]
    assert tuple(dy.shape) == (B, H // 2, W // 2, cout), (dy.shape, x.shape)
    dw = _empty((cout, 4 * c, 1, 1), dy)
    db = _empty((cout,), dy) if want_bias else None
    work = _empty((lib().dmh_conv_unshuffle_wgrad_workspace_floats(B, H, W, c, cout),), dy)
    call('dmh_conv_unshuffle_wgrad', ptr(dy.contiguous()), ptr(x.contiguous()), ptr(dw), ptr(db), ptr(work), B, H, W, c, cout)
    return (dw, db) if want_bias else dw


def conv_unshuffle_dgrad_pack(w, batch=None):
    cout, c4 = w.shape[0], w.shape[1]
    c = c4 // 4
    wt = torch.empty((c4, cout, 1, 1), device=w.device, dtype=torch.float32)
    w_src = w.detach()

    def fill():
        wt.view(4, c, cout).copy_(w_src.view(cout, c, 4).permute(2, 1, 0))
    fill()
    if batch is not None:
        batch.pre.append(fill)
    return PackedConv(wt, None, cout, batch=batch)


def conv_unshuffle_backward(dy, x, w, dpack=None):
    B, H, W, c = x.shape
    dpack = dpack or conv_unshuffle_dgrad_pack(w)
    g4 = conv2d(dpack, dy)
    dx = torch.empty_like(x)
    call('dmh_d2s', ptr(g4), ptr(dx), B, H // 2, W // 2, c)
    dw, db = conv_unshuffle_wgrad(dy, x)
    return dx, dw, db


def act(x, mode, dy=None):
    x = x.contiguous()
    out = torch.empty_like(x)
    call('dmh_act', ptr(x), ptr(None if dy is None else dy.contiguous()), ptr(out), x.numel(), {'silu': 1, 'gelu': 2}[mode])
    return out


def add(a, b):
    B = a.shape[0]
    one = torch.ones((B,), device=a.device, dtype=torch.float32)
    return q_sample(a.contiguous(), b.contiguous(), one, one)


def linear_backward(x, w, dy, want_bias=True):
    Bn, cin = x.shape
    cout = w.shape[0]
    x, dy, w = x.contiguous(), dy.contiguous(), w.contiguous()
    dx = _empty((Bn, cin), x)
    dw = _empty((cout, cin), x)
    if cout >= 1024 and cout % 128 == 0:
        nk = cout // 128
        part = _empty((nk, Bn, cin), x)
        bgemm(dy, (0, 128, cout, 1), w, (0, 128 * cin, cin, 1), part, (0, Bn * cin, cin, 1), Bn, cin, 128, 1, nk)
        call('dmh_sum_over_batch', ptr(part), ptr(dx), nk, Bn * cin)
    else:
        bgemm(dy, (0, 0, cout, 1), w, (0, 0, cin, 1), dx, (0, 0, cin, 1), Bn, cin, cout, 1, 1)
    bgemm(dy, (0, 0, 1, cout), x, (0, 0, cin, 1), dw, (0, 0, cin, 1), cout, cin, Bn, 1, 1)
    db = None
    if want_bias:
        db = _empty((cout,), x)
        call('dmh_sum_over_batch', ptr(dy), ptr(db), Bn, cout)
    return dx, dw, db


def loss_backward(out, target, warped, mask, flow, abar, squared=False):
    B, _, H, W = out.shape
    dout = torch.empty_like(out)
    gD = torch.empty((B, 3, H, W), device=out.device, dtype=F32)
    call('dmh_loss_backward', ptr(out), ptr(target.contiguous()), ptr(warped), ptr(mask.contiguous()),
         ptr(flow.contiguous()), ptr(abar.contiguous()), ptr(dout), ptr(gD), B, H, W, int(bool(squared)))
    return dout


def loss_backward_ddp(out, target, w, squared=False, scale=1.0):
    out = out.contiguous()
    B = out.shape[0]
    dout = torch.empty_like(out)
    call('dmh_loss_backward_ddp', ptr(out), ptr(target.contiguous()), ptr(w.to(F32).contiguous()), ptr(dout), B,
         out.numel() // B, int(bool(squared)), float(scale))
    return dout


def sumsq_blocks():
    return int(lib().dmh_sumsq_blocks())


def grad_norm_clip(grads, max_norm):
    nb = sumsq_blocks()
    dev = grads[0].device
    part = torch.empty((len(grads) * nb,), device=dev, dtype=torch.float64)
    for i, gr in enumerate(grads):
        call('dmh_sumsq', ptr(gr), gr.numel(), ptr(part[i * nb:], torch.float64))
    out = torch.empty((2,), device=dev, dtype=F32)
    call('dmh_gradnorm_finalize', ptr(part, torch.float64), part.numel(), float(max_norm), ptr(out))
    return out


def adam_(p, g, m, v, gscale, lr, b1, b2, eps, step):
    call('dmh_adam', ptr(p), ptr(g), ptr(m), ptr(v), ptr(gscale), p.numel(), float(lr), float(b1), float(b2),
         float(eps), int(step))


def ema_(ema, p, decay):
    call('dmh_ema', ptr(ema), ptr(p), p.numel(), float(decay))


def _ptr_table(tensors):
    for t in tensors:
        assert t.is_cuda and t.dtype == F32 and t.is_contiguous()
    return (C.c_void_p * len(tensors))(*[t.data_ptr() for t in tensors])


def clip_adam_multi_(params, grads, ms, vs, max_norm, lr, b1, b2, eps, step):
    n = len(params)
    sizes = (C.c_int64 * n)(*[p.numel() for p in params])
    gt = _ptr_table(grads)
    nb = int(lib().dmh_multi_blocks(sizes, n))
    part = torch.empty((nb,), device=params[0].device, dtype=torch.float64)
    call('dmh_sumsq_multi', gt, sizes, n, ptr(part, torch.float64))
    clip = torch.empty((2,), device=params[0].device, dtype=F32)
    call('dmh_gradnorm_finalize', ptr(part, torch.float64), nb, float(max_norm), ptr(clip))
    call('dmh_adam_multi', _ptr_table(params), gt, _ptr_table(ms), _ptr_table(vs), sizes, n, ptr(clip), float(lr), float(b1),
         float(b2), float(eps), int(step))
    return clip
```

include/dmhomo_hip.h:

```cpp
#ifndef DMHOMO_HIP_H
#define DMHOMO_HIP_H

#include <stdint.h>

#ifdef __cplusplus
extern "C" {
#endif

#define DMH_OK 0
#define DMH_EINVAL (-1)
#define DMH_ELAUNCH (-2)

const char* dmh_last_error(void);
#define DMH_ABI_VERSION 500
int dmh_version(void);


int dmh_ws_standardize(const float* w, float* w_out, int Cout, int K, float eps, void* stream);

int64_t dmh_conv_pack_floats(int Cout, int C0, int C1, int KH, int KW);

int dmh_pack_conv_weight(const float* w_oihw, float* wpack, int Cout, int C0, int C1, int KH, int KW,
                         void* stream);
typedef struct DmhPackJob {
  const float* src;
  float* ws;
  float* wpack;
  int32_t Cout, C0, C1, KH;
  int32_t transposed;
} DmhPackJob;
int dmh_pack_conv_weights_multi(const DmhPackJob* jobs, int njobs, float ws_eps, void* stream);

int64_t dmh_conv_up2_pack_floats(int Cout, int C0);
int dmh_pack_conv_weight_up2(const float* w_oihw, float* wpack, int Cout, int C0, void* stream);

int dmh_rows_from_keep(const uint8_t* keep, int B, int extra, int32_t* rows, void* stream);

typedef struct DmhConv {
  uint64_t struct_size;
  const float* src0;
  const float* src1;
  const float* wpack;
  const float* bias;
  const float* in_coef;
  const float* res;
  const float* res_coef;
  float* out;
  float* stats;
  int32_t B, Hin, Win, C0, C1, Cout;
  int32_t KH, KW;
  int32_t stride;
  int32_t upsample2;
  const float* in_bound;
  int32_t in_bound_n;
  int32_t fin_n;
  const float* fin_w;
  const float* fin_b;
  float* fin_out;
  float* pix_stats;
  float pix_eps;
  const int32_t* rows;
} DmhConv;

int dmh_conv_tiles(int Hout, int Wout, int KH, int stride);
int dmh_conv2d(const DmhConv* d, void* stream);


int dmh_gn_finalize(const float* stats, int tiles, const float* gamma, const float* beta, const float* ss,
                    int64_t ss_stride, float* coef, int B, int C, int groups, int hw, float eps, const int32_t* rows,
                    void* stream);

int dmh_gn_finalize_bound(const float* stats, int tiles, const float* gamma, const float* beta, const float* ss,
                          int64_t ss_stride, float* coef, float* bound, int B, int C, int groups, int hw, float eps,
                          const int32_t* rows, void* stream);

int dmh_gn_silu_residual(const float* y, const float* coef, const float* res, float* out, int B, int HW, int C,
                         const int32_t* rows, void* stream);

int dmh_gn_silu_residual_stats(const float* y, const float* coef, const float* res, float* out, float* pstats, int B,
                               int HW, int C, float eps, const int32_t* rows, void* stream);

int dmh_chan_layernorm(const float* x, const float* g, const float* res, float* out, int64_t npix, int C,
                       float eps, const int32_t* rows, int64_t pix_per_row, void* stream);

int dmh_linattn_splits(int n);
int64_t dmh_linattn_partial_floats(int B, int n);
int dmh_linattn_context(const float* qkv, float* partial, int B, int n, const int32_t* rows, void* stream);
int dmh_linattn_merge(const float* partial, float* ctx, int B, int n, const int32_t* rows, void* stream);
int dmh_linattn_apply(const float* qkv, const float* ctx, float* out, int B, int n, float scale, const int32_t* rows,
                      void* stream);

int dmh_pixel_stats(const float* x, float* stats, int64_t npix, int C, float eps, const int32_t* rows, int64_t pix_per_row,
                    void* stream);
int64_t dmh_linattn_fused_pack_floats(int C);
int dmh_linattn_fused_pack(const float* w_qkv, float* wpack, int C, void* stream);
int dmh_linattn_fused_splits(int B, int n);
int dmh_linattn_fused_context(const float* x, const float* stats, const float* ln_g, const float* wpack,
                              float* partial, int B, int n, int C, const int32_t* rows, void* stream);
int dmh_linattn_merge_n(const float* partial, float* ctx, int B, int n, int nsplit, const int32_t* rows, void* stream);
int dmh_linattn_fused_apply(const float* x, const float* stats, const float* ln_g, const float* wpack,
                            const float* ctx, float* out, int B, int n, int C, float scale, const int32_t* rows,
                            void* stream);
int64_t dmh_linattn_out_pack_floats(void);
int dmh_linattn_out_pack(const float* w_out, float* wpack, void* stream);
int dmh_linattn_fused_apply_out(const float* x, const float* stats, const float* ln_g, const float* wpack,
                                const float* ctx, const float* wopack, const float* out_bias, const float* out_ln_g,
                                float* y, int B, int n, int C, float scale, float eps, const int32_t* rows, void* stream);

int dmh_attention(const float* qkv, float* out, int B, int n, float scale, const int32_t* rows, void* stream);

int dmh_sinusoidal_embed(const int64_t* t, const float* freq, float* out, int R, int dim, void* stream);
int dmh_fourier_embed(const int64_t* t, const float* weights, float* out, int R, int half, void* stream);
int dmh_class_embed(const int64_t* classes, const uint8_t* keep, const float* table, const float* null_emb,
                    float* out, int R, int dim, int num_classes, void* stream);
int dmh_linear(const float* x, int64_t x_stride, const float* wt, const float* bias, float* y, int64_t y_stride,
               int R, int in_dim, int out_dim, int act_in, int act_out, void* stream);

int dmh_ss_gather(const float* T, const float* C, const float* bias, const int32_t* cursor, const int64_t* classes,
                  const uint8_t* keep, int ncls, float* out, int B, int N, int S, void* stream);

int dmh_assemble_input(const float* a, int Ca, const float* b, int Cb, const float* m, float* out, int B, int reps,
                       int HW, int Cpad, void* stream);
int dmh_final_conv_nchw(const float* x, const float* w, const float* bias, float* out, int R, int HW, int C,
                        int Cout, void* stream);

typedef struct DmhStep {
  int32_t objective;
  int32_t clip;
  int32_t mode;
  float cond_scale;
  float sqrt_recip_ac, sqrt_recipm1_ac, sqrt_ac, sqrt_1m_ac;
  float c0, c1, c2;
} DmhStep;
int dmh_sampler_step(const DmhStep* s, const float* model_cond, const float* model_null, const float* x,
                     const float* noise, float* img_out, float* x_start, float* pred_noise, int64_t n,
                     const uint8_t* keep, int64_t per_row, void* stream);

int dmh_sampler_step_dev(const DmhStep* cur_dev, const float* model_cond, const float* model_null, const float* x,
                         const float* noise, float* img_out, float* x_start, float* pred_noise, int64_t n,
                         const uint8_t* keep, int64_t per_row, void* stream);
int dmh_sampler_seek(int32_t* cursor, int k, const DmhStep* table, const int64_t* times, int S, DmhStep* cur,
                     int64_t* tcond, int B, void* stream);

int dmh_sampler_step_ddp_dev(const DmhStep* cur_dev, const int32_t* cursor, const int32_t* draws, const float* model_out,
                             float* img, const float* noise, const int64_t* sample_ids, uint64_t* state, float* x_start,
                             float* xin_next, int B, int C, int HW, int cpad, int self_cond, void* stream);

int dmh_rng_indexed(float* out, int B, int64_t per_sample, const int64_t* sample_ids, uint64_t* state, int kind,
                    void* stream);

int dmh_rng_keep_mask(uint8_t* keep, int B, const int64_t* sample_ids, uint64_t* state, float prob, void* stream);

int dmh_affine(const float* x, float* y, float scale, float shift, int64_t n, void* stream);
int dmh_affine_tail(float* x, int B, int C, int HW, int c0, float scale, float shift, void* stream);
int dmh_rows_lincomb(const float* x, const float* y, const float* ca, const float* cb, const float* dv, float* out, int B,
                     int64_t per_sample, int clamp, void* stream);
int dmh_q_sample(const float* x_start, const float* noise, const float* ca, const float* cb, float* out, int B,
                 int64_t per_sample, void* stream);
int dmh_diff_mean(const float* a, const float* b, const float* m, int squared, double* ws, float* out, int B, int C,
                  int HW, void* stream);
int dmh_loss_combine(const float* l, const float* photo, const float* w, float* out, int B, void* stream);
int dmh_to_uint8(const float* img, uint8_t* out, int64_t n, void* stream);

int dmh_homography_flow(const double* Hm, float* flow, float* rgb, int B, int H, int W, float max_flow,
                        void* stream);
int dmh_flow_to_image(const float* flow, float* rgb, int B, int HW, float max_flow, void* stream);
int dmh_flow_warp(const float* x, const float* flow, float* out, int32_t* x0, int32_t* y0, int B, int C, int H,
                  int W, int pad, int mode, void* stream);
int dmh_pixel_grid(float* out, int B, int H, int W, float start, void* stream);
int dmh_norm_grid(const float* v, float* out, int B, int H, int W, void* stream);
int dmh_homography_flow_points(const double* Hm, const double* idx, double* flow, int B, int divide, int Bi, int H, int W,
                               void* stream);
int dmh_dlt_points(const double* src, const double* off, double* ws, double* Hout, int N, int P, void* stream);
#define DMH_DLT_BLOCKS 64
int dmh_dlt_homography(const float* flow, double* ws, double* Hout, int B, int H, int W, void* stream);


int64_t dmh_conv_wgrad_workspace_floats(int B, int H, int W, int C0, int C1, int Cout, int KH);
int dmh_conv_wgrad(const float* dy, const float* src0, const float* src1, const float* in_coef, float* dw, float* db,
                   float* work, int B, int H, int W, int C0, int C1, int Cout, int KH, int ups, void* stream);
int64_t dmh_conv_unshuffle_wgrad_workspace_floats(int B, int H, int W, int C, int Cout);
int dmh_conv_unshuffle_wgrad(const float* dy, const float* x, float* dw, float* db, float* work, int B, int H, int W, int C,
                             int Cout, void* stream);
int dmh_s2d_shift(const float* x, float* X, int B, int H, int W, int C, void* stream);
int dmh_d2s(const float* in, float* out, int B, int H, int W, int C, void* stream);
int dmh_sumpool2(const float* in, float* out, int B, int H, int W, int C, void* stream);

int dmh_gn_finalize_train(const float* stats, int tiles, const float* gamma, const float* beta, const float* ss,
                          int64_t ss_stride, float* coef, float* mr, int B, int C, int groups, int hw, float eps,
                          void* stream);

int dmh_gn_bwd_chunks(int HW);
int dmh_gn_silu_backward(const float* dout, const float* y, const float* coef, const float* mr, const float* gamma,
                         const float* beta, const float* ss, int64_t ss_stride, float* dy, float* pg, float* part,
                         float* bcoef, int B, int HW, int C, int groups, void* stream);
int dmh_sum_over_batch(const float* in, float* out, int B, int64_t per, void* stream);
int dmh_ws_backward(const float* w, const float* dwh, float* dw, int Cout, int K, float eps, void* stream);

int dmh_lnb_blocks(void);
int dmh_chan_layernorm_backward(const float* x, const float* g, const float* dout, float* dx, float* dg_part,
                                int64_t npix, int C, float eps, void* stream);

int dmh_linattn_merge_ms(const float* partial, float* ctx, float* ms, int B, int n, void* stream);
int64_t dmh_linattn_bwd_workspace_floats(int B, int n);
int dmh_linattn_backward(const float* qkv, const float* ctx, const float* ms, const float* dout, float* dqkv, float* work,
                         int B, int n, float scale, void* stream);

int dmh_bgemm(const float* A, const int64_t* sa, const float* B, const int64_t* sb, float* C, const int64_t* sc, int M,
              int N, int K, int nbo, int nbi, float alpha, void* stream);
int dmh_softmax_rows(const float* S, float* P, int64_t rows, int n, void* stream);
int dmh_softmax_rows_backward(const float* P, float* dP, int64_t rows, int n, void* stream);

int dmh_act(const float* x, const float* dy, float* out, int64_t n, int mode, void* stream);
int dmh_class_embed_backward(const float* d, const int64_t* classes, const unsigned char* keep, float* dtable, float* dnull,
                             int B, int D, int num_classes, void* stream);
int dmh_loss_backward(const float* out, const float* target, const float* warped, const float* mask, const float* flow,
                      const float* abar, float* dout, float* gD, int B, int H, int W, int squared, void* stream);
int dmh_loss_backward_ddp(const float* out, const float* target, const float* w, float* dout, int B, int64_t per, int squared,
                          float scale, void* stream);
int dmh_sumsq_blocks(void);
int dmh_sumsq(const float* g, int64_t n, double* part, void* stream);
int dmh_gradnorm_finalize(const double* part, int n, float max_norm, float* norm_out, void* stream);
int dmh_adam(float* p, const float* g, float* m, float* v, const float* gscale, int64_t n, float lr, float b1, float b2,
             float eps, int step, void* stream);
int dmh_ema(float* ema, const float* p, int64_t n, float decay, void* stream);
int64_t dmh_multi_blocks(const int64_t* n, int count);
int dmh_sumsq_multi(const float* const* g, const int64_t* n, int count, double* part, void* stream);
int dmh_adam_multi(float* const* p, const float* const* g, float* const* m, float* const* v, const int64_t* n, int count,
                   const float* gscale, float lr, float b1, float b2, float eps, int step, void* stream);


int dmh_resize_bilinear_u8(const unsigned char* src, float* dst, int B, int Hs, int Ws, int C, int Hd, int Wd,
                           int64_t dst_bstride, float div, void* stream);
int dmh_mask_open_nearest(const float* src, float* dst, int B, int Hs, int Ws, int Hd, int Wd, int64_t dst_bstride,
                          void* stream);

int dmh_post_process(const float* img, const float* mask, const float* flow, float* buf1, float* buf2, int B, int H, int W,
                     void* stream);
int dmh_preview_sheet(const float* img, const float* mask, const float* flow, unsigned char* sheet1, unsigned char* sheet2,
                      int B, int H, int W, int nrow, int padding, int bgr, void* stream);
int dmh_homography_warp(const float* src, const double* homos, float* dst, int B, int H, int W, int Hd, int Wd, void* stream);

#ifdef __cplusplus
}
#endif
#endif
```

Before: 91.53 images/s.

## Fold second GroupNorm finalize into residual conv and gn_silu_residual kernels

Removes the separate gn_finalize launch for the second GroupNorm in each resnet block. The per-channel affine coefficients are now derived inside the consuming kernel: either the fp16-piece residual conv epilogue or a new gn_silu_residual_gn kernel. Each block reduces the per-tile statistics into LDS before use. This saves a kernel launch and a coefficient round trip to global memory per block, but every consuming workgroup now repeats the stats reduction and uses more LDS, which may lower occupancy.

```diff
diff --git a/dmhomo_amd/_lib.py b/dmhomo_amd/_lib.py
--- a/dmhomo_amd/_lib.py
+++ b/dmhomo_amd/_lib.py
@@ -13,6 +13,12 @@
 
 
 ABI_VERSION = 500
+
+
+class DmhGnSrc(C.Structure):
+    _fields_ = [('stats', C.c_void_p), ('gamma', C.c_void_p), ('beta', C.c_void_p), ('ss', C.c_void_p),
+                ('ss_stride', C.c_int64), ('tiles', C.c_int32), ('hw', C.c_int32), ('groups', C.c_int32),
+                ('eps', C.c_float)]
 
 
 class DmhConv(C.Structure):
@@ -22,7 +28,7 @@
                [(n, C.c_int32) for n in ('B', 'Hin', 'Win', 'C0', 'C1', 'Cout', 'KH', 'KW', 'stride', 'upsample2')] + \
                [('in_bound', C.c_void_p), ('in_bound_n', C.c_int32), ('fin_n', C.c_int32), ('fin_w', C.c_void_p),
                 ('fin_b', C.c_void_p), ('fin_out', C.c_void_p), ('pix_stats', C.c_void_p), ('pix_eps', C.c_float),
-                ('rows', C.c_void_p)]
+                ('rows', C.c_void_p), ('res_gn', DmhGnSrc)]
 
 
 class DmhPackJob(C.Structure):
@@ -55,6 +61,8 @@
     'dmh_gn_silu_residual': (c_int, [c_f32p, c_f32p, c_f32p, c_f32p, c_int, c_int, c_int, C.c_void_p, C.c_void_p]),
     'dmh_gn_silu_residual_stats': (c_int, [c_f32p, c_f32p, c_f32p, c_f32p, c_f32p, c_int, c_int, c_int, c_float, C.c_void_p,
                                            C.c_void_p]),
+    'dmh_gn_silu_residual_gn': (c_int, [c_f32p, C.POINTER(DmhGnSrc), c_f32p, c_f32p, c_f32p, c_int, c_int, c_int, c_float,
+                                        C.c_void_p, C.c_void_p]),
     'dmh_chan_layernorm': (c_int, [c_f32p, c_f32p, c_f32p, c_f32p, c_i64, c_int, c_float, C.c_void_p, c_i64, C.c_void_p]),
     'dmh_linattn_splits': (c_int, [c_int]),
     'dmh_linattn_partial_floats': (c_i64, [c_int, c_int]),
diff --git a/dmhomo_amd/csrc/conv.hip b/dmhomo_amd/csrc/conv.hip
--- a/dmhomo_amd/csrc/conv.hip
+++ b/dmhomo_amd/csrc/conv.hip
@@ -372,6 +372,14 @@
   DMH_REQUIRE(!(d->in_coef && d->src1), "dmh_conv2d: the GroupNorm prologue applies to a single source");
   DMH_REQUIRE(!(d->res_coef && !d->res), "dmh_conv2d: res_coef without res");
   DMH_REQUIRE(d->Cout % 4 == 0, "dmh_conv2d: Cout must be a multiple of 4 (got %d)", d->Cout);
+  if (d->res_gn.stats) {
+    DMH_REQUIRE(d->res && !d->res_coef, "dmh_conv2d: res_gn describes the affine of res and stands instead of res_coef");
+    DMH_REQUIRE(d->res_gn.gamma && d->res_gn.beta && d->res_gn.tiles > 0 && d->res_gn.hw > 0 && d->res_gn.groups > 0 &&
+                    d->Cout % d->res_gn.groups == 0,
+                "dmh_conv2d: incomplete res_gn (or Cout %% groups != 0)");
+    DMH_REQUIRE(d->stride == 1 && (d->KH == 1 || d->KH == 3) && use_f16x3(d->KH, 1),
+                "dmh_conv2d: res_gn rides on the 1x1 / 3x3 fp16-piece kernels (got %dx%d, stride %d)", d->KH, d->KW, d->stride);
+  }
   DMH_REQUIRE(!d->in_bound || (d->in_coef && d->in_bound_n > 0 && d->in_bound_n <= 64),
               "dmh_conv2d: in_bound needs in_coef and 1..64 bounds per sample (got %d)", d->in_bound_n);
   hipStream_t st = (hipStream_t)stream;
diff --git a/dmhomo_amd/csrc/conv_args.h b/dmhomo_amd/csrc/conv_args.h
--- a/dmhomo_amd/csrc/conv_args.h
+++ b/dmhomo_amd/csrc/conv_args.h
@@ -27,6 +27,7 @@
   int ablate;
   int xcd;
   const int32_t* rows;
+  DmhGnSrc res_gn;
 };
 
 
@@ -65,6 +66,8 @@
   a.ablate = 0;
   a.xcd = 1;
   a.rows = d->rows;
+  a.res_gn = d->res_gn;
+  if (!d->res) a.res_gn.stats = nullptr;
   return a;
 }
 
@@ -87,6 +90,7 @@
   static constexpr int EP = 68;
   int b, n0, chn, c4, rsub;
   bool cok;
+  bool rsilu;
   float4 bias, ra, rb, s1, s2, osc;
 
   __device__ __forceinline__ EpilogueRows(const ConvArgs& p, int b_, int n0_) : b(b_), n0(n0_) {
@@ -101,11 +105,20 @@
     s1 = bias;
     s2 = bias;
     osc = make_float4(1.f, 1.f, 1.f, 1.f);
+    rsilu = p.res_coef != nullptr;
     if (cok && p.oscale) osc = ld4(p.oscale + chn);
     if (cok && p.bias) bias = ld4(p.bias + chn);
     if (cok && p.res_coef) {
       ra = ld4(p.res_coef + (size_t)(b * 2 + 0) * p.Cout + chn);
       rb = ld4(p.res_coef + (size_t)(b * 2 + 1) * p.Cout + chn);
+    }
+  }
+
+  __device__ __forceinline__ void res_coef_from_lds(const float* tab, int pitch, int c0) {
+    rsilu = true;
+    if (cok) {
+      ra = ld4(tab + (chn - c0));
+      rb = ld4(tab + pitch + (chn - c0));
     }
   }
 
@@ -154,7 +167,7 @@
       val[i].w = fmaf(val[i].w, osc.w, bias.w);
     }
     if (p.res) {
-      if (p.res_coef) {
+      if (rsilu) {
 #pragma unroll
         for (int i = 0; i < NR; ++i) {
           val[i].x += silu_fast(fmaf(ra.x, rv[i].x, rb.x));
diff --git a/dmhomo_amd/csrc/conv_f16x3.hip b/dmhomo_amd/csrc/conv_f16x3.hip
--- a/dmhomo_amd/csrc/conv_f16x3.hip
+++ b/dmhomo_amd/csrc/conv_f16x3.hip
@@ -3,6 +3,7 @@
 #include "common.h"
 
 #include "conv_args.h"
+#include "gn_derive.h"
 
 typedef _Float16 half8 __attribute__((ext_vector_type(8)));
 typedef _Float16 half4 __attribute__((ext_vector_type(4)));
@@ -30,7 +31,9 @@
   static constexpr int IN_BYTES = IN_H * ROWP;
   static constexpr int EPI_BYTES = 4 * 32 * EpilogueRows::EP * 4;
   static constexpr int TILE_BYTES = IN_BYTES > EPI_BYTES ? IN_BYTES : EPI_BYTES;
-  static constexpr int LDS_BYTES = TILE_BYTES + 16;
+  static constexpr int GN_CH = SUB ? 64 : 64 * WN;
+  static constexpr int GN_OFF = TILE_BYTES + 16;
+  static constexpr int LDS_BYTES = GN_OFF + 2 * GN_CH * 4 + DMH_GN_RED_BYTES;
 };
 
 __device__ __forceinline__ unsigned absbits(float x) { return __float_as_uint(x) & 0x7fffffffu; }
@@ -204,6 +207,11 @@
   issue_prep(0);
 #pragma unroll
   for (int i = 0; i < NLOAD; ++i) issue_one(i);
+  float* gn_tab = reinterpret_cast<float*>(in_tile + Cfg::GN_OFF);
+  const int gn_c0 = UPS == 3 ? by * 64 : by * (64 * WN);
+  if (p.res_gn.stats)
+    gn_derive_block<DMH_GN_NG>(p.res_gn, b, p.Cout, gn_c0, min(Cfg::GN_CH, p.Cout - gn_c0), gn_tab, Cfg::GN_CH,
+                               reinterpret_cast<double*>(gn_tab + 2 * Cfg::GN_CH));
   __syncthreads();
 #ifdef DMH_STAMPS
   if (p.ablate & 128) {
@@ -421,6 +429,7 @@
     const float inv_s = __uint_as_float((unsigned)(e_run - 14) << 23);
     float* wl = lds + wave * (32 * EP);
     EpilogueRows er(p, b, n0);
+    if (p.res_gn.stats) er.res_coef_from_lds(gn_tab, Cfg::GN_CH, gn_c0);
     if (UPS == 3 && p.oscale) er.osc = ld4(p.oscale + nt * 64 + er.c4 * 4);
     er.osc.x *= inv_s;
     er.osc.y *= inv_s;
diff --git a/dmhomo_amd/csrc/gn_derive.h b/dmhomo_amd/csrc/gn_derive.h
--- /dev/null
+++ b/dmhomo_amd/csrc/gn_derive.h
@@ -0,0 +1,104 @@
+#pragma once
+#include "common.h"
+
+struct GnGroupStat {
+  float rstd, meanf, spread;
+};
+
+template <int NG>
+__device__ __forceinline__ void gn_wave_sums(const float* __restrict__ stats, int tiles, int C, int cg, int b, int g0,
+                                             int ng, int lane, double (&s1)[NG], double (&s2)[NG]) {
+#pragma unroll
+  for (int k = 0; k < NG; ++k) s1[k] = s2[k] = 0.0;
+  const int total = tiles * cg;
+  for (int i = lane; i < total; i += 256) {
+    const int tile = i / cg, cc = i % cg;
+    const float* q = stats + ((size_t)(b * tiles + tile) * C + g0 * cg + cc) * 2;
+#pragma unroll
+    for (int k = 0; k < NG; ++k) {
+      if (k < ng) {
+        const float2 st = *reinterpret_cast<const float2*>(q + (size_t)k * cg * 2);
+        s1[k] += (double)st.x;
+        s2[k] += (double)st.y;
+      }
+    }
+  }
+#pragma unroll
+  for (int k = 0; k < NG; ++k) {
+    for (int off = 32; off; off >>= 1) {
+      s1[k] += __shfl_xor(s1[k], off);
+      s2[k] += __shfl_xor(s2[k], off);
+    }
+  }
+}
+
+__device__ __forceinline__ GnGroupStat gn_group_finish(double s1, double s2, int hw, int cg, float eps) {
+  const double n = (double)hw * (double)cg;
+  const double mean = s1 / n;
+  double var = s2 / n - mean * mean;
+  if (var < 0.0) var = 0.0;
+  GnGroupStat st;
+  st.rstd = (float)(1.0 / sqrt(var + (double)eps));
+  st.meanf = (float)mean;
+  st.spread = (s2 > 4096.0 * n * (var + (double)eps)) ? INFINITY : (float)sqrt(s2 > 0.0 ? s2 : 0.0);
+  return st;
+}
+
+__device__ __forceinline__ void gn_channel_coef(const GnGroupStat& st, const float* __restrict__ gamma,
+                                                const float* __restrict__ beta, const float* __restrict__ ss,
+                                                int64_t ss_stride, int b, int c, int C, float& a, float& bb) {
+  a = st.rstd * gamma[c];
+  bb = beta[c] - st.meanf * a;
+  if (ss) {
+    const float sc = ss[b * ss_stride + c] + 1.0f;
+    const float sh = ss[b * ss_stride + C + c];
+    a = a * sc;
+    bb = fmaf(bb, sc, sh);
+  }
+}
+
+__device__ __forceinline__ float gn_bound_term(const GnGroupStat& st, float a, float bb) {
+  return st.spread < INFINITY ? fmaf(fabsf(a), st.spread, fabsf(fmaf(st.meanf, a, bb))) : INFINITY;
+}
+
+template <int NG>
+__device__ __forceinline__ void gn_derive_block(const DmhGnSrc& d, int b, int C, int c0, int cn, float* coef_lds, int cpitch,
+                                                double* red) {
+  const int t = threadIdx.x, cg = C / d.groups;
+  const int gfirst = c0 / cg, glast = (c0 + cn - 1) / cg;
+  for (int gb = gfirst; gb <= glast; gb += NG) {
+    const int ng = min(NG, glast + 1 - gb);
+    double s1[NG], s2[NG];
+    gn_wave_sums<NG>(d.stats, d.tiles, C, cg, b, gb, ng, t, s1, s2);
+    if (gb != gfirst) __syncthreads();
+    if ((t & 63) == 0) {
+#pragma unroll
+      for (int k = 0; k < NG; ++k) {
+        if (k < ng) {
+          red[k * 4 + (t >> 6)] = s1[k];
+          red[(NG + k) * 4 + (t >> 6)] = s2[k];
+        }
+      }
+    }
+    __syncthreads();
+    for (int c = c0 + t; c < c0 + cn; c += 256) {
+      const int k = c / cg - gb;
+      if (k >= 0 && k < ng) {
+        const double* r1 = red + k * 4;
+        const double* r2 = red + (NG + k) * 4;
+        const GnGroupStat st =
+            gn_group_finish((r1[0] + r1[1]) + (r1[2] + r1[3]), (r2[0] + r2[1]) + (r2[2] + r2[3]), d.hw, cg, d.eps);
+        float a, bb;
+        gn_channel_coef(st, d.gamma, d.beta, d.ss, d.ss_stride, b, c, C, a, bb);
+        coef_lds[c - c0] = a;
+        coef_lds[cpitch + c - c0] = bb;
+      }
+    }
+  }
+}
+constexpr int DMH_GN_NG = 8;
+constexpr int DMH_GN_RED_BYTES = 2 * DMH_GN_NG * 4 * 8;
+
+static inline bool dmh_gn_src_ok(const DmhGnSrc& g, int C) {
+  return g.stats && g.gamma && g.beta && g.tiles > 0 && g.hw > 0 && g.groups > 0 && C % g.groups == 0;
+}
diff --git a/dmhomo_amd/csrc/norm.hip b/dmhomo_amd/csrc/norm.hip
--- a/dmhomo_amd/csrc/norm.hip
+++ b/dmhomo_amd/csrc/norm.hip
@@ -1,4 +1,5 @@
 #include "common.h"
+#include "gn_derive.h"
 
 __global__ __launch_bounds__(256) void gn_finalize_kernel(const float* __restrict__ stats, int tiles,
                                                           const float* __restrict__ gamma,
@@ -14,56 +15,64 @@
   const int bg = b * groups + g;
   const int cg = C / groups;
   const int lane = threadIdx.x;
-  double s1 = 0.0, s2 = 0.0;
-  const int total = tiles * cg;
-  for (int i = lane; i < total; i += 256) {
-    const int tile = i / cg, cc = i % cg;
-    const float2 st = *reinterpret_cast<const float2*>(stats + ((size_t)(b * tiles + tile) * C + g * cg + cc) * 2);
-    s1 += (double)st.x;
-    s2 += (double)st.y;
-  }
-  for (int off = 32; off; off >>= 1) {
-    s1 += __shfl_xor(s1, off);
-    s2 += __shfl_xor(s2, off);
-  }
+  double w1[1], w2[1];
+  gn_wave_sums<1>(stats, tiles, C, cg, b, g, 1, lane, w1, w2);
   if ((lane & 63) == 0) {
-    red[0][lane >> 6] = s1;
-    red[1][lane >> 6] = s2;
+    red[0][lane >> 6] = w1[0];
+    red[1][lane >> 6] = w2[0];
   }
   __syncthreads();
-  s1 = (red[0][0] + red[0][1]) + (red[0][2] + red[0][3]);
-  s2 = (red[1][0] + red[1][1]) + (red[1][2] + red[1][3]);
-  const double n = (double)hw * (double)cg;
-  const double mean = s1 / n;
-  double var = s2 / n - mean * mean;
-  if (var < 0.0) var = 0.0;
-  const float rstd = (float)(1.0 / sqrt(var + (double)eps));
-  const float meanf = (float)mean;
+  const GnGroupStat gs = gn_group_finish((red[0][0] + red[0][1]) + (red[0][2] + red[0][3]),
+                                         (red[1][0] + red[1][1]) + (red[1][2] + red[1][3]), hw, cg, eps);
   if (mr && lane == 0) {
-    mr[(size_t)bg * 2 + 0] = meanf;
-    mr[(size_t)bg * 2 + 1] = rstd;
-  }
-  const float spread = (s2 > 4096.0 * n * (var + (double)eps)) ? INFINITY : (float)sqrt(s2 > 0.0 ? s2 : 0.0);
+    mr[(size_t)bg * 2 + 0] = gs.meanf;
+    mr[(size_t)bg * 2 + 1] = gs.rstd;
+  }
   float bmax = 0.f;
   for (int cc = lane; cc < cg; cc += 256) {
     const int c = g * cg + cc;
-    float a = rstd * gamma[c];
-    float bb = beta[c] - meanf * a;
-    if (ss) {
-      const float sc = ss[b * ss_stride + c] + 1.0f;
-      const float sh = ss[b * ss_stride + C + c];
-      a = a * sc;
-      bb = fmaf(bb, sc, sh);
-    }
+    float a, bb;
+    gn_channel_coef(gs, gamma, beta, ss, ss_stride, b, c, C, a, bb);
     coef[(size_t)(b * 2 + 0) * C + c] = a;
     coef[(size_t)(b * 2 + 1) * C + c] = bb;
-    bmax = fmaxf(bmax, spread < INFINITY ? fmaf(fabsf(a), spread, fabsf(fmaf(meanf, a, bb))) : INFINITY);
+    bmax = fmaxf(bmax, gn_bound_term(gs, a, bb));
   }
   if (bound) {
     for (int off = 32; off; off >>= 1) bmax = fmaxf(bmax, __shfl_xor(bmax, off));
     if ((lane & 63) == 0) bred[lane >> 6] = bmax;
     __syncthreads();
     if (lane == 0) bound[bg] = fmaxf(fmaxf(bred[0], bred[1]), fmaxf(bred[2], bred[3]));
+  }
+}
+
+template <int LPP>
+__device__ __forceinline__ void gn_silu_residual_elem(const float4 a, const float4 bb, const float* __restrict__ y,
+                                                      const float* __restrict__ res, float* __restrict__ out, int64_t i,
+                                                      bool ok, int C, float* __restrict__ pstats, float eps) {
+  const int C4 = C >> 2;
+  const float4 v = ld4(y + i * 4);
+  float4 r = make_float4(0.f, 0.f, 0.f, 0.f);
+  if (res) r = ld4(res + i * 4);
+  float4 o;
+  o.x = silu_fast(fmaf(a.x, v.x, bb.x)) + r.x;
+  o.y = silu_fast(fmaf(a.y, v.y, bb.y)) + r.y;
+  o.z = silu_fast(fmaf(a.z, v.z, bb.z)) + r.z;
+  o.w = silu_fast(fmaf(a.w, v.w, bb.w)) + r.w;
+  if (ok) st4(out + i * 4, o);
+  if (LPP > 0) {
+    float s = 0.f;
+    s += (o.x + o.y) + (o.z + o.w);
+    s = lanes_sum<(LPP > 0 ? LPP : 1)>(s);
+    const float mean = s / (float)C;
+    float qsum = 0.f;
+    const float dx = o.x - mean, dy = o.y - mean, dz = o.z - mean, dw = o.w - mean;
+    qsum += (dx * dx + dy * dy) + (dz * dz + dw * dw);
+    qsum = lanes_sum<(LPP > 0 ? LPP : 1)>(qsum);
+    if (ok && (threadIdx.x % (LPP > 0 ? LPP : 1)) == 0) {
+      const int64_t pix = i / C4;
+      pstats[pix * 2 + 0] = mean;
+      pstats[pix * 2 + 1] = 1.0f / sqrtf(qsum / (float)C + eps);
+    }
   }
 }
 
@@ -87,30 +96,32 @@
     const int c = (int)(i % C4) * 4;
     const float4 a = ld4(coef + (size_t)(b * 2 + 0) * C + c);
     const float4 bb = ld4(coef + (size_t)(b * 2 + 1) * C + c);
-    const float4 v = ld4(y + i * 4);
-    float4 r = make_float4(0.f, 0.f, 0.f, 0.f);
-    if (res) r = ld4(res + i * 4);
-    float4 o;
-    o.x = silu_fast(fmaf(a.x, v.x, bb.x)) + r.x;
-    o.y = silu_fast(fmaf(a.y, v.y, bb.y)) + r.y;
-    o.z = silu_fast(fmaf(a.z, v.z, bb.z)) + r.z;
-    o.w = silu_fast(fmaf(a.w, v.w, bb.w)) + r.w;
-    if (ok) st4(out + i * 4, o);
-    if (LPP > 0) {
-      float s = 0.f;
-      s += (o.x + o.y) + (o.z + o.w);
-      s = lanes_sum<(LPP > 0 ? LPP : 1)>(s);
-      const float mean = s / (float)C;
-      float qsum = 0.f;
-      const float dx = o.x - mean, dy = o.y - mean, dz = o.z - mean, dw = o.w - mean;
-      qsum += (dx * dx + dy * dy) + (dz * dz + dw * dw);
-      qsum = lanes_sum<(LPP > 0 ? LPP : 1)>(qsum);
-      if (ok && (threadIdx.x % (LPP > 0 ? LPP : 1)) == 0) {
-        const int64_t pix = i / C4;
-        pstats[pix * 2 + 0] = mean;
-        pstats[pix * 2 + 1] = 1.0f / sqrtf(qsum / (float)C + eps);
-      }
-    }
+    gn_silu_residual_elem<LPP>(a, bb, y, res, out, i, ok, C, pstats, eps);
+  }
+}
+
+template <int LPP>
+__global__ __launch_bounds__(256) void gn_silu_residual_gn_kernel(const float* __restrict__ y, DmhGnSrc gn,
+                                                                  const float* __restrict__ res, float* __restrict__ out,
+                                                                  int64_t per_sample4, int C, float* __restrict__ pstats,
+                                                                  float eps, const int32_t* __restrict__ rows) {
+  extern __shared__ __attribute__((aligned(16))) float gn_lds[];
+  const int jb = blockIdx.y;
+  if (jb >= dmh_rows_n(rows, gridDim.y)) return;
+  const int b = dmh_rows_phys(rows, jb);
+  gn_derive_block<DMH_GN_NG>(gn, b, C, 0, C, gn_lds, C, reinterpret_cast<double*>(gn_lds + 2 * C));
+  __syncthreads();
+  const int C4 = C >> 2;
+  const int lane = threadIdx.x & 63;
+  const int64_t base = (int64_t)b * per_sample4;
+  for (int64_t i0 = (int64_t)blockIdx.x * 256 + threadIdx.x; i0 - lane < per_sample4; i0 += (int64_t)gridDim.x * 256) {
+    const bool ok = i0 < per_sample4;
+    if (LPP == 0 && !ok) break;
+    const int64_t il = ok ? i0 : per_sample4 - 1;
+    const int c = (int)(il % C4) * 4;
+    const float4 a = ld4(gn_lds + c);
+    const float4 bb = ld4(gn_lds + C + c);
+    gn_silu_residual_elem<LPP>(a, bb, y, res, out, base + il, ok, C, pstats, eps);
   }
 }
 
@@ -239,6 +250,31 @@
   return DMH_OK;
 }
 
+extern "C" int dmh_gn_silu_residual_gn(const float* y, const DmhGnSrc* gn, const float* res, float* out, float* pstats, int B,
+                                       int HW, int C, float eps, const int32_t* rows, void* stream) {
+  DMH_REQUIRE(y && gn && out, "dmh_gn_silu_residual_gn: null pointer");
+  DMH_REQUIRE(B > 0 && B <= 65535 && HW > 0 && C > 0 && C % 4 == 0 && C <= 4096,
+              "dmh_gn_silu_residual_gn: bad shape (B %d, HW %d, C %d)", B, HW, C);
+  DMH_REQUIRE(dmh_gn_src_ok(*gn, C), "dmh_gn_silu_residual_gn: incomplete descriptor (or C %% groups != 0)");
+  DMH_REQUIRE(!pstats || C == 64 || C == 128 || C == 256,
+              "dmh_gn_silu_residual_gn: pixel statistics need C = 64, 128 or 256 (got %d)", C);
+  const int64_t per_sample4 = (int64_t)HW * C / 4;
+  const int64_t want = cdiv64(per_sample4, 256), cap = 2048 / B > 0 ? 2048 / B : 1;
+  const dim3 grid((unsigned)(want < cap ? want : cap), (unsigned)B);
+  const size_t lds = (size_t)2 * C * sizeof(float) + DMH_GN_RED_BYTES;
+  hipStream_t st = (hipStream_t)stream;
+  if (!pstats)
+    hipLaunchKernelGGL(gn_silu_residual_gn_kernel<0>, grid, dim3(256), lds, st, y, *gn, res, out, per_sample4, C, pstats, eps, rows);
+  else if (C == 64)
+    hipLaunchKernelGGL(gn_silu_residual_gn_kernel<16>, grid, dim3(256), lds, st, y, *gn, res, out, per_sample4, C, pstats, eps, rows);
+  else if (C == 128)
+    hipLaunchKernelGGL(gn_silu_residual_gn_kernel<32>, grid, dim3(256), lds, st, y, *gn, res, out, per_sample4, C, pstats, eps, rows);
+  else
+    hipLaunchKernelGGL(gn_silu_residual_gn_kernel<64>, grid, dim3(256), lds, st, y, *gn, res, out, per_sample4, C, pstats, eps, rows);
+  DMH_CHECK_LAUNCH("dmh_gn_silu_residual_gn");
+  return DMH_OK;
+}
+
 template <int LPP, int NV>
 static int launch_ln(const float* x, const float* g, const float* res, float* out, int64_t npix, int C, float eps,
                      const int32_t* rows, int64_t ppr, hipStream_t st) {
diff --git a/dmhomo_amd/engine.py b/dmhomo_amd/engine.py
--- a/dmhomo_amd/engine.py
+++ b/dmhomo_amd/engine.py
@@ -19,6 +19,7 @@
         self.module = module
         self.groups = groups
         self._sig = None
+        self._taps = False
         self._rows = None
 
     def _signature(self):
@@ -122,20 +123,26 @@
         ss = ss_all[:, r.ss_off:r.ss_off + 2 * r.cout]
         coef1, bound1 = ops.gn_finalize(st1, r.g1, r.b1, hw, self.groups, ss, want_bound=True, rows=rows)
         y2, st2 = ops.conv2d(r.conv2, y1, in_coef=coef1, want_stats=True, in_bound=bound1, rows=rows)
-        coef2 = ops.gn_finalize(st2, r.g2, r.b2, hw, self.groups, rows=rows)
+        coef2 = gn2 = None
+        fold = not self._taps and (r.res is None or (r.res.k in (1, 3) and r.res.stride == 1 and ops.f16x3_default()))
+        if fold:
+            gn2 = ops.gn_src(st2, r.g2, r.b2, hw, self.groups)
+        else:
+            coef2 = ops.gn_finalize(st2, r.g2, r.b2, hw, self.groups, rows=rows)
         if final is not None:
-            return ops.conv2d(r.res, x0, x1, res=y2, res_coef=coef2, final=final, keep_out=keep_out, fin_out=fin_out, rows=rows)
+            return ops.conv2d(r.res, x0, x1, res=y2, res_coef=coef2, res_gn=gn2, final=final, keep_out=keep_out,
+                              fin_out=fin_out, rows=rows)
         if r.res is not None:
             if pixel_stats and r.cout == 64 and r.res.k == 1 and ops.f16x3_default():
-                return ops.conv2d(r.res, x0, x1, res=y2, res_coef=coef2, pixel_stats=True, rows=rows)
-            x = ops.conv2d(r.res, x0, x1, res=y2, res_coef=coef2, rows=rows)
+                return ops.conv2d(r.res, x0, x1, res=y2, res_coef=coef2, res_gn=gn2, pixel_stats=True, rows=rows)
+            x = ops.conv2d(r.res, x0, x1, res=y2, res_coef=coef2, res_gn=gn2, rows=rows)
             return (x, None) if pixel_stats else x
         assert x1 is None
         if pixel_stats:
             if r.cout in ops.PIXEL_STATS_FUSABLE:
-                return ops.gn_silu_residual(y2, coef2, x0, pixel_stats=True, rows=rows)
-            return ops.gn_silu_residual(y2, coef2, x0, rows=rows), None
-        return ops.gn_silu_residual(y2, coef2, x0, rows=rows)
+                return ops.gn_silu_residual(y2, coef2, x0, pixel_stats=True, rows=rows, gn=gn2)
+            return ops.gn_silu_residual(y2, coef2, x0, rows=rows, gn=gn2), None
+        return ops.gn_silu_residual(y2, coef2, x0, rows=rows, gn=gn2)
 
     def _attn(self, a, x, stats=None):
         rows = self._rows
@@ -197,10 +204,12 @@
     def trunk(self, x0, cond, taps=None, first=None, out=None, ss_all=None, rows=None):
         self.ensure_prepared()
         self._rows = rows
+        self._taps = taps is not None
         try:
             return self._trunk(x0, cond, taps, first, out, ss_all)
         finally:
             self._rows = None
+            self._taps = False
 
     def _trunk(self, x0, cond, taps, first, out, ss_all):
         rows = self._rows
diff --git a/dmhomo_amd/ops.py b/dmhomo_amd/ops.py
--- a/dmhomo_amd/ops.py
+++ b/dmhomo_amd/ops.py
@@ -110,7 +110,7 @@
 
 
 def conv2d(pc, src0, src1=None, in_coef=None, res=None, res_coef=None, want_stats=False, in_bound=None, final=None,
-           keep_out=True, pixel_stats=False, eps=1e-5, fin_out=None, rows=None):
+           keep_out=True, pixel_stats=False, eps=1e-5, fin_out=None, rows=None, res_gn=None):
     B, H, W, c0 = src0.shape
     assert c0 == pc.c0 and (pc.c1 == 0) == (src1 is None), (src0.shape, pc.c0, pc.c1)
     if src1 is not None:
@@ -140,7 +140,8 @@
     d = _lib.DmhConv(C.sizeof(_lib.DmhConv), ptr(src0), ptr(src1), ptr(pc.wpack), ptr(pc.bias), ptr(in_coef), ptr(res), ptr(res_coef),
                      ptr(out), ptr(stats), B, H, W, pc.c0, pc.c1, pc.cout, pc.k, pc.k, pc.stride, pc.upsample2,
                      ptr(in_bound), 0 if in_bound is None else in_bound.shape[1],
-                     0 if fin_w is None else fin_w.shape[0], ptr(fin_w), ptr(fin_b), ptr(fin_out), ptr(pst), float(eps), _rows(rows))
+                     0 if fin_w is None else fin_w.shape[0], ptr(fin_w), ptr(fin_b), ptr(fin_out), ptr(pst), float(eps), _rows(rows),
+                     res_gn.c if res_gn is not None else _lib.DmhGnSrc())
     if CONV_LOG is not None:
         e0, e1 = torch.cuda.Event(enable_timing=True), torch.cuda.Event(enable_timing=True)
         e0.record()
@@ -173,12 +174,31 @@
     return coef
 
 
+class gn_src:
+
+    def __init__(self, stats, gamma, beta, hw, groups, ss=None, eps=1e-5):
+        B, tiles, Cc, _ = stats.shape
+        ss_ptr, ss_stride = None, 0
+        if ss is not None:
+            assert ss.stride(1) == 1 and ss.shape[0] == B and ss.shape[1] == 2 * Cc
+            ss_ptr, ss_stride = C.c_void_p(ss.data_ptr()), ss.stride(0)
+        self.keep = (stats, gamma, beta, ss)
+        self.channels = Cc
+        self.c = _lib.DmhGnSrc(ptr(stats), ptr(gamma), ptr(beta), ss_ptr, ss_stride, tiles, hw, groups, float(eps))
+
+
 PIXEL_STATS_FUSABLE = (64, 128, 256)
 
 
-def gn_silu_residual(y, coef, res, pixel_stats=False, eps=1e-5, rows=None):
+def gn_silu_residual(y, coef, res, pixel_stats=False, eps=1e-5, rows=None, gn=None):
     B, H, W, Cc = y.shape
     out = torch.empty_like(y)
+    if gn is not None:
+        assert coef is None and gn.channels == Cc
+        stats = _empty((B, H * W, 2), y) if pixel_stats else None
+        call('dmh_gn_silu_residual_gn', ptr(y), C.byref(gn.c), ptr(res), ptr(out), ptr(stats), B, H * W, Cc, float(eps),
+             _rows(rows))
+        return (out, stats) if pixel_stats else out
     if pixel_stats:
         stats = _empty((B, H * W, 2), y)
         call('dmh_gn_silu_residual_stats', ptr(y), ptr(coef), ptr(res), ptr(out), ptr(stats), B, H * W, Cc, float(eps),
diff --git a/include/dmhomo_hip.h b/include/dmhomo_hip.h
--- a/include/dmhomo_hip.h
+++ b/include/dmhomo_hip.h
@@ -35,6 +35,18 @@
 int dmh_pack_conv_weight_up2(const float* w_oihw, float* wpack, int Cout, int C0, void* stream);
 
 int dmh_rows_from_keep(const uint8_t* keep, int B, int extra, int32_t* rows, void* stream);
+
+typedef struct DmhGnSrc {
+  const float* stats;
+  const float* gamma;
+  const float* beta;
+  const float* ss;
+  int64_t ss_stride;
+  int32_t tiles;
+  int32_t hw;
+  int32_t groups;
+  float eps;
+} DmhGnSrc;
 
 typedef struct DmhConv {
   uint64_t struct_size;
@@ -60,6 +72,7 @@
   float* pix_stats;
   float pix_eps;
   const int32_t* rows;
+  DmhGnSrc res_gn;
 } DmhConv;
 
 int dmh_conv_tiles(int Hout, int Wout, int KH, int stride);
@@ -79,6 +92,9 @@
 
 int dmh_gn_silu_residual_stats(const float* y, const float* coef, const float* res, float* out, float* pstats, int B,
                                int HW, int C, float eps, const int32_t* rows, void* stream);
+
+int dmh_gn_silu_residual_gn(const float* y, const DmhGnSrc* gn, const float* res, float* out, float* pstats, int B, int HW,
+                            int C, float eps, const int32_t* rows, void* stream);
 
 int dmh_chan_layernorm(const float* x, const float* g, const float* res, float* out, int64_t npix, int C,
                        float eps, const int32_t* rows, int64_t pix_per_row, void* stream);
```

Result: slower. 86.78 images/s (-5.2%).
